# JianCao92/speaker-diarization

Hardware: AMD Instinct MI355X
Metric: diarized audio throughput (CD gw/BIC + CL hi/BIC) (higher is better)
Workload: dtype f64

## Files before the change

include/spkd.h:

```cpp
#ifndef SPKD_H
#define SPKD_H

#include <stddef.h>
#include <stdint.h>

#ifdef __cplusplus
extern "C" {
#endif

#define SPKD_ABI_VERSION 2
#define SPKD_DIM 39
#define SPKD_REC 820

typedef enum {
    SPKD_OK = 0,
    SPKD_EINVAL = 1,
    SPKD_EHIP = 2,
    SPKD_ENONFINITE = 3,
    SPKD_EOVERFLOW = 4,
    SPKD_ENOMEM = 5
} spkd_status;

typedef enum { SPKD_BIC = 0, SPKD_GLR = 1, SPKD_KL2 = 2, SPKD_KL2_PINV = 3 } spkd_kind;


typedef struct spkd_ctx spkd_ctx;

int spkd_abi_version(void);

spkd_status spkd_create(int device, void *stream, spkd_ctx **out);
spkd_status spkd_create_on_stream(int device, void *stream, spkd_ctx **out);
void spkd_destroy(spkd_ctx *ctx);
const char *spkd_last_error(const spkd_ctx *ctx);
spkd_status spkd_sync(spkd_ctx *ctx);

spkd_status spkd_malloc(spkd_ctx *ctx, size_t bytes, void **d_ptr);
spkd_status spkd_free(spkd_ctx *ctx, void *d_ptr);
spkd_status spkd_memcpy_h2d(spkd_ctx *ctx, void *d_dst, const void *h_src, size_t bytes);
spkd_status spkd_memcpy_d2h(spkd_ctx *ctx, void *h_dst, const void *d_src, size_t bytes);
spkd_status spkd_memcpy_d2d(spkd_ctx *ctx, void *d_dst, const void *d_src, size_t bytes);

enum {
    SPKD_T_CALL = 0, SPKD_T_CHUNK_STATS, SPKD_T_REDUCE_SETS, SPKD_T_PAIR_TERMS,
    SPKD_T_CLUSTER_PREP, SPKD_T_MATRIX, SPKD_T_AHC, SPKD_T_GW, SPKD_T_SW, SPKD_N_TIMERS
};
spkd_status spkd_last_kernel_ms(spkd_ctx *ctx, int which, float *ms);

spkd_status spkd_last_gw_items(spkd_ctx *ctx, int64_t *items);

spkd_status spkd_set_stats(spkd_ctx *ctx, const float *d_frames, int64_t n_frames,
                           const int64_t *h_range_begin, const int64_t *h_range_end,
                           const int32_t *h_range_set, int64_t n_ranges,
                           int64_t n_sets, double *d_stats);

#define SPKD_WANT_GLR 1
#define SPKD_WANT_KL2 2
#define SPKD_WANT_KL2_PINV 4
spkd_status spkd_pair_terms(spkd_ctx *ctx, const double *d_stats,
                            const int32_t *h_idx_a, const int32_t *h_idx_b,
                            int64_t n_pairs, int flags, double *h_terms);

spkd_status spkd_distance_matrix(spkd_ctx *ctx, int kind, double lambdac,
                                 const double *d_stats, int64_t n, double *d_matrix);

spkd_status spkd_cluster_in(spkd_ctx *ctx, const double *d_stats, int64_t n, int kind,
                            double lambdac, double threshold, int32_t *h_label,
                            double *h_dist, int64_t dist_cap, int64_t *h_dist_off,
                            int64_t *h_n_done, int64_t *h_n_clusters);

spkd_status spkd_distance_rows(spkd_ctx *ctx, int variant, int kind, double lambdac,
                               const double *d_stats, int64_t n, int64_t row_begin, int64_t row_end,
                               double *d_rows, double *h_stat_max, double *h_stat_min);

typedef struct {
    int32_t kind;
    int32_t trace;
    double lambdac;
    double threshold;
    double winsize;
    double winstep;
    double deltaws;
    double rate;
} spkd_cd_params;

typedef struct {
    int32_t turn;
    int32_t coarse;
    int64_t seq;
    double start, i, d;
    int64_t n1, n2;
} spkd_cand_log;

int64_t spkd_gw_event_capacity(int64_t turn_len, double rate);
int64_t spkd_gw_event_capacity_p(int64_t turn_len, const spkd_cd_params *params);
spkd_status spkd_gw(spkd_ctx *ctx, const float *d_frames, int64_t n_frames,
                    const int64_t *h_turn_begin, const int64_t *h_turn_end, int64_t n_turns,
                    const spkd_cd_params *params, const int64_t *h_ev_off,
                    int32_t *h_n_win, double *h_win_maxd, int32_t *h_win_det,
                    double *h_det_start, double *h_det_maxi, double *h_det_d,
                    double *h_final_start,
                    spkd_cand_log *h_log, int64_t log_cap, int64_t *h_log_count);

spkd_status spkd_gw_ex(spkd_ctx *ctx, const float *d_frames, int64_t n_frames,
                       const int64_t *h_turn_begin, const int64_t *h_turn_end, int64_t n_turns,
                       const spkd_cd_params *params, const int64_t *h_ev_off, int check_capacity,
                       int32_t *h_n_win, double *h_win_maxd, int32_t *h_win_det,
                       double *h_det_start, double *h_det_maxi, double *h_det_d,
                       double *h_final_start,
                       spkd_cand_log *h_log, int64_t log_cap, int64_t *h_log_count);

spkd_status spkd_gw_fused(spkd_ctx *ctx, const float *d_frames, int64_t n_frames,
                          const int64_t *h_turn_begin, const int64_t *h_turn_end, int64_t n_turns,
                          const spkd_cd_params *params, const int64_t *h_ev_off, int check_capacity,
                          int32_t *h_n_win, double *h_win_maxd, int32_t *h_win_det,
                          double *h_det_start, double *h_det_maxi, double *h_det_d,
                          double *h_final_start, double *d_seg_stats,
                          spkd_cand_log *h_log, int64_t log_cap, int64_t *h_log_count);

spkd_status spkd_gather_stats(spkd_ctx *ctx, const double *d_src, int64_t n_src,
                              const int64_t *h_src_index, const int64_t *h_dst_index,
                              int64_t n, int64_t n_dst, double *d_dst);

typedef struct {
    int64_t n_lines;
    int64_t n_redo;
    const int32_t *n_win;
    const double *times;
    const int32_t *turn;
    const int64_t *frame_b;
    const int64_t *frame_e;
    const int64_t *index;
    const int64_t *d_index;
    const int64_t *redo_line;
    const int64_t *redo_begin;
    const int64_t *redo_end;
} spkd_gw_lines_view;

spkd_status spkd_gw_batch(spkd_ctx *ctx, const float *d_frames, int64_t n_frames,
                          const int64_t *h_turn_begin, const int64_t *h_turn_end, int64_t n_turns,
                          const spkd_cd_params *params, const int64_t *h_ev_off,
                          const double *h_turn_start_s, const double *h_turn_end_s,
                          const int64_t *h_turn_file_off, const int64_t *h_turn_file_len,
                          double *d_seg_stats, int want_index, spkd_gw_lines_view *view);

int64_t spkd_sw_window_count(int64_t turn_len, double winsize, double winstep);
spkd_status spkd_sw(spkd_ctx *ctx, const float *d_frames, int64_t n_frames,
                    const int64_t *h_turn_begin, const int64_t *h_turn_end, int64_t n_turns,
                    const spkd_cd_params *params, const int64_t *h_d_off, double *h_d);

enum { SPKD_AHC_AUTO = 0, SPKD_AHC_MONO = 1, SPKD_AHC_WIDE = 2 };

typedef struct {
    int32_t variant;
    int32_t kind;
    int32_t max_spk;
    int32_t path;
    double lambdac;
    double threshold;
} spkd_ahc_params;

spkd_status spkd_ahc(spkd_ctx *ctx, const double *d_stats, const int64_t *h_seg_off,
                     int64_t n_problems, const spkd_ahc_params *params,
                     int32_t *h_n_merges, int32_t *h_merge_a, int32_t *h_merge_b,
                     double *h_merge_d, double *h_stat_max, double *h_stat_min);

spkd_status spkd_ahc_matrix(spkd_ctx *ctx, const double *d_stats, int64_t n, const spkd_ahc_params *params,
                            const double *d_matrix, double stat_max_in, double stat_min_in,
                            int32_t *h_n_merges, int32_t *h_merge_a, int32_t *h_merge_b,
                            double *h_merge_d, double *h_stat_max, double *h_stat_min);

spkd_status spkd_ahc_fused(spkd_ctx *ctx, const float *d_frames, int64_t n_frames,
                           const double *d_records, int64_t n_records, int64_t *d_line_index,
                           const int64_t *h_seg_off, int64_t n_problems,
                           const int64_t *h_redo_line, const int64_t *h_redo_begin,
                           const int64_t *h_redo_end, int64_t n_redo,
                           const spkd_ahc_params *params,
                           const int32_t **h_n_merges, const int32_t **h_merge_a,
                           const int32_t **h_merge_b, const double **h_merge_d,
                           const int32_t **h_labels);

typedef struct {
    int32_t sample_rate, frame_rate, window_width, n_fft, n_mel, n_cep;
    int32_t cms_left, cms_right;
    int32_t delta_width[2];
    float pre_emph;
    float delta_norm[2];
} spkd_mfcc_params;
spkd_status spkd_mfcc(spkd_ctx *ctx, const int16_t *d_pcm, int64_t n_samples,
                      const spkd_mfcc_params *params, const float *h_melfb, const float *h_dct,
                      const float *h_mean, const float *h_scale, const float *h_transform,
                      float *d_features, int64_t *h_n_frames);

typedef struct {
    int32_t n_kernels, n_states, dim;
    const float *mean;
    const float *inv_var;
    const float *log_norm;
    const int32_t *state_off;
    const int32_t *kernel;
    const float *log_weight;
} spkd_gmm_params;
spkd_status spkd_gmm_loglik(spkd_ctx *ctx, const float *d_features, int64_t n_frames,
                            const spkd_gmm_params *params, float *d_scores);

void spkd_py2_roundtrip(double *h_values, int64_t n);
spkd_status spkd_labels_from_merges(int64_t n, int64_t n_merges, const int32_t *h_a,
                                    const int32_t *h_b, int32_t *h_labels);
spkd_status spkd_labels_from_merges_batch(int64_t n_problems, const int64_t *h_seg_off,
                                          const int32_t *h_n_merges, const int32_t *h_a,
                                          const int32_t *h_b, int32_t *h_labels);

spkd_status spkd_count_flags(const int32_t *h_flags, const int64_t *h_off, const int32_t *h_n,
                             int64_t n_groups, int32_t *h_out);

spkd_status spkd_gw_lines(int64_t n_turns, const int64_t *h_off, const int32_t *h_n_det,
                          const double *h_det_start, const double *h_det_maxi,
                          const double *h_final_start, const double *h_turn_start_s,
                          const double *h_turn_end_s, const int64_t *h_turn_begin,
                          const int64_t *h_turn_end, double rate, int text_contract,
                          int64_t n_lines, double *h_times, int64_t *h_frame_b,
                          int64_t *h_frame_e, int64_t *h_index, int32_t *h_line_turn);

spkd_status spkd_vad_viterbi(int64_t n_frames, int32_t n_states, const float *h_scores,
                             int32_t n_words, const int32_t *h_word_state, const double *h_stay,
                             const double *h_exit, const double *h_enter, int64_t *h_tok_frame,
                             int32_t *h_tok_word, int64_t *h_n_tokens, double *h_score);

#ifdef __cplusplus
}
#endif
#endif
```

speaker-diarization_amd/csrc/spkd_cluster.hpp:

```cpp
#pragma once
#include "spkd_device.hpp"
#include "spkd_quad.hpp"
#include "spkd_tri.hpp"
#include "../../include/spkd.h"

namespace spkd {

constexpr double MAXINT_F = 9223372036854775808.0;
constexpr double PEN_UNIT = 39.0 + 0.5 * 39.0 * 40.0;
constexpr int AUX = 3 * DA;
constexpr int ERR_DEGENERATE_MERGE = 2;

__device__ __forceinline__ unsigned long long dkey(double v) {
    unsigned long long b = (unsigned long long)__double_as_longlong(v);
    return (b >> 63) ? ~b : (b | 0x8000000000000000ull);
}
__device__ __forceinline__ double dkey_inv(unsigned long long k) {
    unsigned long long b = (k >> 63) ? (k & 0x7fffffffffffffffull) : ~k;
    return __longlong_as_double((long long)b);
}
template <bool MAXOP>
__device__ __forceinline__ unsigned wave_red_u32(unsigned x) {
    auto op = [](unsigned a, unsigned b) { return MAXOP ? (a > b ? a : b) : (a < b ? a : b); };
    x = op(x, (unsigned)__builtin_amdgcn_update_dpp((int)x, (int)x, 0xB1, 0xf, 0xf, false));
// ... 522 lines not shown
            const double* row = Dm + r * N;
            double mv = __builtin_huge_val();
            int mc = NO_COL, nc = NO_COL;
            for (long long c0 = 0; c0 < N; c0 += 4 * WAVE) {
                double v[4];
                int a[4];
#pragma unroll
                for (int u = 0; u < 4; ++u) {
                    const long long c = c0 + u * WAVE + lane;
                    const long long cc = c < N ? c : N - 1;
                    a[u] = (c < N) ? al[cc] : 0;
                    v[u] = row[cc];
                }
#pragma unroll
                for (int u = 0; u < 4; ++u) {
                    const int c = (int)(c0 + u * WAVE + lane);
                    if (!a[u]) continue;
                    if (v[u] != v[u]) { if (c < nc) nc = c; continue; }
                    if (v[u] < mv || (v[u] == mv && c < mc)) { mv = v[u]; mc = c; }
                }
            }
            {
                unsigned long long okey;
                unsigned oc;
                wave_argmin_key(mc != NO_COL ? dkey(mv) : ~0ull, (unsigned)mc, okey, oc);
                mv = okey != ~0ull ? dkey_inv(okey) : __builtin_huge_val();
                mc = okey != ~0ull ? (int)oc : NO_COL;
                nc = __any(nc != NO_COL) ? (int)wave_red_u32<false>((unsigned)nc) : NO_COL;
            }
            if (lane == 0) { rmin[r] = mv; rarg[r] = mc; rnan[r] = nc; dirty[r] = 0; }
#ifdef SPKD_PROFILE
            if (lane == 0) atomicAdd(&g_ahc_prof[0], 1ull);
#endif
        }
    }
}

template <bool TWO>
__global__ __launch_bounds__(AHC_TPB) void k_ahc(
        double* __restrict__ ex, double* __restrict__ pk, const int64_t* __restrict__ seg_off,
        int variant, int kind, int max_spk, double lambdac, double threshold,
        double* __restrict__ ld, double* __restrict__ aux,
        double* __restrict__ mat, const int64_t* __restrict__ mat_off,
        int32_t* __restrict__ alive, double* __restrict__ tmp,
        double* __restrict__ rmin_all, int32_t* __restrict__ rcache_all,
        int32_t* __restrict__ out_n, int32_t* __restrict__ out_a, int32_t* __restrict__ out_b,
        double* __restrict__ out_d, unsigned long long* stat_max, unsigned long long* stat_min,
        double* __restrict__ final_max, double* __restrict__ final_min, int* err,
        double* pinv_ws) {
    extern __shared__ int32_t ids[];
    __shared__ double ldsA[QREC];
    __shared__ unsigned long long red3[AHC_WAVES][3];
    __shared__ unsigned long long s_masks[AHC_MAX_N / WAVE];
    __shared__ int s_cnt[2];
    __shared__ int s_nids;
    __shared__ int s_next;
    __shared__ double s_tmax[AHC_WAVES];
    const int tid = threadIdx.x, lane = lane_id(), wave = tid >> 6;
    const QuadLane L = quad_lane();
    const int p = blockIdx.x;
    const int64_t off = seg_off[p];
    const long long N = seg_off[p + 1] - off;
    double* Dm = mat + mat_off[p];
    int32_t* al = alive + off;
    double* ldp = ld + off;
    double* tp = tmp + off;
    double* rmin = rmin_all + off;
    int32_t* rarg = rcache_all + 3 * off;
    int32_t* rnan = rarg + N;
    int32_t* dirty = rnan + N;
    for (long long c = tid; c < N; c += AHC_TPB) { al[c] = 1; dirty[c] = 1; }
    __syncthreads();
    long long m = N;
    int n_merges = 0;
    const long long INF_IDX = 0x7fffffffffffffffLL;
    double fmin = 0.0;
#ifdef SPKD_PROFILE
    unsigned long long ahc_acc[5] = {0ull, 0ull, 0ull, 0ull, 0ull}, ahc_t = clock64();
#define AHC_TICK(i) do { const unsigned long long now_ = clock64(); ahc_acc[i] += now_ - ahc_t; ahc_t = now_; } while (0)
#else
#define AHC_TICK(i) ((void)0)
#endif
    while (true) {
        refresh_rows(Dm, N, al, dirty, rmin, rarg, rnan, s_masks, tid, wave, lane);
        __syncthreads();
        AHC_TICK(0);
        unsigned long long kb = ~0ull, ib = ~0ull, inan = ~0ull;
        for (long long r = tid; r < N; r += AHC_TPB) {
            if (!al[r]) continue;
            const double v = rmin[r];
            const int c = rarg[r], nc = rnan[r];
            if (nc != NO_COL) { const unsigned long long l = (unsigned long long)(r * N + nc); inan = l < inan ? l : inan; }
            if (c != NO_COL) {
                const unsigned long long kv = dkey(v);
                if (kv < kb) { kb = kv; ib = (unsigned long long)(r * N + c); }
            }
        }
        {
            const unsigned long long wk = wave_red_u64<false>(kb);
            const unsigned long long wi = wave_red_u64<false>(kb == wk ? ib : ~0ull);
            const unsigned long long wn = __any(inan != ~0ull) ? wave_red_u64<false>(inan) : ~0ull;
            if (lane == 0) { red3[wave][0] = wk; red3[wave][1] = wi; red3[wave][2] = wn; }
        }
        __syncthreads();
        unsigned long long bk = red3[0][0], bi = red3[0][1], bn = red3[0][2];
#pragma unroll
        for (int w = 1; w < AHC_WAVES; ++w) {
            const unsigned long long ok = red3[w][0], oi = red3[w][1], on = red3[w][2];
            const bool t = ok < bk || (ok == bk && oi < bi);
            bk = t ? ok : bk; bi = t ? oi : bi;
            bn = on < bn ? on : bn;
        }
        const bool has_nan = bn != ~0ull;
        const double mind = has_nan ? __builtin_nan("") : (bi != ~0ull ? dkey_inv(bk) : __builtin_huge_val());
        const long long index = has_nan ? (long long)bn : (bi != ~0ull ? (long long)bi : INF_IDX);
        fmin = mind;
        const bool go = (mind <= threshold) || (max_spk > 0 && m > max_spk);
        if (!go) break;
        AHC_TICK(1);
        const long long r0 = index / N, c0 = index - r0 * N;
        if (r0 == c0) {
            if (tid == 0) atomicOr(err, ERR_DEGENERATE_MERGE);
            break;
        }
        const long long sa = r0 < c0 ? r0 : c0, sb = r0 < c0 ? c0 : r0;
        if (tid < 2) s_cnt[tid] = 0;
        if (tid == 0) { s_nids = 1; s_next = 0; }
        __syncthreads();
        {
            int ca = 0, cb = 0;
            for (long long c = tid; c < sb; c += AHC_TPB) {
                if (al[c]) { cb++; if (c < sa) ca++; }
            }
            ca = __builtin_amdgcn_readlane(wave_scan_i32(ca), WAVE - 1);
            cb = __builtin_amdgcn_readlane(wave_scan_i32(cb), WAVE - 1);
            if (lane == 0 && ca) atomicAdd(&s_cnt[0], ca);
            if (lane == 0 && cb) atomicAdd(&s_cnt[1], cb);
        }
        __syncthreads();
        if (tid == 0) {
            const int64_t o = off + n_merges;
            out_a[o] = s_cnt[0]; out_b[o] = s_cnt[1]; out_d[o] = mind;
            al[sb] = 0;
            ids[0] = (int32_t)sa;
        }
        n_merges++;
        m--;
#ifdef SPKD_PROFILE
        if (tid == 0) atomicAdd(&g_ahc_prof[1], 1ull);
#endif
        double* A = ex + (off + sa) * QREC;
        const double* B = ex + (off + sb) * QREC;
        {
            double* Ap = pk + (off + sa) * REC;
            const double* Bp = pk + (off + sb) * REC;
            constexpr int NQ = (QREC + AHC_TPB - 1) / AHC_TPB, NP = (REC + AHC_TPB - 1) / AHC_TPB;
            double qa[NQ], qb[NQ], pa[NP], pb[NP];
#pragma unroll
            for (int u = 0; u < NQ; ++u) {
                const int e = tid + u * AHC_TPB;
                qa[u] = A[e < QREC ? e : 0]; qb[u] = B[e < QREC ? e : 0];
            }
#pragma unroll
            for (int u = 0; u < NP; ++u) {
                const int e = tid + u * AHC_TPB;
                pa[u] = Ap[e < REC ? e : 0]; pb[u] = Bp[e < REC ? e : 0];
            }
#pragma unroll
            for (int u = 0; u < NQ; ++u) {
                const int e = tid + u * AHC_TPB;
                const double v = qa[u] + qb[u];
                if (e < QREC) { A[e] = v; ldsA[e] = v; }
            }
#pragma unroll
            for (int u = 0; u < NP; ++u) {
                const int e = tid + u * AHC_TPB;
                if (e < REC) Ap[e] = pa[u] + pb[u];
            }
        }
        __syncthreads();
        for (long long c0 = 0; c0 < N; c0 += AHC_TPB) {
            const long long c = c0 + tid;
            const bool take = c < N && c != sa && al[c < N ? c : N - 1];
            const unsigned long long mk = __ballot(take);
            int base = 0;
            if (lane == 0 && mk) base = atomicAdd(&s_nids, __popcll(mk));
            base = __shfl(base, 0);
            if (take) ids[base + __popcll(mk & ((1ull << lane) - 1ull))] = (int32_t)c;
        }
        __syncthreads();
        AHC_TICK(2);
        const int nids = s_nids;
        const double nA = ldsA[QREC_COUNT_AT];
        if (kind == SPKD_KL2) {
            if (wave == 0) {
                double a[DA];
                single_rows_from_qr(A, a);
                const double mean_i = a[D] / nA;
                cov_rows(a, nA);
                kl2_aux_from_cov(a, mean_i, aux + (off + sa) * AUX, pinv_ws);
            }
        } else {
            for (;;) {
                int q4 = 0;
                if (lane == 0) q4 = atomicAdd(&s_next, 1);
                const int base = 4 * __builtin_amdgcn_readfirstlane(q4);
                if (base >= nids) break;
                int k = base + L.m;
                const bool valid = k < nids;
                k = valid ? k : nids - 1;
                const int32_t slot = ids[k];
                const double v = quad_pair_det<TWO>(kind, ldsA, nA, A, ex + (off + slot) * QREC, pk + (off + slot) * REC, k == 0, L, err);
                if (valid && L.t == 0) {
                    if (k == 0) ldp[sa] = log(v); else tp[slot] = v;
                }
            }
        }
        __syncthreads();
        AHC_TICK(3);
        double wmax = __builtin_nan(""), wmin = __builtin_nan("");
        const double ldA = ldp[sa];
        for (long long c = tid; c < N; c += AHC_TPB) {
            if (c == sa || !al[c]) continue;
            double d;
            if (kind == SPKD_KL2) {
                const double* a1 = aux + (off + sa) * AUX;
                const double* a2 = aux + (off + c) * AUX;
                double t1 = 0.0, t2 = 0.0;
                for (int i = 0; i < D; ++i) {
                    const float dm = (float)a1[2 * DA + i] - (float)a2[2 * DA + i];
                    const double delta = (double)dm;
                    t1 += (a1[i] - a2[i]) * (a2[DA + i] - a1[DA + i]);
                    t2 += ((a1[DA + i] + a2[DA + i]) * delta) * delta;
                }
                d = 0.5 * t1 + 0.5 * t2;
            } else {
                const double nC = qr_count(ex + (off + c) * QREC);
                d = finish_distance(kind, lambdac, nA, ldA, nC, ldp[c], log(tp[c]));
            }
            Dm[sa * N + c] = d;
            const int ra = rarg[c], rn = rnan[c];
            if (variant == 1) {
                Dm[c * N + sa] = d;
                if (ra == sa || ra == sb || rn == sa || rn == sb) {
                    if (rn != sa && rn != sb && d < rmin[c]) { rmin[c] = d; rarg[c] = (int)sa; }
                    else dirty[c] = 1;
                }
                else if (d != d) { if ((int)sa < rn) rnan[c] = (int)sa; }
                else if (d < rmin[c] || (d == rmin[c] && (int)sa < ra)) { rmin[c] = d; rarg[c] = (int)sa; }
                if (stat_valid(d)) {
                    wmax = (wmax != wmax || d > wmax) ? d : wmax;
                    wmin = (wmin != wmin || d < wmin) ? d : wmin;
                }
            } else {
                if (ra == sb || rn == sb) dirty[c] = 1;
            }
        }
        if (tid == 0) dirty[sa] = 1;
        if (variant == 1) {
            const unsigned long long kmax = wave_red_u64<true>(wmax == wmax ? dkey(wmax) : 0ull);
            const unsigned long long kmin = wave_red_u64<false>(wmin == wmin ? dkey(wmin) : ~0ull);
            if (lane == 0) {
                if (kmax != 0ull) atomicMax(stat_max + p, kmax);
                if (kmin != ~0ull) atomicMin(stat_min + p, kmin);
            }
        }
        __syncthreads();
        AHC_TICK(4);
    }
#ifdef SPKD_PROFILE
    if (tid == 0) for (int i = 0; i < 5; ++i) atomicAdd(&g_ahc_prof[2 + i], ahc_acc[i]);
#endif
    double tmax = -__builtin_huge_val();
    bool anynan = false;
    for (long long r = wave; r < N; r += AHC_WAVES) {
        if (!al[r]) continue;
        const double* row = Dm + r * N;
        for (long long c = lane; c < N; c += WAVE) {
            if (!al[c]) continue;
            const double v = row[c];
            if (v != v) anynan = true; else tmax = v > tmax ? v : tmax;
        }
    }
#pragma unroll
    for (int s = 1; s < WAVE; s <<= 1) {
        const double t2 = __shfl_xor(tmax, s);
        tmax = t2 > tmax ? t2 : tmax;
    }
    anynan = __any(anynan);
    if (lane == 0) s_tmax[wave] = anynan ? __builtin_nan("") : tmax;
    __syncthreads();
    if (tid == 0) {
        double mx = s_tmax[0];
        for (int w = 1; w < AHC_WAVES; ++w) {
            const double x = s_tmax[w];
            if (mx == mx) mx = (x != x) ? x : (x > mx ? x : mx);
        }
        out_n[p] = n_merges;
        final_max[p] = mx;
        final_min[p] = fmin;
    }
}

__device__ __forceinline__ void ahc_scan_row(const double* __restrict__ row, long long N,
                                             const int32_t* __restrict__ al, bool all_alive,
                                             long long sub_col, double sub_val, int lane,
                                             double& mv, int& mc, int& nc) {
    mv = __builtin_huge_val();
    mc = NO_COL; nc = NO_COL;
    for (long long c0 = 0; c0 < N; c0 += 4 * WAVE) {
        double v[4];
        int a[4];
#pragma unroll
        for (int u = 0; u < 4; ++u) {
            const long long c = c0 + u * WAVE + lane;
            const long long cc = c < N ? c : N - 1;
            a[u] = (c < N) ? (all_alive ? 1 : al[cc]) : 0;
            v[u] = row[cc];
        }
#pragma unroll
        for (int u = 0; u < 4; ++u) {
            const long long cl = c0 + u * WAVE + lane;
            const int c = (int)cl;
            if (!a[u]) continue;
            const double x = (cl == sub_col) ? sub_val : v[u];
            if (x != x) { if (c < nc) nc = c; continue; }
            if (x < mv || (x == mv && c < mc)) { mv = x; mc = c; }
        }
    }
#pragma unroll
    for (int s = 1; s < WAVE; s <<= 1) {
        const double v2 = __shfl_xor(mv, s);
        const int c2 = __shfl_xor(mc, s), n2 = __shfl_xor(nc, s);
        if (v2 < mv || (v2 == mv && c2 < mc)) { mv = v2; mc = c2; }
        nc = n2 < nc ? n2 : nc;
    }
}

constexpr int STEP_WAVES = 4;
constexpr int STEP_WIDE_FROM = 1024;
constexpr int STEP_PARTNERS = 4 * STEP_WAVES - 1;
constexpr int ALIVE_ROUND = 0x7fffffff;
constexpr int STEP_MAX_N = 16384;
constexpr int STEP_IDX_SHIFT = 14;

struct StepState {
    int32_t done, n_merges;
    long long psa;
    double fmin;
    double diag;
};

__host__ __device__ inline unsigned long long step_slot_word(int round, int new_slot, int old_slot) {
    return ((unsigned long long)(unsigned)round << 40) | ((unsigned long long)(unsigned)new_slot << 20) |
           (unsigned long long)(unsigned)old_slot;
}
__device__ __forceinline__ int step_slot_of(unsigned long long w, int k) {
    return ((int)(w >> 40) < k) ? (int)((w >> 20) & 0xfffffull) : (int)(w & 0xfffffull);
}

struct StepSel {
    double rmin, newrow;
    int32_t rarg, rnan, death, pad;
};

struct StepArrays {
    double* ex;
    double* pk;
    double* exm;
    double* pkm;
    int32_t* death;
    StepSel* sel2;
    unsigned long long* sw;
    double* cnt;
    StepState* state2;
    int64_t n_total;
    int32_t n_prob;
};

__global__ __launch_bounds__(AHC_TPB) void k_step_init(
        const int64_t* __restrict__ seg_off, const double* __restrict__ mat,
        const int64_t* __restrict__ mat_off, StepArrays Q) {
    const int lane = lane_id(), wave = threadIdx.x >> 6;
    const int p = blockIdx.y;
    const int64_t off = seg_off[p];
    const long long N = seg_off[p + 1] - off;
    if (blockIdx.x == 0 && threadIdx.x == 0) {
        StepState S;
        S.done = 0; S.n_merges = 0; S.psa = -1; S.fmin = 0.0; S.diag = 0.0;
        Q.state2[(size_t)1 * Q.n_prob + p] = S;
        Q.state2[(size_t)0 * Q.n_prob + p] = S;
    }
    const long long r = (long long)blockIdx.x * AHC_WAVES + wave;
    if (r >= N) return;
    double mv;
    int mc, nc;
    ahc_scan_row(mat + mat_off[p] + r * N, N, nullptr, true, -1, 0.0, lane, mv, mc, nc);
    if (lane == 0) {
        StepSel e;
        e.rmin = mv; e.newrow = 0.0; e.rarg = mc; e.rnan = nc; e.death = ALIVE_ROUND; e.pad = 0;
        Q.sel2[Q.n_total + off + r] = e;
        Q.sel2[off + r] = e;
        Q.death[off + r] = ALIVE_ROUND;
        Q.sw[off + r] = step_slot_word(0, (int)r, (int)r);
        Q.cnt[off + r] = Q.pk[(off + r) * REC + REC - 1];
    }
}

__device__ __forceinline__ void step_scan_row(const double* __restrict__ row, long long N,
                                              const int32_t* __restrict__ death, int k, long long sb,
                                              long long sub_col, double sub_val, int lane,
                                              double& mv, int& mc, int& nc) {
    mv = __builtin_huge_val();
    mc = NO_COL; nc = NO_COL;
    for (long long c0 = 0; c0 < N; c0 += 4 * WAVE) {
        double v[4];
        int a[4];
#pragma unroll
        for (int u = 0; u < 4; ++u) {
            const long long c = c0 + u * WAVE + lane;
            const long long cc = c < N ? c : N - 1;
            a[u] = (c < N && c != sb) ? (death[cc] > k ? 1 : 0) : 0;
            v[u] = row[cc];
        }
#pragma unroll
        for (int u = 0; u < 4; ++u) {
            const long long cl = c0 + u * WAVE + lane;
            const int c = (int)cl;
            if (!a[u]) continue;
            const double x = (cl == sub_col) ? sub_val : v[u];
            if (x != x) { if (c < nc) nc = c; continue; }
            if (x < mv || (x == mv && c < mc)) { mv = x; mc = c; }
        }
    }
#pragma unroll
    for (int s = 1; s < WAVE; s <<= 1) {
        const double v2 = __shfl_xor(mv, s);
        const int c2 = __shfl_xor(mc, s), n2 = __shfl_xor(nc, s);
        if (v2 < mv || (v2 == mv && c2 < mc)) { mv = v2; mc = c2; }
        nc = n2 < nc ? n2 : nc;
    }
}

template <bool TWO, int SW, int SP>
__global__ __launch_bounds__(SW * WAVE) void k_ahc_step(
        int k, const int64_t* __restrict__ seg_off, int variant, int kind, int max_spk, double lambdac,
        double threshold, double* __restrict__ ld, double* __restrict__ aux,
        double* __restrict__ mat, const int64_t* __restrict__ mat_off, StepArrays Q,
        int32_t* __restrict__ out_a, int32_t* __restrict__ out_b, double* __restrict__ out_d,
        unsigned long long* stat_max, unsigned long long* stat_min, int* err,
        double* pinv_ws) {
    constexpr int TPB = SW * WAVE;
    extern __shared__ int32_t s_dyn[];
    __shared__ double ldsA[QREC];
    __shared__ double s_auxA[AUX];
    __shared__ double s_ldx[4 * STEP_WAVES];
    __shared__ double s_dfin[4 * STEP_WAVES];
    __shared__ int s_rescan[4 * STEP_WAVES];
    struct RowRed { double mv; int mc, nc; };
    struct WaveRed { unsigned long long kb, kr, kmax, kmin; unsigned ib, inan; int mc, nc; };
    __shared__ WaveRed wred[SW];
    __shared__ int s_cnt[2];
    const int tid = threadIdx.x, lane = lane_id(), wave = tid >> 6;
    const QuadLane L = quad_lane();
    const int p = blockIdx.y;
#ifdef SPKD_PROFILE
    unsigned long long st_t = clock64();
#define STEP_TICK(i) do { const unsigned long long now_ = clock64(); if (blockIdx.x == 0 && tid == 0) atomicAdd(&g_ahc_prof[i], now_ - st_t); st_t = now_; } while (0)
    unsigned long long st_f = st_t;
#define STEP_FINE(i) do { const unsigned long long now_ = clock64(); if (blockIdx.x == 0 && tid == 0) atomicAdd(&g_step_prof[i], now_ - st_f); st_f = now_; } while (0)
#else
#define STEP_TICK(i) ((void)0)
#define STEP_FINE(i) ((void)0)
#endif
    asm volatile("" :: "s"(Q.state2), "s"(Q.sel2), "s"(Q.sw), "s"(Q.ex), "s"(Q.exm), "s"(Q.n_total), "s"(Q.n_prob),
                 "s"(seg_off), "s"(mat_off), "s"(mat), "s"(k));
    StepState S = Q.state2[(size_t)(k & 1) * Q.n_prob + p];
    StepState* Snext = Q.state2 + (size_t)((k + 1) & 1) * Q.n_prob + p;
    int64_t off = seg_off[p], off_end = seg_off[p + 1], moff = mat_off[p];
    asm volatile("" :: "s"(S.done), "s"(S.n_merges), "s"(off), "s"(off_end), "s"(moff));
    const long long N = off_end - off;
    const bool lead = blockIdx.x == 0;
    if (S.done) {
        if (lead && tid == 0) *Snext = S;
        return;
    }
    STEP_FINE(0);
    const int n_merges = S.n_merges;
    const long long psa = S.psa;
    const long long m = N - n_merges;
    const int n_part = (int)(m - 2);
    constexpr int sp = SP;
    const int nb = n_part > 0 ? (n_part + sp - 1) / sp : 1;
    if ((int)blockIdx.x > nb) return;
    const bool keeper = (int)blockIdx.x == nb;
    int32_t* s_ids = s_dyn;
    int32_t* s_slot = s_dyn + N;
    const int nch = (int)((N + WAVE - 1) / WAVE);
    int32_t* s_base = s_dyn + 2 * N;
    unsigned long long* s_mask = reinterpret_cast<unsigned long long*>(s_dyn + ((2 * N + nch + 1) & ~1LL));
    const int rb = k & 1, wb = (k + 1) & 1;
    const int32_t* death = Q.death + off;
    const StepSel* sel_r = Q.sel2 + (size_t)rb * Q.n_total + off;
    StepSel* sel_w = Q.sel2 + (size_t)wb * Q.n_total + off;
    double* Dm = mat + moff;
    double* ldp = ld + off;
    const long long INF_IDX = 0x7fffffffffffffffLL;
    auto rec_quad = [&](int slot) -> const double* {
        return slot < N ? Q.ex + (off + slot) * QREC : Q.exm + (off + (slot - N)) * QREC;
    };
    auto rec_packed = [&](int slot) -> const double* {
        return slot < N ? Q.pk + (off + slot) * REC : Q.pkm + (off + (slot - N)) * REC;
    };
    const double diag_psa = S.diag;
    const bool hp = psa >= 0, v1 = variant == 1;
    const unsigned NONE = 0xffffffffu;
    unsigned long long kb = ~0ull, kr = ~0ull, kmax = 0ull, kmin = ~0ull;
    unsigned ib = NONE, inan = NONE;
    int mc = NO_COL, nc = NO_COL;
    constexpr int SEL_U = 8;
    for (long long xb = 0; xb < N; xb += (long long)SEL_U * TPB) {
        const long long x0 = xb + tid;
        int dth[SEL_U], c_[SEL_U], rn_[SEL_U];
        unsigned long long w_[SEL_U];
        double dn_[SEL_U], v_[SEL_U];
#pragma unroll
        for (int u = 0; u < SEL_U; ++u) {
            if (xb + (long long)u * TPB < N) {
                const long long x = x0 + (long long)u * TPB;
                const long long xc = x < N ? x : N - 1;
                const StepSel e = sel_r[xc];
                w_[u] = Q.sw[off + xc];
                dth[u] = e.death; dn_[u] = e.newrow; v_[u] = e.rmin; c_[u] = e.rarg; rn_[u] = e.rnan;
            }
        }
#pragma unroll
        for (int u = 0; u < SEL_U; ++u) {
            if (xb + (long long)u * TPB >= N) break;
            const long long x = x0 + (long long)u * TPB;
            const unsigned xu = (unsigned)x;
            const bool in = x < N;
            const bool a = in && dth[u] >= k;
            const unsigned long long mk = __ballot(a);
            if (in) {
                s_slot[x] = a ? step_slot_of(w_[u], k) : -1;
                if (lane == 0) s_mask[x >> 6] = mk;
            }
            const bool np = a && x != psa;
            const unsigned long long kv = dkey(v_[u]);
            const bool bet = np && c_[u] != NO_COL && kv < kb;
            kb = bet ? kv : kb;
            ib = bet ? ((xu << STEP_IDX_SHIFT) | (unsigned)c_[u]) : ib;
            const unsigned ni = (np && rn_[u] != NO_COL) ? ((xu << STEP_IDX_SHIFT) | (unsigned)rn_[u]) : NONE;
            inan = ni < inan ? ni : inan;
            if (hp) {
                const double d = x == psa ? diag_psa : dn_[u];
                const bool dnan = d != d;
                const unsigned long long kd = dkey(d);
                const bool bt = a && !dnan && kd < kr;
                kr = bt ? kd : kr;
                mc = bt ? (int)x : mc;
                nc = (a && dnan && (int)x < nc) ? (int)x : nc;
                if (v1) {
                    const bool sv = np && stat_valid(d);
                    kmax = (sv && kd > kmax) ? kd : kmax;
                    kmin = (sv && kd < kmin) ? kd : kmin;
                }
            }
        }
    }
    STEP_FINE(1);
    {
        WaveRed w;
        wave_argmin_key(kb, ib, w.kb, w.ib);
        w.inan = __any(inan != NONE) ? wave_red_u32<false>(inan) : NONE;
        w.kr = ~0ull; w.mc = NO_COL; w.nc = NO_COL; w.kmax = 0ull; w.kmin = ~0ull;
        if (hp) {
            unsigned mcu;
            wave_argmin_key(kr, (unsigned)mc, w.kr, mcu);
            w.mc = (int)mcu;
            if (__any(nc != NO_COL)) w.nc = (int)wave_red_u32<false>((unsigned)nc);
            if (v1) { w.kmax = wave_red_u64<true>(kmax); w.kmin = wave_red_u64<false>(kmin); }
        }
        STEP_FINE(2);
        if (lane == 0) wred[wave] = w;
    }
    __syncthreads();
    WaveRed fw[SW];
#pragma unroll
    for (int w = 0; w < SW; ++w) fw[w] = wred[w];
#pragma unroll
    for (int st = 1; st < SW; st <<= 1) {
#pragma unroll
        for (int w = 0; w + st < SW; w += 2 * st) {
            WaveRed& x = fw[w];
            const WaveRed& o = fw[w + st];
            const bool b1 = o.kb < x.kb || (o.kb == x.kb && o.ib < x.ib);
            x.kb = b1 ? o.kb : x.kb; x.ib = b1 ? o.ib : x.ib;
            x.inan = o.inan < x.inan ? o.inan : x.inan;
            const bool b2 = o.kr < x.kr || (o.kr == x.kr && o.mc < x.mc);
            x.kr = b2 ? o.kr : x.kr; x.mc = b2 ? o.mc : x.mc;
            x.nc = o.nc < x.nc ? o.nc : x.nc;
            x.kmax = o.kmax > x.kmax ? o.kmax : x.kmax;
            x.kmin = o.kmin < x.kmin ? o.kmin : x.kmin;
        }
    }
// ... 363 lines not shown
```

speaker-diarization_amd/csrc/spkd_hip.hip:

```cpp
#include <hip/hip_runtime.h>

#include <algorithm>
#include <cmath>
#include <cstddef>
#include <cstdio>
#include <cstdlib>
#include <cstring>
#include <string>
#include <atomic>
#include <thread>
#include <vector>

#include "../../include/spkd.h"
#include "spkd_cd.hpp"
#include "spkd_cluster.hpp"
#include "spkd_device.hpp"
#include "spkd_handoff.hpp"
#include "spkd_stats.hpp"
#include "spkd_mfcc.hpp"
#include "spkd_vad.hpp"

using namespace spkd;

namespace {
constexpr int N_SLOTS = 40;
enum { PIN_GW_TURNS = 0, PIN_GW_LINES, PIN_AHC_OUT, N_PIN };
}

struct spkd_ctx {
    int device = 0;
    hipStream_t stream = nullptr;
    bool own_stream = false;
    bool gw_lds_ok = false;
    int gw_waves = 0;
    unsigned long long init_keys[2] = {0ull, ~0ull};
    int step_waves = 0;
    int step_partners = 0;
    int64_t last_gw_items = 0;
    std::string err;
    int* d_err = nullptr;
    unsigned long long* d_counter = nullptr;
    hipEvent_t ev0 = nullptr, ev1 = nullptr;
    float last_ms = 0.f;
    hipEvent_t ka[SPKD_N_TIMERS] = {}, kb[SPKD_N_TIMERS] = {};
    bool kused[SPKD_N_TIMERS] = {};
    float kms[SPKD_N_TIMERS] = {};
    void* slot[N_SLOTS] = {};
    size_t slot_bytes[N_SLOTS] = {};
    void* pinv_ws = nullptr;
    double* pinv_cur = nullptr;
    void* pin[N_PIN] = {};
    size_t pin_bytes[N_PIN] = {};
    std::vector<int64_t> redo_line, redo_begin, redo_end;
    std::vector<Chunk> redo_chunks;
    std::vector<int64_t> redo_setoff;
    std::vector<int32_t> redo_sets;
};

namespace {

spkd_status fail(spkd_ctx* c, spkd_status s, const std::string& msg) {
    if (c) c->err = msg;
    return s;
}

#define HIPCHK(c, call)                                                              \
    do {                                                                             \
        hipError_t e_ = (call);                                                      \
        if (e_ != hipSuccess)                                                        \
            return fail((c), SPKD_EHIP, std::string(#call) + ": " + hipGetErrorString(e_)); \
    } while (0)

#define TRY(expr) do { const spkd_status s_ = (expr); if (s_ != SPKD_OK) return s_; } while (0)

spkd_status scratch(spkd_ctx* c, int slot, size_t bytes, void** out) {
    if (bytes == 0) bytes = 16;
    if (c->slot_bytes[slot] < bytes) {
        if (c->slot[slot]) HIPCHK(c, hipFree(c->slot[slot]));
        c->slot[slot] = nullptr;
        c->slot_bytes[slot] = 0;
        size_t want = bytes + bytes / 4;
        hipError_t e = hipMalloc(&c->slot[slot], want);
        if (e != hipSuccess) {
            want = bytes;
            e = hipMalloc(&c->slot[slot], want);
        }
        if (e != hipSuccess) return fail(c, SPKD_ENOMEM, "scratch allocation failed");
        c->slot_bytes[slot] = want;
    }
    *out = c->slot[slot];
    return SPKD_OK;
}

spkd_status pinned(spkd_ctx* c, int which, size_t bytes, void** out) {
    if (bytes == 0) bytes = 16;
    if (c->pin_bytes[which] < bytes) {
        if (c->pin[which]) HIPCHK(c, hipHostFree(c->pin[which]));
        c->pin[which] = nullptr;
        c->pin_bytes[which] = 0;
        const size_t want = bytes + bytes / 4;
        if (hipHostMalloc(&c->pin[which], want, hipHostMallocDefault) != hipSuccess) {
            c->pin[which] = nullptr;
            return fail(c, SPKD_ENOMEM, "pinned host allocation failed");
        }
        c->pin_bytes[which] = want;
    }
    *out = c->pin[which];
    return SPKD_OK;
}

template <class T>
spkd_status upload(spkd_ctx* c, int slot, const T* h, size_t n, T** d) {
    void* p = nullptr;
    TRY(scratch(c, slot, n * sizeof(T), &p));
    if (n) HIPCHK(c, hipMemcpyAsync(p, h, n * sizeof(T), hipMemcpyHostToDevice, c->stream));
    *d = (T*)p;
    return SPKD_OK;
}

struct Layout {
    char* const base;
    char* const stage;
    size_t at = 0;
    explicit Layout(void* b = nullptr, void* s = nullptr) : base((char*)b), stage((char*)s) {}
    template <class T>
    Layout& part(T*& p, size_t count, const T* src = nullptr) {
        at = (at + alignof(T) - 1) / alignof(T) * alignof(T);
        p = base ? (T*)(base + at) : nullptr;
        if (stage && src) std::memcpy(stage + at, src, count * sizeof(T));
        at += count * sizeof(T);
        return *this;
    }
    size_t bytes() const { return at; }
};

template <class Parts>
spkd_status carve(spkd_ctx* c, spkd_status (*alloc)(spkd_ctx*, int, size_t, void**), int slot, Parts parts) {
    void* p = nullptr;
    TRY(alloc(c, slot, parts(Layout()), &p));
    parts(Layout(p));
    return SPKD_OK;
}

template <class Parts>
spkd_status upload_parts(spkd_ctx* c, int slot, std::vector<char>& image, Parts parts) {
    image.resize(parts(Layout()));
    parts(Layout(nullptr, image.data()));
    char* d = nullptr;
    TRY(upload(c, slot, image.data(), image.size(), &d));
    parts(Layout(d));
    return SPKD_OK;
}

struct Call {
    spkd_ctx* const c;
    spkd_status opened;
    int herr = 0;
    bool drained = false;
    explicit Call(spkd_ctx* ctx) : c(ctx) { opened = open(); }
    ~Call() { if (!drained) (void)hipStreamSynchronize(c->stream); }
    spkd_status open() {
        HIPCHK(c, hipSetDevice(c->device));
        for (int i = 0; i < SPKD_N_TIMERS; ++i) c->kused[i] = false;
        HIPCHK(c, hipMemsetAsync(c->d_err, 0, sizeof(int), c->stream));
        HIPCHK(c, hipEventRecord(c->ev0, c->stream));
        return SPKD_OK;
    }

    spkd_status finish() {
        HIPCHK(c, hipEventRecord(c->ev1, c->stream));
        HIPCHK(c, hipMemcpyAsync(&herr, c->d_err, sizeof(int), hipMemcpyDeviceToHost, c->stream));
        HIPCHK(c, hipStreamSynchronize(c->stream));
        drained = true;
        HIPCHK(c, hipEventElapsedTime(&c->last_ms, c->ev0, c->ev1));
        c->kms[0] = c->last_ms;
        for (int i = 1; i < SPKD_N_TIMERS; ++i)
            if (c->kused[i]) HIPCHK(c, hipEventElapsedTime(&c->kms[i], c->ka[i], c->kb[i]));
        if (herr & ERR_SWEEP) return fail(c, SPKD_EHIP, "internal error: growing-window sweep order");
        if (herr & 4) return fail(c, SPKD_EOVERFLOW, "device scratch capacity exceeded");
        if (herr & ERR_DEGENERATE_MERGE) return fail(c, SPKD_EINVAL, "degenerate merge: a diagonal cell was the minimum");
        if (herr & ERR_NONFINITE) return fail(c, SPKD_ENONFINITE, "array must not contain infs or NaNs");
        return SPKD_OK;
    }
};

spkd_status use_kind(spkd_ctx* c, int kind, int* base) {
    c->pinv_cur = nullptr;
    *base = kind;
    if (kind != SPKD_KL2_PINV) return SPKD_OK;
    *base = SPKD_KL2;
    if (!c->pinv_ws) {
        if (hipMalloc(&c->pinv_ws, PINV_WS_BYTES) != hipSuccess) {
            c->pinv_ws = nullptr;
            return fail(c, SPKD_ENOMEM, "pinv workspace allocation failed");
        }
        HIPCHK(c, hipMemsetAsync(c->pinv_ws, 0, PINV_LOCK_BYTES, c->stream));
    }
    c->pinv_cur = (double*)c->pinv_ws;
    return SPKD_OK;
}

bool bad_kind(int kind) { return kind < 0 || kind > 3; }

template <class Params>
spkd_status kernel_params(spkd_ctx* c, const Params*& P, Params& Pk) {
    Pk = *P;
    TRY(use_kind(c, P->kind, &Pk.kind));
    P = &Pk;
    return SPKD_OK;
}

struct Timer {
    spkd_ctx* const c;
    const int idx;
    Timer(spkd_ctx* ctx, int i) : c(ctx), idx(i) { (void)hipEventRecord(c->ka[idx], c->stream); }
    ~Timer() { (void)hipEventRecord(c->kb[idx], c->stream); c->kused[idx] = true; }
};

enum {
    S_CHUNKS = 0, S_SETOFF, S_PARTIAL, S_IDXA, S_IDXB, S_TERMS, S_TURNS, S_SNAP, S_CAND,
    S_GW_N_WIN, S_GW_WIN_DET, S_GW_WIN_MAXD, S_GW_DET_START, S_GW_DET_MAXI, S_GW_DET_D, S_GW_FINAL_START, S_LOG,
    S_AHC_STATS, S_AHC_LD, S_AHC_AUX, S_AHC_MAT, S_AHC_MISC, S_AHC_OUT, S_AHC_OFF, S_AHC_PROB, S_AHC_PACKED, S_MFCC_TAB, S_MFCC_STATIC,
    S_STEP_EXM, S_STEP_PKM, S_STEP_MISC, S_GMM_TAB, S_GMM_IDX,
    S_CP_TURNS, S_CP_TIMES, S_CP_LINES, S_REDO_STATS, S_REDO_IDX, S_COUNT
};
static_assert(S_COUNT <= N_SLOTS, "scratch slot table too small");

}

extern "C" {

int spkd_abi_version(void) { return SPKD_ABI_VERSION; }

static spkd_status create_ctx(int device, void* stream, bool borrow, spkd_ctx** out) {
    if (!out) return SPKD_EINVAL;
    *out = nullptr;
    int count = 0;
    if (hipGetDeviceCount(&count) != hipSuccess || device < 0 || device >= count) return SPKD_EHIP;
    spkd_ctx* c = new spkd_ctx();
    c->device = device;
    if (hipSetDevice(device) != hipSuccess) { delete c; return SPKD_EHIP; }
    if (borrow) {
        c->stream = (hipStream_t)stream;
    } else {
        if (hipStreamCreateWithFlags(&c->stream, hipStreamDefault) != hipSuccess) { delete c; return SPKD_EHIP; }
        c->own_stream = true;
    }
    if (hipMalloc(&c->d_err, sizeof(int)) != hipSuccess ||
        hipMalloc(&c->d_counter, 2 * sizeof(unsigned long long)) != hipSuccess ||
        hipEventCreate(&c->ev0) != hipSuccess || hipEventCreate(&c->ev1) != hipSuccess) {
        spkd_destroy(c);
        return SPKD_EHIP;
    }
    for (int i = 0; i < SPKD_N_TIMERS; ++i)
        if (hipEventCreate(&c->ka[i]) != hipSuccess || hipEventCreate(&c->kb[i]) != hipSuccess) {
            spkd_destroy(c);
            return SPKD_EHIP;
        }
    int lds_max = 0;
    c->gw_lds_ok = hipDeviceGetAttribute(&lds_max, hipDeviceAttributeMaxSharedMemoryPerBlock, device) == hipSuccess &&
                   Gw<4>::LDS_BYTES <= lds_max &&
                   hipFuncSetAttribute((const void*)k_gw<8>, hipFuncAttributeMaxDynamicSharedMemorySize, Gw<8>::LDS_BYTES) == hipSuccess &&
                   hipFuncSetAttribute((const void*)k_gw<4>, hipFuncAttributeMaxDynamicSharedMemorySize, Gw<4>::LDS_BYTES) == hipSuccess &&
                   hipFuncSetAttribute((const void*)k_gw<2>, hipFuncAttributeMaxDynamicSharedMemorySize, Gw<2>::LDS_BYTES) == hipSuccess &&
                   hipFuncSetAttribute((const void*)k_gw<1>, hipFuncAttributeMaxDynamicSharedMemorySize, Gw<1>::LDS_BYTES) == hipSuccess;
    if (const char* e = getenv("SPKD_GW_WAVES")) c->gw_waves = atoi(e);
    if (const char* e = getenv("SPKD_STEP_WAVES")) { const int v = atoi(e); c->step_waves = (v == 4 || v == 8) ? v : 0; }
    if (const char* e = getenv("SPKD_STEP_PARTNERS")) { const int v = atoi(e); c->step_partners = (v == 3 || v == 7 || v == 15) ? v : 0; }
    *out = c;
    return SPKD_OK;
}

spkd_status spkd_create(int device, void* stream, spkd_ctx** out) {
    return create_ctx(device, stream, stream != nullptr, out);
}

spkd_status spkd_create_on_stream(int device, void* stream, spkd_ctx** out) {
    return create_ctx(device, stream, true, out);
}

void spkd_destroy(spkd_ctx* c) {
    if (!c) return;
    (void)hipSetDevice(c->device);
    if (c->stream) (void)hipStreamSynchronize(c->stream);
    for (int i = 0; i < N_SLOTS; ++i)
        if (c->slot[i]) (void)hipFree(c->slot[i]);
    if (c->d_err) (void)hipFree(c->d_err);
    if (c->pinv_ws) (void)hipFree(c->pinv_ws);
    for (int i = 0; i < N_PIN; ++i)
        if (c->pin[i]) (void)hipHostFree(c->pin[i]);
    if (c->d_counter) (void)hipFree(c->d_counter);
    if (c->ev0) (void)hipEventDestroy(c->ev0);
    if (c->ev1) (void)hipEventDestroy(c->ev1);
    for (int i = 0; i < SPKD_N_TIMERS; ++i) {
        if (c->ka[i]) (void)hipEventDestroy(c->ka[i]);
        if (c->kb[i]) (void)hipEventDestroy(c->kb[i]);
    }
    if (c->own_stream && c->stream) (void)hipStreamDestroy(c->stream);
    delete c;
}

const char* spkd_last_error(const spkd_ctx* c) { return c ? c->err.c_str() : "null context"; }

spkd_status spkd_sync(spkd_ctx* c) {
    if (!c) return SPKD_EINVAL;
    HIPCHK(c, hipStreamSynchronize(c->stream));
    return SPKD_OK;
}

spkd_status spkd_malloc(spkd_ctx* c, size_t bytes, void** d_ptr) {
    if (!c || !d_ptr) return SPKD_EINVAL;
    HIPCHK(c, hipSetDevice(c->device));
    hipError_t e = hipMalloc(d_ptr, bytes ? bytes : 16);
    if (e != hipSuccess) return fail(c, SPKD_ENOMEM, hipGetErrorString(e));
    return SPKD_OK;
}

spkd_status spkd_free(spkd_ctx* c, void* d_ptr) {
    if (!c) return SPKD_EINVAL;
    HIPCHK(c, hipFree(d_ptr));
    return SPKD_OK;
}

spkd_status spkd_memcpy_h2d(spkd_ctx* c, void* d_dst, const void* h_src, size_t bytes) {
    if (!c) return SPKD_EINVAL;
    HIPCHK(c, hipMemcpyAsync(d_dst, h_src, bytes, hipMemcpyHostToDevice, c->stream));
    HIPCHK(c, hipStreamSynchronize(c->stream));
    return SPKD_OK;
}

spkd_status spkd_memcpy_d2h(spkd_ctx* c, void* h_dst, const void* d_src, size_t bytes) {
    if (!c) return SPKD_EINVAL;
    HIPCHK(c, hipMemcpyAsync(h_dst, d_src, bytes, hipMemcpyDeviceToHost, c->stream));
    HIPCHK(c, hipStreamSynchronize(c->stream));
    return SPKD_OK;
}

spkd_status spkd_memcpy_d2d(spkd_ctx* c, void* d_dst, const void* d_src, size_t bytes) {
    if (!c) return SPKD_EINVAL;
    HIPCHK(c, hipMemcpyAsync(d_dst, d_src, bytes, hipMemcpyDeviceToDevice, c->stream));
    HIPCHK(c, hipStreamSynchronize(c->stream));
    return SPKD_OK;
}

spkd_status spkd_last_gw_items(spkd_ctx* c, int64_t* items) {
    if (!c || !items) return SPKD_EINVAL;
    *items = c->last_gw_items;
    return SPKD_OK;
}

spkd_status spkd_last_kernel_ms(spkd_ctx* c, int which, float* ms) {
    if (!c || !ms || which < 0 || which >= SPKD_N_TIMERS) return SPKD_EINVAL;
    *ms = c->kms[which];
    return SPKD_OK;
}

namespace {
spkd_status set_stats_launch(spkd_ctx* c, const float* d_frames, int64_t n_frames,
                             const int64_t* h_begin, const int64_t* h_end, const int32_t* h_set,
                             int64_t n_ranges, int64_t n_sets, double* d_stats,
                             std::vector<Chunk>& chunks, std::vector<int64_t>& set_off) {
    chunks.clear();
    set_off.assign((size_t)n_sets + 1, 0);
    int32_t prev = 0;
    for (int64_t r = 0; r < n_ranges; ++r) {
        const int64_t b = h_begin[r], e = h_end[r];
        const int32_t s = h_set[r];
        if (b < 0 || e < b || e > n_frames || s < prev || s >= n_sets)
            return fail(c, SPKD_EINVAL, "bad frame range or set id");
        prev = s;
        for (int64_t t = b; t < e; t += STATS_CHUNK) {
            Chunk ch;
            ch.begin = t;
            ch.len = (int32_t)std::min<int64_t>(STATS_CHUNK, e - t);
            ch.set = s;
            chunks.push_back(ch);
            set_off[(size_t)s + 1]++;
        }
    }
    for (int64_t s = 0; s < n_sets; ++s) set_off[(size_t)s + 1] += set_off[(size_t)s];
    Chunk* d_chunks = nullptr;
    int64_t* d_setoff = nullptr;
    void* d_partial = nullptr;
    TRY(upload(c, S_CHUNKS, chunks.data(), chunks.size(), &d_chunks));
    TRY(upload(c, S_SETOFF, set_off.data(), set_off.size(), &d_setoff));
    TRY(scratch(c, S_PARTIAL, chunks.size() * REC * sizeof(double), &d_partial));
    if (!chunks.empty()) {
        Timer t(c, SPKD_T_CHUNK_STATS);
        hipLaunchKernelGGL(k_chunk_stats, dim3((unsigned)chunks.size()), dim3(STATS_TPB), 0, c->stream,
                           d_frames, d_chunks, (double*)d_partial);
    }
    Timer t(c, SPKD_T_REDUCE_SETS);
    hipLaunchKernelGGL(k_reduce_sets, dim3((unsigned)n_sets), dim3(STATS_TPB), 0, c->stream,
                       (const double*)d_partial, d_setoff, d_stats);
    HIPCHK(c, hipGetLastError());
    return SPKD_OK;
}
}

spkd_status spkd_set_stats(spkd_ctx* c, const float* d_frames, int64_t n_frames,
                           const int64_t* h_begin, const int64_t* h_end, const int32_t* h_set,
                           int64_t n_ranges, int64_t n_sets, double* d_stats) {
    if (!c || !d_stats || n_sets < 0 || n_ranges < 0) return SPKD_EINVAL;
    if (n_sets == 0) return SPKD_OK;
    if (n_ranges > 0 && (!h_begin || !h_end || !h_set || !d_frames)) return fail(c, SPKD_EINVAL, "null range arrays");
    std::vector<Chunk> chunks;
    std::vector<int64_t> set_off;
    Call call(c);
    TRY(call.opened);
    TRY(set_stats_launch(c, d_frames, n_frames, h_begin, h_end, h_set, n_ranges, n_sets, d_stats, chunks, set_off));
    return call.finish();
}

spkd_status spkd_pair_terms(spkd_ctx* c, const double* d_stats, const int32_t* h_a, const int32_t* h_b,
                            int64_t n_pairs, int flags, double* h_terms) {
    if (!c || n_pairs < 0) return SPKD_EINVAL;
    if (n_pairs == 0) return SPKD_OK;
    if (!d_stats || !h_a || !h_b || !h_terms) return fail(c, SPKD_EINVAL, "null argument");
    if ((flags & SPKD_WANT_KL2) && (flags & SPKD_WANT_KL2_PINV))
        return fail(c, SPKD_EINVAL, "pair_terms: SPKD_WANT_KL2 and SPKD_WANT_KL2_PINV exclude each other");
    Call call(c);
    TRY(call.opened);
    int kind_unused;
    TRY(use_kind(c, (flags & SPKD_WANT_KL2_PINV) ? (int)SPKD_KL2_PINV : (int)SPKD_KL2, &kind_unused));
    if (flags & SPKD_WANT_KL2_PINV) flags = (flags & ~SPKD_WANT_KL2_PINV) | SPKD_WANT_KL2;
    int32_t *d_a = nullptr, *d_b = nullptr;
    void* d_terms = nullptr;
    TRY(upload(c, S_IDXA, h_a, (size_t)n_pairs, &d_a));
    TRY(upload(c, S_IDXB, h_b, (size_t)n_pairs, &d_b));
    TRY(scratch(c, S_TERMS, (size_t)n_pairs * 8 * sizeof(double), &d_terms));
    const unsigned blocks = (unsigned)((n_pairs + PT2_WAVES - 1) / PT2_WAVES);
    {
        Timer t(c, SPKD_T_PAIR_TERMS);
        hipLaunchKernelGGL(k_pair_terms, dim3(blocks), dim3(PT2_WAVES * WAVE), 0, c->stream,
                           d_stats, d_a, d_b, n_pairs, flags, (double*)d_terms, c->d_err, c->pinv_cur);
    }
    HIPCHK(c, hipGetLastError());
    HIPCHK(c, hipMemcpyAsync(h_terms, d_terms, (size_t)n_pairs * 8 * sizeof(double), hipMemcpyDeviceToHost, c->stream));
    return call.finish();
}

namespace {
struct AhcPrep {
    double* ex;
    double* pk;
    double* ld;
    double* aux;
    double* mat;
    int64_t* seg_off;
    int64_t* mat_off;
    unsigned long long* smax;
    unsigned long long* smin;
    int64_t n_total = 0;
    int64_t grid_rows = 0;
    std::vector<char> offs;
    std::vector<char> prob_of;
};

unsigned long long host_dkey(double v) {
    unsigned long long b;
    std::memcpy(&b, &v, sizeof b);
    return (b >> 63) ? ~b : (b | 0x8000000000000000ull);
}

struct MatrixPlan {
    const double* d_init = nullptr;
    double init_max = NAN, init_min = NAN;
    int64_t row_begin = -1, row_end = -1;
    int64_t* d_map = nullptr;
    int64_t n_src = 0;
    const float* d_frames = nullptr;
    int64_t n_frames = 0;
    const int64_t *redo_line = nullptr, *redo_begin = nullptr, *redo_end = nullptr;
    int64_t n_redo = 0;
};

void to_quadrec(spkd_ctx* c, const double* d_stats, int64_t n, double* ex) {
    hipLaunchKernelGGL(k_to_quadrec, dim3((unsigned)n), dim3(256), 0, c->stream, d_stats, n, ex);
}

void cluster_prep(spkd_ctx* c, const double* ex, int64_t n, int kind, double* ld, double* aux) {
    const int64_t per_block = kind == SPKD_KL2 ? PT_WAVES : 4 * PT_WAVES;
    const unsigned blocks = (unsigned)((n + per_block - 1) / per_block);
    hipLaunchKernelGGL(k_cluster_prep, dim3(blocks), dim3(PT_WAVES * WAVE), 0, c->stream, ex, n, kind, ld, aux, c->d_err,
                       c->pinv_cur);
}

spkd_status ahc_prepare(spkd_ctx* c, const double* d_stats, const int64_t* h_seg_off, int64_t n_prob,
                        int variant, int kind, double lambdac, AhcPrep& B, const MatrixPlan& plan = MatrixPlan()) {
    const int64_t n_total = B.n_total = h_seg_off[n_prob];
    const size_t np = (size_t)n_prob;
    std::vector<int64_t> mat_off(np + 1);
    int64_t cells = 0;
    for (int64_t p = 0; p < n_prob; ++p) {
        const int64_t n = h_seg_off[p + 1] - h_seg_off[p];
        if (n < 0) return fail(c, SPKD_EINVAL, "seg_off must be non-decreasing");
        mat_off[(size_t)p] = cells;
        cells += n * n;
    }
    mat_off[np] = cells;
    std::vector<int32_t> prob((size_t)n_total, 0);
    for (int64_t p = 0; p < n_prob; ++p)
        for (int64_t r = h_seg_off[p]; r < h_seg_off[p + 1]; ++r) prob[(size_t)r] = (int32_t)p;
    int32_t *d_prob = nullptr, *d_sched = nullptr;
    {
        const int X = 8;
        std::vector<std::vector<int32_t>> lists(X);
        if (plan.row_begin >= 0) {
            for (int64_t r = plan.row_begin; r < plan.row_end; ++r) lists[(size_t)((r - plan.row_begin) % X)].push_back((int32_t)r);
        } else if (n_prob >= X) {
            std::vector<int64_t> order((size_t)n_prob);
            for (int64_t p = 0; p < n_prob; ++p) order[(size_t)p] = p;
            std::stable_sort(order.begin(), order.end(), [&](int64_t a, int64_t b) {
                return h_seg_off[a + 1] - h_seg_off[a] > h_seg_off[b + 1] - h_seg_off[b];
            });
            double load[X] = {0, 0, 0, 0, 0, 0, 0, 0};
            for (int64_t p : order) {
                int x = 0;
                for (int i = 1; i < X; ++i) if (load[i] < load[x]) x = i;
                const double n = (double)(h_seg_off[p + 1] - h_seg_off[p]);
                load[x] += n * n;
                for (int64_t r = h_seg_off[p]; r < h_seg_off[p + 1]; ++r) lists[x].push_back((int32_t)r);
            }
        } else {
            for (int64_t r = 0; r < n_total; ++r) lists[(size_t)(r % X)].push_back((int32_t)r);
        }
        size_t longest = 0;
        for (auto& l : lists) longest = std::max(longest, l.size());
        B.grid_rows = (int64_t)longest * X;
        std::vector<int32_t> sched((size_t)B.grid_rows, -1);
        for (int x = 0; x < X; ++x)
            for (size_t i = 0; i < lists[x].size(); ++i) sched[i * X + x] = lists[x][i];
        TRY(upload_parts(c, S_AHC_OFF, B.offs, [&](Layout L) {
            return L.part(B.seg_off, np + 1, h_seg_off).part(B.mat_off, np + 1, mat_off.data()).bytes();
        }));
        TRY(upload_parts(c, S_AHC_PROB, B.prob_of, [&](Layout L) {
            return L.part(d_prob, prob.size(), prob.data()).part(d_sched, sched.size(), sched.data()).bytes();
        }));
    }
    const size_t nt = (size_t)n_total;
    TRY(carve(c, scratch, S_AHC_LD, [&](Layout L) { return L.part(B.ld, nt).bytes(); }));
    TRY(carve(c, scratch, S_AHC_AUX, [&](Layout L) { return L.part(B.aux, nt * AUX).bytes(); }));
    TRY(carve(c, scratch, S_AHC_MAT, [&](Layout L) { return L.part(B.mat, (size_t)cells).bytes(); }));
    TRY(carve(c, scratch, S_AHC_MISC, [&](Layout L) { return L.part(B.smax, np).part(B.smin, np).bytes(); }));
    HIPCHK(c, hipMemsetAsync(B.smax, 0x00, (size_t)n_prob * sizeof(unsigned long long), c->stream));
    HIPCHK(c, hipMemsetAsync(B.smin, 0xff, (size_t)n_prob * sizeof(unsigned long long), c->stream));
    if (plan.d_init && n_prob == 1) {
        c->init_keys[0] = plan.init_max == plan.init_max ? host_dkey(plan.init_max) : 0ull;
        c->init_keys[1] = plan.init_min == plan.init_min ? host_dkey(plan.init_min) : ~0ull;
        HIPCHK(c, hipMemcpyAsync(B.smax, &c->init_keys[0], sizeof(unsigned long long), hipMemcpyHostToDevice, c->stream));
        HIPCHK(c, hipMemcpyAsync(B.smin, &c->init_keys[1], sizeof(unsigned long long), hipMemcpyHostToDevice, c->stream));
    }
    TRY(carve(c, scratch, S_AHC_STATS, [&](Layout L) { return L.part(B.ex, nt * QREC).bytes(); }));
    TRY(carve(c, scratch, S_AHC_PACKED, [&](Layout L) { return L.part(B.pk, nt * REC).bytes(); }));
    if (n_total > 0) {
        if (plan.d_map) {
            void* d_redo = nullptr;
            if (plan.n_redo > 0) {
                int64_t* d_rl = nullptr;
                TRY(scratch(c, S_REDO_STATS, (size_t)plan.n_redo * REC * sizeof(double), &d_redo));
                TRY(upload(c, S_REDO_IDX, plan.redo_line, (size_t)plan.n_redo, &d_rl));
                c->redo_sets.resize((size_t)plan.n_redo);
                for (int64_t k = 0; k < plan.n_redo; ++k) c->redo_sets[(size_t)k] = (int32_t)k;
                TRY(set_stats_launch(c, plan.d_frames, plan.n_frames, plan.redo_begin, plan.redo_end, c->redo_sets.data(),
                                     plan.n_redo, plan.n_redo, (double*)d_redo, c->redo_chunks, c->redo_setoff));
                hipLaunchKernelGGL(k_patch_map, dim3((unsigned)((plan.n_redo + 255) / 256)), dim3(256), 0, c->stream,
                                   (const int64_t*)d_rl, plan.n_redo, plan.d_map);
            }
            hipLaunchKernelGGL(k_records_from_map, dim3((unsigned)n_total), dim3(256), 0, c->stream, d_stats, plan.n_src,
                               (const int64_t*)plan.d_map, (const double*)d_redo, plan.n_redo, n_total, B.ex, B.pk, c->d_err);
        } else {
            to_quadrec(c, d_stats, n_total, B.ex);
            HIPCHK(c, hipMemcpyAsync(B.pk, d_stats, (size_t)n_total * REC * sizeof(double), hipMemcpyDeviceToDevice, c->stream));
        }
        {
            Timer t(c, SPKD_T_CLUSTER_PREP);
            cluster_prep(c, B.ex, n_total, kind, B.ld, B.aux);
        }
        auto kmat = kind == SPKD_GLR ? k_matrix<true> : k_matrix<false>;
        if (plan.d_init) {
            HIPCHK(c, hipMemcpyAsync(B.mat, plan.d_init, (size_t)cells * sizeof(double), hipMemcpyDeviceToDevice, c->stream));
        } else if (B.grid_rows > 0) {
            Timer t(c, SPKD_T_MATRIX);
            hipLaunchKernelGGL(kmat, dim3((unsigned)B.grid_rows), dim3(MX_WAVES * WAVE), 0, c->stream,
                               (const double*)B.ex, (const double*)B.pk, (const int64_t*)B.seg_off, (const int32_t*)d_prob,
                               (const int32_t*)d_sched, variant, kind, lambdac,
                               (const double*)B.ld, (const double*)B.aux, B.mat, (const int64_t*)B.mat_off,
                               B.smax, B.smin, c->d_err);
        }
    }
    HIPCHK(c, hipGetLastError());
    return SPKD_OK;
}

double key_to_double(unsigned long long k, bool is_max) {
    if (is_max ? (k == 0ull) : (k == ~0ull)) return std::nan("");
    unsigned long long b = (k >> 63) ? (k & 0x7fffffffffffffffull) : ~k;
    double v;
    std::memcpy(&v, &b, sizeof v);
    return v;
}
}

spkd_status spkd_distance_matrix(spkd_ctx* c, int kind, double lambdac, const double* d_stats,
                                 int64_t n, double* d_matrix) {
    if (!c || n < 0 || bad_kind(kind)) return SPKD_EINVAL;
    if (n == 0) return SPKD_OK;
    if (!d_stats || !d_matrix) return fail(c, SPKD_EINVAL, "null argument");
    const int64_t seg_off[2] = {0, n};
    AhcPrep B;
    Call call(c);
    TRY(call.opened);
    TRY(use_kind(c, kind, &kind));
    TRY(ahc_prepare(c, d_stats, seg_off, 1, 1, kind, lambdac, B));
    HIPCHK(c, hipMemcpyAsync(d_matrix, B.mat, (size_t)n * n * sizeof(double), hipMemcpyDeviceToDevice, c->stream));
    return call.finish();
}

spkd_status spkd_cluster_in(spkd_ctx* c, const double* d_stats, int64_t n, int kind, double lambdac, double threshold,
                            int32_t* h_label, double* h_dist, int64_t dist_cap, int64_t* h_dist_off,
                            int64_t* h_n_done, int64_t* h_n_clusters) {
    if (!c || n < 0 || dist_cap < 0 || bad_kind(kind)) return SPKD_EINVAL;
    if (h_n_done) *h_n_done = 0;
    if (h_n_clusters) *h_n_clusters = 0;
    if (n == 0) return SPKD_OK;
    if (!d_stats || !h_label || !h_dist_off || !h_n_done || !h_n_clusters || (dist_cap > 0 && !h_dist))
        return fail(c, SPKD_EINVAL, "null argument");
    long long done2[2] = {0, 0};
    Call call(c);
    TRY(call.opened);
    TRY(use_kind(c, kind, &kind));
    void *p_ex = nullptr, *p_ld = nullptr, *p_aux = nullptr, *p_cex = nullptr, *p_cpk = nullptr, *p_dist = nullptr;
    const size_t nn = (size_t)n;
    TRY(scratch(c, S_AHC_STATS, nn * QREC * sizeof(double), &p_ex));
    TRY(scratch(c, S_AHC_LD, nn * sizeof(double), &p_ld));
    TRY(scratch(c, S_AHC_AUX, nn * AUX * sizeof(double), &p_aux));
    TRY(scratch(c, S_STEP_EXM, nn * QREC * sizeof(double), &p_cex));
    TRY(scratch(c, S_STEP_PKM, nn * REC * sizeof(double), &p_cpk));
    double *clu_ld, *tmp, *clu_aux;
    long long *d_off, *d_done;
    int32_t* d_label;
    TRY(carve(c, scratch, S_STEP_MISC, [&](Layout L) {
        return L.part(clu_ld, nn).part(tmp, nn).part(clu_aux, nn * AUX).part(d_off, nn + 1).part(d_done, 2)
            .part(d_label, nn).bytes();
    }));
    TRY(scratch(c, S_AHC_MAT, (size_t)std::max<int64_t>(dist_cap, 1) * sizeof(double), &p_dist));
    HIPCHK(c, hipMemsetAsync(d_done, 0, 2 * sizeof(long long), c->stream));
    to_quadrec(c, d_stats, n, (double*)p_ex);
    {
        Timer t(c, SPKD_T_CLUSTER_PREP);
        cluster_prep(c, (const double*)p_ex, n, kind == SPKD_KL2 ? (int)SPKD_BIC : kind, (double*)p_ld, (double*)p_aux);
    }
    if (kind == SPKD_KL2) {
        void* p_ld2 = nullptr;
        TRY(scratch(c, S_AHC_OUT, nn * sizeof(double), &p_ld2));
        cluster_prep(c, (const double*)p_ex, n, SPKD_KL2, (double*)p_ld2, (double*)p_aux);
    }
    auto kin = kind == SPKD_GLR ? k_cluster_in<true> : k_cluster_in<false>;
    {
        Timer t(c, SPKD_T_AHC);
        hipLaunchKernelGGL(kin, dim3(1), dim3(CIN_TPB), 0, c->stream,
                           (const double*)p_ex, d_stats, (const double*)p_ld, (const double*)p_aux, (long long)n, kind, lambdac, threshold,
                           (double*)p_cex, (double*)p_cpk, clu_ld, clu_aux, tmp, d_label, (double*)p_dist, (long long)dist_cap,
                           d_off, d_done, c->d_err, c->pinv_cur);
    }
    HIPCHK(c, hipGetLastError());
    HIPCHK(c, hipMemcpyAsync(done2, d_done, sizeof done2, hipMemcpyDeviceToHost, c->stream));
    HIPCHK(c, hipMemcpyAsync(h_label, d_label, nn * sizeof(int32_t), hipMemcpyDeviceToHost, c->stream));
    HIPCHK(c, hipMemcpyAsync(h_dist_off, d_off, (nn + 1) * sizeof(long long), hipMemcpyDeviceToHost, c->stream));
    if (dist_cap > 0)
        HIPCHK(c, hipMemcpyAsync(h_dist, p_dist, (size_t)dist_cap * sizeof(double), hipMemcpyDeviceToHost, c->stream));
    const spkd_status st = call.finish();
    *h_n_done = done2[0];
    *h_n_clusters = done2[1];
    return st;
}

spkd_status spkd_distance_rows(spkd_ctx* c, int variant, int kind, double lambdac, const double* d_stats,
                               int64_t n, int64_t row_begin, int64_t row_end, double* d_rows,
                               double* h_stat_max, double* h_stat_min) {
    if (!c || n < 0 || bad_kind(kind) || (variant != 1 && variant != 2)) return SPKD_EINVAL;
    if (row_begin < 0 || row_end < row_begin || row_end > n) return fail(c, SPKD_EINVAL, "distance_rows: bad row block");
    if (h_stat_max) *h_stat_max = std::nan("");
    if (h_stat_min) *h_stat_min = std::nan("");
    if (n == 0 || row_end == row_begin) return SPKD_OK;
    if (!d_stats || !d_rows) return fail(c, SPKD_EINVAL, "null argument");
    const int64_t seg_off[2] = {0, n};
    AhcPrep B;
    MatrixPlan plan;
    plan.row_begin = row_begin;
    plan.row_end = row_end;
    unsigned long long keys[2] = {0ull, ~0ull};
    Call call(c);
    TRY(call.opened);
    TRY(use_kind(c, kind, &kind));
    TRY(ahc_prepare(c, d_stats, seg_off, 1, variant, kind, lambdac, B, plan));
    HIPCHK(c, hipMemcpyAsync(d_rows, B.mat + row_begin * n, (size_t)(row_end - row_begin) * n * sizeof(double),
                             hipMemcpyDeviceToDevice, c->stream));
    HIPCHK(c, hipMemcpyAsync(&keys[0], B.smax, sizeof(unsigned long long), hipMemcpyDeviceToHost, c->stream));
    HIPCHK(c, hipMemcpyAsync(&keys[1], B.smin, sizeof(unsigned long long), hipMemcpyDeviceToHost, c->stream));
    const spkd_status st = call.finish();
    if (h_stat_max) *h_stat_max = key_to_double(keys[0], true);
    if (h_stat_min) *h_stat_min = key_to_double(keys[1], false);
    return st;
}

namespace {
spkd_status ahc_impl(spkd_ctx* c, const double* d_stats, const int64_t* h_seg_off, int64_t n_prob,
                     const spkd_ahc_params* P, const MatrixPlan& plan, int32_t* h_n_merges, int32_t* h_merge_a,
                     int32_t* h_merge_b, double* h_merge_d, double* h_stat_max, double* h_stat_min) {
    if (!c || !P || n_prob < 0) return SPKD_EINVAL;
    if (n_prob == 0) return SPKD_OK;
    if (!d_stats || !h_seg_off || !h_n_merges || !h_merge_a || !h_merge_b || !h_merge_d ||
        !h_stat_max || !h_stat_min)
        return fail(c, SPKD_EINVAL, "null argument");
    if ((P->variant != 1 && P->variant != 2) || bad_kind(P->kind))
        return fail(c, SPKD_EINVAL, "bad variant / kind");
    for (int64_t p = 0; p < n_prob; ++p)
        if (h_seg_off[p + 1] - h_seg_off[p] < 1) return fail(c, SPKD_EINVAL, "empty clustering problem");
    int64_t n_max = 0;
    for (int64_t p = 0; p < n_prob; ++p) n_max = std::max<int64_t>(n_max, h_seg_off[p + 1] - h_seg_off[p]);
    if (n_max > AHC_MAX_N) return fail(c, SPKD_EINVAL, "clustering problem larger than 65536 records");
    int path = P->path;
    if (path != SPKD_AHC_MONO && path != SPKD_AHC_WIDE) path = n_prob <= 64 ? SPKD_AHC_WIDE : SPKD_AHC_MONO;
    const size_t lds = (size_t)(n_max + 4) * sizeof(int32_t);
    if (path == SPKD_AHC_MONO && lds > 150 * 1024) path = SPKD_AHC_WIDE;
    if (path == SPKD_AHC_WIDE && n_max > STEP_MAX_N)
        return fail(c, SPKD_EINVAL, "clustering problem larger than 16384 records (wide merge loop)");
    AhcPrep B;
    std::vector<unsigned long long> kmax((size_t)n_prob), kmin((size_t)n_prob);
    std::vector<double> fmax((size_t)n_prob), fmin((size_t)n_prob);
    Call call(c);
    TRY(call.opened);
    spkd_ahc_params Pk;
    TRY(kernel_params(c, P, Pk));
    TRY(ahc_prepare(c, d_stats, h_seg_off, n_prob, P->variant, P->kind, P->lambdac, B, plan));
    const int64_t n_total = B.n_total;
    const size_t nt = (size_t)n_total, np = (size_t)n_prob;
    double *d_merge_d, *d_tmp, *d_rmin, *d_fmax, *d_fmin;
    int32_t *d_a, *d_b, *d_alive, *d_rcache, *d_n;
    TRY(carve(c, scratch, S_AHC_OUT, [&](Layout L) {
        return L.part(d_merge_d, nt).part(d_tmp, nt).part(d_rmin, nt).part(d_fmax, np).part(d_fmin, np)
            .part(d_a, nt).part(d_b, nt).part(d_alive, nt).part(d_rcache, 3 * nt).part(d_n, np).bytes();
    }));
    if (path == SPKD_AHC_MONO) {
        auto kahc = P->kind == SPKD_GLR ? k_ahc<true> : k_ahc<false>;
        if (lds > 48 * 1024)
            (void)hipFuncSetAttribute((const void*)kahc, hipFuncAttributeMaxDynamicSharedMemorySize, (int)lds);
        Timer t(c, SPKD_T_AHC);
        hipLaunchKernelGGL(kahc, dim3((unsigned)n_prob), dim3(AHC_TPB), lds, c->stream,
                           B.ex, B.pk, (const int64_t*)B.seg_off, P->variant, P->kind, P->max_spk, P->lambdac,
                           P->threshold, B.ld, B.aux, B.mat, (const int64_t*)B.mat_off, d_alive, d_tmp,
                           d_rmin, d_rcache, d_n, d_a, d_b, d_merge_d, B.smax, B.smin, d_fmax, d_fmin, c->d_err,
                           c->pinv_cur);
    } else {
        StepArrays Q;
        void *pe = nullptr, *pp = nullptr;
        TRY(carve(c, scratch, S_STEP_MISC, [&](Layout L) {
            return L.part(Q.sel2, 2 * nt).part(Q.cnt, nt).part(Q.sw, nt).part(Q.state2, 2 * np).part(Q.death, nt).bytes();
        }));
        TRY(scratch(c, S_STEP_EXM, nt * QREC * sizeof(double), &pe));
        TRY(scratch(c, S_STEP_PKM, nt * REC * sizeof(double), &pp));
        Q.ex = B.ex; Q.pk = B.pk; Q.exm = (double*)pe; Q.pkm = (double*)pp;
        Q.n_total = n_total;
        Q.n_prob = (int32_t)n_prob;
        const int step_waves = c->step_waves ? c->step_waves : (n_max > STEP_WIDE_FROM ? 8 : 4);
        const bool glr_k = P->kind == SPKD_GLR;
        using StepKernel = decltype(&k_ahc_step<false, 4, 3>);
        StepKernel kvar[3];
        if (step_waves == 8) {
            kvar[0] = glr_k ? k_ahc_step<true, 8, 3> : k_ahc_step<false, 8, 3>;
            kvar[1] = glr_k ? k_ahc_step<true, 8, 7> : k_ahc_step<false, 8, 7>;
            kvar[2] = glr_k ? k_ahc_step<true, 8, STEP_PARTNERS> : k_ahc_step<false, 8, STEP_PARTNERS>;
        } else {
            kvar[0] = glr_k ? k_ahc_step<true, 4, 3> : k_ahc_step<false, 4, 3>;
            kvar[1] = glr_k ? k_ahc_step<true, 4, 7> : k_ahc_step<false, 4, 7>;
            kvar[2] = glr_k ? k_ahc_step<true, 4, STEP_PARTNERS> : k_ahc_step<false, 4, STEP_PARTNERS>;
        }
        auto sp_of_round = [&](int64_t partners) -> int {
            if (c->step_partners) return c->step_partners;
            const int64_t free_cus = 255;
            if (partners * n_prob <= 3 * free_cus) return 3;
            if (partners * n_prob <= 7 * free_cus) return 7;
            return STEP_PARTNERS;
        };
        const size_t nch_max = (size_t)((n_max + WAVE - 1) / WAVE);
        const size_t step_lds = ((size_t)2 * n_max + nch_max + 2) * sizeof(int32_t) + nch_max * sizeof(unsigned long long);
        if (step_lds + 20 * 1024 > 48 * 1024)
            for (int v = 0; v < 3; ++v)
                (void)hipFuncSetAttribute((const void*)kvar[v], hipFuncAttributeMaxDynamicSharedMemorySize, (int)step_lds);
        Timer t(c, SPKD_T_AHC);
        const unsigned row_blocks = (unsigned)((n_max + AHC_WAVES - 1) / AHC_WAVES);
        hipLaunchKernelGGL(k_step_init, dim3(row_blocks, (unsigned)n_prob), dim3(AHC_TPB), 0, c->stream,
                           (const int64_t*)B.seg_off, (const double*)B.mat, (const int64_t*)B.mat_off, Q);
        for (int64_t it = 1; it < n_max; ++it) {
            const int64_t partners = n_max - it - 1;
            const int step_sp = sp_of_round(partners);
            StepKernel kstep = kvar[step_sp == 3 ? 0 : (step_sp == 7 ? 1 : 2)];
            const unsigned blocks = (unsigned)std::max<int64_t>(1, (partners + step_sp - 1) / step_sp) + 1;
            hipLaunchKernelGGL(kstep, dim3(blocks, (unsigned)n_prob), dim3(step_waves * WAVE), step_lds, c->stream,
                               (int)it, (const int64_t*)B.seg_off, P->variant, P->kind, P->max_spk, P->lambdac,
                               P->threshold, B.ld, B.aux, B.mat, (const int64_t*)B.mat_off, Q, d_a, d_b, d_merge_d,
                               B.smax, B.smin, c->d_err, c->pinv_cur);
        }
        hipLaunchKernelGGL(k_step_final, dim3((unsigned)n_prob), dim3(AHC_TPB), 0, c->stream,
                           (int)(n_max - 1), (const int64_t*)B.seg_off, (const double*)B.mat, (const int64_t*)B.mat_off,
                           Q, d_n, d_fmax, d_fmin);
    }
    HIPCHK(c, hipGetLastError());
    HIPCHK(c, hipMemcpyAsync(h_n_merges, d_n, (size_t)n_prob * sizeof(int32_t), hipMemcpyDeviceToHost, c->stream));
    HIPCHK(c, hipMemcpyAsync(h_merge_a, d_a, (size_t)n_total * sizeof(int32_t), hipMemcpyDeviceToHost, c->stream));
    HIPCHK(c, hipMemcpyAsync(h_merge_b, d_b, (size_t)n_total * sizeof(int32_t), hipMemcpyDeviceToHost, c->stream));
    HIPCHK(c, hipMemcpyAsync(h_merge_d, d_merge_d, (size_t)n_total * sizeof(double), hipMemcpyDeviceToHost, c->stream));
    HIPCHK(c, hipMemcpyAsync(kmax.data(), B.smax, (size_t)n_prob * sizeof(unsigned long long), hipMemcpyDeviceToHost, c->stream));
    HIPCHK(c, hipMemcpyAsync(kmin.data(), B.smin, (size_t)n_prob * sizeof(unsigned long long), hipMemcpyDeviceToHost, c->stream));
    HIPCHK(c, hipMemcpyAsync(fmax.data(), d_fmax, (size_t)n_prob * sizeof(double), hipMemcpyDeviceToHost, c->stream));
    HIPCHK(c, hipMemcpyAsync(fmin.data(), d_fmin, (size_t)n_prob * sizeof(double), hipMemcpyDeviceToHost, c->stream));
    const spkd_status st = call.finish();
    for (int64_t p = 0; p < n_prob; ++p) {
        if (P->variant == 1) {
            h_stat_max[p] = key_to_double(kmax[(size_t)p], true);
            h_stat_min[p] = key_to_double(kmin[(size_t)p], false);
        } else {
            h_stat_max[p] = fmax[(size_t)p];
            h_stat_min[p] = fmin[(size_t)p];
        }
    }
    return st;
}
}

spkd_status spkd_ahc(spkd_ctx* c, const double* d_stats, const int64_t* h_seg_off, int64_t n_prob,
                     const spkd_ahc_params* P, int32_t* h_n_merges, int32_t* h_merge_a,
                     int32_t* h_merge_b, double* h_merge_d, double* h_stat_max, double* h_stat_min) {
    return ahc_impl(c, d_stats, h_seg_off, n_prob, P, MatrixPlan(), h_n_merges, h_merge_a, h_merge_b, h_merge_d,
                    h_stat_max, h_stat_min);
}

spkd_status spkd_ahc_matrix(spkd_ctx* c, const double* d_stats, int64_t n, const spkd_ahc_params* P,
                            const double* d_matrix, double stat_max_in, double stat_min_in,
                            int32_t* h_n_merges, int32_t* h_merge_a, int32_t* h_merge_b, double* h_merge_d,
                            double* h_stat_max, double* h_stat_min) {
    if (!c || n < 1) return SPKD_EINVAL;
    if (!d_matrix) return fail(c, SPKD_EINVAL, "ahc_matrix: null matrix");
    const int64_t seg_off[2] = {0, n};
    MatrixPlan plan;
    plan.d_init = d_matrix;
    plan.init_max = stat_max_in;
    plan.init_min = stat_min_in;
    return ahc_impl(c, d_stats, seg_off, 1, P, plan, h_n_merges, h_merge_a, h_merge_b, h_merge_d, h_stat_max, h_stat_min);
}

int64_t spkd_gw_event_capacity(int64_t turn_len, double rate) {
    if (turn_len < 0 || !(rate >= 10.0)) return -1;
    return (int64_t)((double)turn_len / (0.2 * rate)) + 8;
}

int64_t spkd_gw_event_capacity_p(int64_t turn_len, const spkd_cd_params* P) {
    if (turn_len < 0 || !P || !(P->rate >= 10.0) || !(P->winstep >= 1.0)) return -1;
    const double step = std::min(0.2 * P->rate, std::min(0.5 * P->rate, P->winstep));
    return (int64_t)((double)turn_len / step) + 8;
}

int64_t spkd_sw_window_count(int64_t turn_len, double winsize, double winstep) {
    if (!(winstep >= 1.0) || !(winsize >= 1.0)) return -1;
    int64_t w = 0;
    for (double s = 0; s + 2 * winsize <= (double)turn_len; s += winstep) ++w;
    return w;
}

namespace {
spkd_status build_turns(spkd_ctx* c, int64_t n_frames, const int64_t* hb, const int64_t* he, int64_t n_turns,
                        const spkd_cd_params* P, const int64_t* h_off, bool gw, std::vector<TurnDesc>& turns,
                        int64_t& n_cand) {
    n_cand = 0;
    turns.resize((size_t)n_turns);
    for (int64_t t = 0; t < n_turns; ++t) {
        if (hb[t] < 0 || he[t] < hb[t] || he[t] > n_frames) return fail(c, SPKD_EINVAL, "bad turn range");
        TurnDesc& T = turns[(size_t)t];
        T.begin = hb[t];
        T.len = he[t] - hb[t];
        T.cand_off = n_cand;
        T.cand_cap = gw ? (int64_t)((double)T.len / (P->rate / 10)) + (int64_t)(2 * (P->rate / 10)) + 16 : 0;
        n_cand += T.cand_cap;
        T.ev_off = h_off[t];
        T.ev_cap = h_off[t + 1] - h_off[t];
        T.id = t;
        if (T.ev_cap < 0) return fail(c, SPKD_EINVAL, "offsets must be non-decreasing");
    }
    if (gw) std::stable_sort(turns.begin(), turns.end(), [](const TurnDesc& a, const TurnDesc& b) { return a.len > b.len; });
    return SPKD_OK;
}

struct GwBatch {
    const double *turn_start_s, *turn_end_s;
    const int64_t *file_off, *file_len;
    int want_index;
    spkd_gw_lines_view* view;
    double *d_ls = nullptr, *d_le = nullptr;
    int64_t* d_line_off = nullptr;
    int32_t *d_n_det = nullptr, *d_pos = nullptr;
    int64_t* h_head = nullptr;
    int32_t* h_n_win = nullptr;
    int64_t n_lines = 0;
    bool have_lines = false;
};

spkd_status gw_batch_upload(spkd_ctx* c, GwBatch& G, int64_t n_turns) {
    const size_t nt = (size_t)n_turns;
    TRY(carve(c, scratch, S_CP_TURNS, [&](Layout L) {
        return L.part(G.d_ls, nt).part(G.d_le, nt).part(G.d_line_off, nt + 1).part(G.d_n_det, nt).part(G.d_pos, nt).bytes();
    }));
    HIPCHK(c, hipMemcpyAsync(G.d_ls, G.turn_start_s, nt * sizeof(double), hipMemcpyHostToDevice, c->stream));
    HIPCHK(c, hipMemcpyAsync(G.d_le, G.turn_end_s, nt * sizeof(double), hipMemcpyHostToDevice, c->stream));
    return carve(c, pinned, PIN_GW_TURNS, [&](Layout L) { return L.part(G.h_head, 2).part(G.h_n_win, nt).bytes(); });
}

struct GwEvents {
    int32_t* n_win = nullptr;
    double* win_maxd = nullptr;
    int32_t* win_det = nullptr;
    double *det_start = nullptr, *det_maxi = nullptr, *det_d = nullptr, *final_start = nullptr;
};

struct LineArrays {
    int64_t* frame;
    int64_t* index;
    int32_t* turn;
    Layout& parts(Layout& L, size_t n) { return L.part(frame, 2 * n).part(index, n).part(turn, n); }
};

spkd_status gw_batch_compact(spkd_ctx* c, GwBatch& G, const TurnDesc* d_turns, int64_t n_turns, const GwEvents& ev,
                             double rate) {
    const unsigned blocks = (unsigned)((n_turns + CP_TPB - 1) / CP_TPB);
    hipLaunchKernelGGL(k_cp_count, dim3(blocks), dim3(CP_TPB), 0, c->stream, d_turns, n_turns, (const int32_t*)ev.n_win,
                       (const int32_t*)ev.win_det, (const int*)c->d_err, G.d_n_det, G.d_pos);
    hipLaunchKernelGGL(k_cp_scan, dim3(1), dim3(CP_SCAN_TPB), 0, c->stream, (const int32_t*)G.d_n_det, n_turns,
                       (const int*)c->d_err, G.d_line_off);
    HIPCHK(c, hipGetLastError());
    G.h_head[0] = 0;
    G.h_head[1] = 0;
    HIPCHK(c, hipMemcpyAsync(&G.h_head[0], G.d_line_off + n_turns, sizeof(int64_t), hipMemcpyDeviceToHost, c->stream));
    HIPCHK(c, hipMemcpyAsync(&G.h_head[1], c->d_err, sizeof(int), hipMemcpyDeviceToHost, c->stream));
    HIPCHK(c, hipMemcpyAsync(G.h_n_win, ev.n_win, (size_t)n_turns * sizeof(int32_t), hipMemcpyDeviceToHost, c->stream));
    HIPCHK(c, hipStreamSynchronize(c->stream));
    if (G.h_head[1] != 0) return SPKD_OK;
    const int64_t n = G.h_head[0];
    if (n < n_turns) return fail(c, SPKD_EHIP, "internal error: fewer lines than turns");
    const size_t nn = (size_t)n;
    void* d_t = nullptr;
    LineArrays D, H;
    double* h_times;
    TRY(scratch(c, S_CP_TIMES, nn * 2 * sizeof(double), &d_t));
    TRY(carve(c, scratch, S_CP_LINES, [&](Layout L) { return D.parts(L, nn).bytes(); }));
    TRY(carve(c, pinned, PIN_GW_LINES, [&](Layout L) { return H.parts(L.part(h_times, 2 * nn), nn).bytes(); }));
    hipLaunchKernelGGL(k_cp_lines, dim3(blocks), dim3(CP_TPB), 0, c->stream, d_turns, n_turns,
                       (const int32_t*)G.d_n_det, (const int32_t*)G.d_pos, (const int64_t*)G.d_line_off, n,
                       (const double*)ev.det_start, (const double*)ev.det_maxi, (const double*)ev.final_start,
                       (const double*)G.d_ls, (const double*)G.d_le, rate,
                       (const int*)c->d_err, (double*)d_t, D.frame, D.frame + nn, D.index, D.turn);
    HIPCHK(c, hipGetLastError());
    HIPCHK(c, hipMemcpyAsync(h_times, d_t, nn * 2 * sizeof(double), hipMemcpyDeviceToHost, c->stream));
    HIPCHK(c, hipMemcpyAsync(H.frame, D.frame, nn * 2 * sizeof(int64_t), hipMemcpyDeviceToHost, c->stream));
    HIPCHK(c, hipMemcpyAsync(H.turn, D.turn, nn * sizeof(int32_t), hipMemcpyDeviceToHost, c->stream));
    if (G.want_index)
        HIPCHK(c, hipMemcpyAsync(H.index, D.index, nn * sizeof(int64_t), hipMemcpyDeviceToHost, c->stream));
    spkd_gw_lines_view& V = *G.view;
    V.n_lines = n;
    V.n_win = G.h_n_win;
    V.times = h_times;
    V.turn = H.turn;
    V.frame_b = H.frame;
    V.frame_e = H.frame + nn;
    V.index = G.want_index ? H.index : nullptr;
    V.d_index = D.index;
    G.n_lines = n;
    G.have_lines = true;
    return SPKD_OK;
}

spkd_status gw_batch_finish(spkd_ctx* c, GwBatch& G, int64_t n_turns, double rate) {
    spkd_gw_lines_view& V = *G.view;
    double* times = const_cast<double*>(V.times);
    spkd_py2_roundtrip(times, 2 * V.n_lines);
    c->redo_line.clear();
    c->redo_begin.clear();
    c->redo_end.clear();
    for (int64_t i = 0; i < V.n_lines; ++i) {
        const int64_t t = V.turn[i];
        if (t < 0 || t >= n_turns) return fail(c, SPKD_EHIP, "internal error: line of no turn");
        const int64_t fn = G.file_len[t];
        int64_t a0 = (int64_t)(times[2 * i] * rate), a1 = (int64_t)(times[2 * i + 1] * rate);
        a0 = a0 < 0 ? 0 : (a0 > fn ? fn : a0);
        a1 = a1 < 0 ? 0 : (a1 > fn ? fn : a1);
        if (a1 < a0) a1 = a0;
        const int64_t b = G.file_off[t] + a0, e = G.file_off[t] + a1;
        if (b != V.frame_b[i] || e != V.frame_e[i]) {
            c->redo_line.push_back(i);
            c->redo_begin.push_back(b);
            c->redo_end.push_back(e);
        }
    }
    V.n_redo = (int64_t)c->redo_line.size();
    V.redo_line = c->redo_line.data();
    V.redo_begin = c->redo_begin.data();
    V.redo_end = c->redo_end.data();
    return SPKD_OK;
}

struct GwIn {
    const float* d_frames = nullptr;
    int64_t n_frames = 0, n_turns = 0;
    const int64_t *hb = nullptr, *he = nullptr, *h_ev_off = nullptr;
    const spkd_cd_params* P = nullptr;
    int check_capacity = 0;
    double* d_seg_stats = nullptr;
};
struct GwOut {
    int32_t *h_n_win = nullptr, *h_win_det = nullptr;
    double *h_win_maxd = nullptr, *h_det_start = nullptr, *h_det_maxi = nullptr, *h_det_d = nullptr,
           *h_final_start = nullptr;
    spkd_cand_log* h_log = nullptr;
    int64_t log_cap = 0;
    int64_t* h_log_count = nullptr;
};

struct GwEventArray { int slot; size_t elem; bool per_turn; size_t dev, host; };
#define SPKD_EV(SLOT, T, per_turn, name) {SLOT, sizeof(T), per_turn, offsetof(GwEvents, name), offsetof(GwOut, h_##name)}
const GwEventArray GW_EVENT_ARRAYS[] = {
    SPKD_EV(S_GW_N_WIN, int32_t, true, n_win),
    SPKD_EV(S_GW_WIN_MAXD, double, false, win_maxd),
    SPKD_EV(S_GW_WIN_DET, int32_t, false, win_det),
    SPKD_EV(S_GW_DET_START, double, false, det_start),
    SPKD_EV(S_GW_DET_MAXI, double, false, det_maxi),
    SPKD_EV(S_GW_DET_D, double, false, det_d),
    SPKD_EV(S_GW_FINAL_START, double, true, final_start),
};
#undef SPKD_EV
void* get_pointer(const void* s, size_t off) { void* p; std::memcpy(&p, (const char*)s + off, sizeof p); return p; }
void set_pointer(void* s, size_t off, void* p) { std::memcpy((char*)s + off, &p, sizeof p); }

constexpr int64_t GW_WAVE_PER_TURN_FROM = 4096;
constexpr int64_t GW_EIGHT_WAVES_UP_TO = 256;
spkd_status gw_impl(spkd_ctx* c, const GwIn& in, const GwOut& out, GwBatch* batch = nullptr) {
    const int64_t n_turns = in.n_turns, log_cap = out.log_cap;
    const spkd_cd_params* P = in.P;
    if (!c || !P || n_turns < 0) return SPKD_EINVAL;
    if (out.h_log_count) *out.h_log_count = 0;
    if (n_turns == 0) return SPKD_OK;
    if (!in.d_frames || !in.hb || !in.he || !in.h_ev_off) return fail(c, SPKD_EINVAL, "null argument");
    for (const GwEventArray& a : GW_EVENT_ARRAYS)
        if (!batch && !get_pointer(&out, a.host)) return fail(c, SPKD_EINVAL, "null argument");
    if (bad_kind(P->kind)) return fail(c, SPKD_EINVAL, "gw: bad kind");
    if (!(P->rate >= 10.0) || !(P->winsize >= 1.0) || !(P->winstep >= 1.0))
        return fail(c, SPKD_EINVAL, "gw: rate >= 10, winsize >= 1 frame and winstep >= 1 frame required");
    if (log_cap < 0 || (log_cap > 0 && !out.h_log)) return fail(c, SPKD_EINVAL, "gw: log capacity without a log buffer");
    if (!c->gw_lds_ok) return fail(c, SPKD_EHIP, "gw: the kernel's dynamic LDS size was not admitted on this device");
    std::vector<TurnDesc> turns;
    int64_t n_cand;
    TRY(build_turns(c, in.n_frames, in.hb, in.he, n_turns, P, in.h_ev_off, true, turns, n_cand));
    for (int64_t t = 0; in.check_capacity && t < n_turns; ++t)
        if (turns[(size_t)t].ev_cap < spkd_gw_event_capacity_p(turns[(size_t)t].len, P))
            return fail(c, SPKD_EINVAL, "gw: event capacity too small, see spkd_gw_event_capacity_p");
    unsigned long long cnt2[2] = {0ull, 0ull};
    Call call(c);
    TRY(call.opened);
    spkd_cd_params Pk;
    TRY(kernel_params(c, P, Pk));
    const int64_t n_ev = in.h_ev_off[n_turns];
    TurnDesc* d_turns = nullptr;
    void *d_snap = nullptr, *d_cand = nullptr, *d_log = nullptr;
    GwEvents ev;
    TRY(upload(c, S_TURNS, turns.data(), turns.size(), &d_turns));
    TRY(scratch(c, S_SNAP, (size_t)n_cand * REC * sizeof(double), &d_snap));
    TRY(scratch(c, S_CAND, (size_t)n_cand * 4 * sizeof(double), &d_cand));
    auto ev_bytes = [&](const GwEventArray& a) { return (size_t)(a.per_turn ? n_turns : n_ev) * a.elem; };
    bool missing = false;
    for (const GwEventArray& a : GW_EVENT_ARRAYS) {
        void* p = nullptr;
        TRY(scratch(c, a.slot, ev_bytes(a), &p));
        set_pointer(&ev, a.dev, p);
        missing = missing || !p;
    }
    TRY(scratch(c, S_LOG, (size_t)std::max<int64_t>(log_cap, 1) * sizeof(spkd_cand_log), &d_log));
    if (missing || !d_turns || !d_snap || !d_cand || !d_log || !c->d_counter || !c->d_err)
        return fail(c, SPKD_EHIP, "gw: a device scratch buffer is missing");
    HIPCHK(c, hipMemsetAsync(c->d_counter, 0, 2 * sizeof(unsigned long long), c->stream));
    if (batch) TRY(gw_batch_upload(c, *batch, n_turns));
    int nw = c->gw_waves;
    if (nw != 1 && nw != 2 && nw != 4 && nw != 8)
        nw = n_turns >= GW_WAVE_PER_TURN_FROM ? 1 : (n_turns <= GW_EIGHT_WAVES_UP_TO ? 8 : 4);
#define SPKD_GW_LAUNCH(NW_)                                                                                     \
    hipLaunchKernelGGL(k_gw<NW_>, dim3((unsigned)n_turns), dim3(Gw<NW_>::TPB), Gw<NW_>::LDS_BYTES, c->stream, \
                       in.d_frames, (const TurnDesc*)d_turns, *P, (double*)d_snap, (double*)d_cand,            \
                       ev.n_win, ev.win_maxd, ev.win_det, ev.det_start, ev.det_maxi, ev.det_d, ev.final_start,  \
                       in.d_seg_stats, (spkd_cand_log*)d_log, (long long)log_cap, c->d_counter, c->d_err,      \
                       c->pinv_cur)
    {
        Timer t(c, SPKD_T_GW);
        if (nw == 1) SPKD_GW_LAUNCH(1); else if (nw == 2) SPKD_GW_LAUNCH(2);
        else if (nw == 8) SPKD_GW_LAUNCH(8); else SPKD_GW_LAUNCH(4);
    }
#undef SPKD_GW_LAUNCH
    HIPCHK(c, hipGetLastError());
    unsigned long long& cnt = cnt2[0];
    if (batch) {
        TRY(gw_batch_compact(c, *batch, d_turns, n_turns, ev, P->rate));
        HIPCHK(c, hipMemcpyAsync(cnt2, c->d_counter, sizeof cnt2, hipMemcpyDeviceToHost, c->stream));
        const spkd_status st = call.finish();
        c->last_gw_items = (int64_t)cnt2[1];
        if (st != SPKD_OK) return st;
        if (!batch->have_lines) return fail(c, SPKD_EHIP, "internal error: no lines from a clean call");
        return gw_batch_finish(c, *batch, n_turns, P->rate);
    }
    for (const GwEventArray& a : GW_EVENT_ARRAYS)
        HIPCHK(c, hipMemcpyAsync(get_pointer(&out, a.host), get_pointer(&ev, a.dev), ev_bytes(a), hipMemcpyDeviceToHost,
                                 c->stream));
    HIPCHK(c, hipMemcpyAsync(cnt2, c->d_counter, sizeof cnt2, hipMemcpyDeviceToHost, c->stream));
    const spkd_status st = call.finish();
    c->last_gw_items = (int64_t)cnt2[1];
    if (out.h_log_count) *out.h_log_count = (int64_t)cnt;
    if (out.h_log && log_cap > 0 && cnt > 0) {
        const size_t ncopy = (size_t)std::min<int64_t>((int64_t)cnt, log_cap);
        HIPCHK(c, hipMemcpy(out.h_log, d_log, ncopy * sizeof(spkd_cand_log), hipMemcpyDeviceToHost));
    }
    if (st == SPKD_OK && (int64_t)cnt > log_cap && out.h_log)
        return fail(c, SPKD_EOVERFLOW, "candidate log too small");
    return st;
}

spkd_status gw_to_host(spkd_ctx* c, const float* d_frames, int64_t n_frames, const int64_t* hb,
                       const int64_t* he, int64_t n_turns, const spkd_cd_params* P, const int64_t* h_ev_off,
                       int check_capacity, int32_t* h_n_win, double* h_win_maxd, int32_t* h_win_det,
                       double* h_det_start, double* h_det_maxi, double* h_det_d, double* h_final_start,
                       double* d_seg_stats, spkd_cand_log* h_log, int64_t log_cap, int64_t* h_log_count) {
    GwIn in;
    in.d_frames = d_frames; in.n_frames = n_frames; in.hb = hb; in.he = he; in.n_turns = n_turns;
    in.P = P; in.h_ev_off = h_ev_off; in.check_capacity = check_capacity; in.d_seg_stats = d_seg_stats;
    GwOut out;
    out.h_n_win = h_n_win; out.h_win_maxd = h_win_maxd; out.h_win_det = h_win_det; out.h_det_start = h_det_start;
    out.h_det_maxi = h_det_maxi; out.h_det_d = h_det_d; out.h_final_start = h_final_start;
    out.h_log = h_log; out.log_cap = log_cap; out.h_log_count = h_log_count;
    return gw_impl(c, in, out);
}
}

spkd_status spkd_gw(spkd_ctx* c, const float* d_frames, int64_t n_frames, const int64_t* hb,
                    const int64_t* he, int64_t n_turns, const spkd_cd_params* P, const int64_t* h_ev_off,
                    int32_t* h_n_win, double* h_win_maxd, int32_t* h_win_det, double* h_det_start,
                    double* h_det_maxi, double* h_det_d, double* h_final_start, spkd_cand_log* h_log,
                    int64_t log_cap, int64_t* h_log_count) {
    return gw_to_host(c, d_frames, n_frames, hb, he, n_turns, P, h_ev_off, 1, h_n_win, h_win_maxd, h_win_det,
                      h_det_start, h_det_maxi, h_det_d, h_final_start, nullptr, h_log, log_cap, h_log_count);
}

spkd_status spkd_gw_ex(spkd_ctx* c, const float* d_frames, int64_t n_frames, const int64_t* hb,
                       const int64_t* he, int64_t n_turns, const spkd_cd_params* P, const int64_t* h_ev_off,
                       int check_capacity, int32_t* h_n_win, double* h_win_maxd, int32_t* h_win_det,
                       double* h_det_start, double* h_det_maxi, double* h_det_d, double* h_final_start,
                       spkd_cand_log* h_log, int64_t log_cap, int64_t* h_log_count) {
    return gw_to_host(c, d_frames, n_frames, hb, he, n_turns, P, h_ev_off, check_capacity, h_n_win, h_win_maxd,
                      h_win_det, h_det_start, h_det_maxi, h_det_d, h_final_start, nullptr, h_log, log_cap, h_log_count);
}

spkd_status spkd_gw_fused(spkd_ctx* c, const float* d_frames, int64_t n_frames, const int64_t* hb,
                          const int64_t* he, int64_t n_turns, const spkd_cd_params* P, const int64_t* h_ev_off,
                          int check_capacity, int32_t* h_n_win, double* h_win_maxd, int32_t* h_win_det,
                          double* h_det_start, double* h_det_maxi, double* h_det_d, double* h_final_start,
                          double* d_seg_stats, spkd_cand_log* h_log, int64_t log_cap, int64_t* h_log_count) {
    if (c && !d_seg_stats) return fail(c, SPKD_EINVAL, "gw_fused: null statistics buffer");
    return gw_to_host(c, d_frames, n_frames, hb, he, n_turns, P, h_ev_off, check_capacity, h_n_win, h_win_maxd,
                      h_win_det, h_det_start, h_det_maxi, h_det_d, h_final_start, d_seg_stats, h_log, log_cap,
                      h_log_count);
}

spkd_status spkd_gw_batch(spkd_ctx* c, const float* d_frames, int64_t n_frames, const int64_t* hb,
                          const int64_t* he, int64_t n_turns, const spkd_cd_params* P, const int64_t* h_ev_off,
                          const double* h_turn_start_s, const double* h_turn_end_s, const int64_t* h_turn_file_off,
                          const int64_t* h_turn_file_len, double* d_seg_stats, int want_index,
                          spkd_gw_lines_view* view) {
    if (!c || !view) return SPKD_EINVAL;
    std::memset(view, 0, sizeof *view);
    if (!d_seg_stats) return fail(c, SPKD_EINVAL, "gw_batch: null statistics buffer");
    if (n_turns > 0 && (!h_turn_start_s || !h_turn_end_s || !h_turn_file_off || !h_turn_file_len))
        return fail(c, SPKD_EINVAL, "gw_batch: null turn arrays");
    GwBatch G;
    G.turn_start_s = h_turn_start_s;
    G.turn_end_s = h_turn_end_s;
    G.file_off = h_turn_file_off;
    G.file_len = h_turn_file_len;
    G.want_index = want_index;
    G.view = view;
    GwIn in;
    in.d_frames = d_frames; in.n_frames = n_frames; in.hb = hb; in.he = he; in.n_turns = n_turns;
    in.P = P; in.h_ev_off = h_ev_off; in.d_seg_stats = d_seg_stats;
    const spkd_status st = gw_impl(c, in, GwOut(), &G);
    if (st != SPKD_OK) std::memset(view, 0, sizeof *view);
    return st;
}

spkd_status spkd_ahc_fused(spkd_ctx* c, const float* d_frames, int64_t n_frames, const double* d_records,
                           int64_t n_records, int64_t* d_line_index, const int64_t* h_seg_off, int64_t n_prob,
                           const int64_t* h_redo_line, const int64_t* h_redo_begin, const int64_t* h_redo_end,
                           int64_t n_redo, const spkd_ahc_params* P, const int32_t** h_n_merges,
                           const int32_t** h_merge_a, const int32_t** h_merge_b, const double** h_merge_d,
                           const int32_t** h_labels) {
    if (!c || !P || n_prob < 0 || n_redo < 0) return SPKD_EINVAL;
    if (!h_n_merges || !h_merge_a || !h_merge_b || !h_merge_d || !h_labels)
        return fail(c, SPKD_EINVAL, "ahc_fused: null output");
    *h_n_merges = *h_merge_a = *h_merge_b = *h_labels = nullptr;
    *h_merge_d = nullptr;
    if (n_prob == 0) return SPKD_OK;
    if (!d_records || !d_line_index || !h_seg_off || n_records < 1 || h_seg_off[0] != 0)
        return fail(c, SPKD_EINVAL, "ahc_fused: null argument or first offset not 0");
    for (int64_t p = 0; p < n_prob; ++p)
        if (h_seg_off[p + 1] < h_seg_off[p]) return fail(c, SPKD_EINVAL, "seg_off must be non-decreasing");
    const int64_t n_total = h_seg_off[n_prob];
    if (n_redo > 0 && (!h_redo_line || !h_redo_begin || !h_redo_end || !d_frames))
        return fail(c, SPKD_EINVAL, "ahc_fused: null redo arrays");
    for (int64_t k = 0; k < n_redo; ++k)
        if (h_redo_line[k] < 0 || h_redo_line[k] >= n_total || (k > 0 && h_redo_line[k] <= h_redo_line[k - 1]))
            return fail(c, SPKD_EINVAL, "ahc_fused: redo lines must be ascending line indices");
    const size_t nt = (size_t)n_total, np = (size_t)n_prob;
    double *md, *smax, *smin;
    int32_t *ma, *mb, *lab, *nm;
    TRY(carve(c, pinned, PIN_AHC_OUT, [&](Layout L) {
        return L.part(md, nt).part(smax, np).part(smin, np).part(ma, nt).part(mb, nt).part(lab, nt).part(nm, np).bytes();
    }));
    MatrixPlan plan;
    plan.d_map = d_line_index;
    plan.n_src = n_records;
    plan.d_frames = d_frames;
    plan.n_frames = n_frames;
    plan.redo_line = h_redo_line;
    plan.redo_begin = h_redo_begin;
    plan.redo_end = h_redo_end;
    plan.n_redo = n_redo;
    TRY(ahc_impl(c, d_records, h_seg_off, n_prob, P, plan, nm, ma, mb, md, smax, smin));
    if (spkd_labels_from_merges_batch(n_prob, h_seg_off, nm, ma, mb, lab) != SPKD_OK)
        return fail(c, SPKD_EHIP, "internal error: merge log does not replay");
    *h_n_merges = nm;
    *h_merge_a = ma;
    *h_merge_b = mb;
    *h_merge_d = md;
    *h_labels = lab;
    return SPKD_OK;
}

spkd_status spkd_gather_stats(spkd_ctx* c, const double* d_src, int64_t n_src, const int64_t* h_src_index,
                              const int64_t* h_dst_index, int64_t n, int64_t n_dst, double* d_dst) {
    if (!c || n < 0) return SPKD_EINVAL;
    if (n == 0) return SPKD_OK;
    if (!d_src || !h_src_index || !d_dst) return fail(c, SPKD_EINVAL, "null argument");
    for (int64_t i = 0; i < n; ++i) {
        if (h_src_index[i] < 0 || h_src_index[i] >= n_src) return fail(c, SPKD_EINVAL, "gather: source index out of range");
        const int64_t d = h_dst_index ? h_dst_index[i] : i;
        if (d < 0 || d >= n_dst) return fail(c, SPKD_EINVAL, "gather: destination index out of range");
    }
    Call call(c);
    TRY(call.opened);
    int64_t *d_si = nullptr, *d_di = nullptr;
    TRY(upload(c, S_IDXA, h_src_index, (size_t)n, &d_si));
    if (h_dst_index) TRY(upload(c, S_IDXB, h_dst_index, (size_t)n, &d_di));
    hipLaunchKernelGGL(k_gather_records, dim3((unsigned)n), dim3(256), 0, c->stream, d_src,
                       (const int64_t*)d_si, (const int64_t*)d_di, n, d_dst);
    HIPCHK(c, hipGetLastError());
    return call.finish();
}

spkd_status spkd_sw(spkd_ctx* c, const float* d_frames, int64_t n_frames, const int64_t* hb,
                    const int64_t* he, int64_t n_turns, const spkd_cd_params* P, const int64_t* h_d_off,
                    double* h_d) {
    if (!c || !P || n_turns < 0) return SPKD_EINVAL;
    if (n_turns == 0) return SPKD_OK;
    if (!d_frames || !hb || !he || !h_d_off || !h_d) return fail(c, SPKD_EINVAL, "null argument");
    if (bad_kind(P->kind)) return fail(c, SPKD_EINVAL, "bad kind");
    if (!(P->winsize >= 1.0) || !(P->winstep >= 1.0)) return fail(c, SPKD_EINVAL, "sw: window and step must be >= 1 frame");
    const int64_t n_d = h_d_off[n_turns];
    std::vector<int64_t> rb, re;
    std::vector<int32_t> rs;
    rb.reserve((size_t)(2 * n_d)); re.reserve((size_t)(2 * n_d)); rs.reserve((size_t)(2 * n_d));
    const int64_t wsz = (int64_t)P->winsize;
    for (int64_t t = 0; t < n_turns; ++t) {
        if (hb[t] < 0 || he[t] < hb[t] || he[t] > n_frames) return fail(c, SPKD_EINVAL, "bad turn range");
        const int64_t len = he[t] - hb[t];
        const int64_t W = spkd_sw_window_count(len, P->winsize, P->winstep);
        if (h_d_off[t + 1] - h_d_off[t] != W) return fail(c, SPKD_EINVAL, "sw: offsets do not match spkd_sw_window_count");
        for (int64_t w = 0; w < W; ++w) {
            const int64_t a = hb[t] + (int64_t)((double)w * P->winstep);
            const int32_t s0 = (int32_t)(2 * (h_d_off[t] + w));
            rb.push_back(a); re.push_back(a + wsz); rs.push_back(s0);
            rb.push_back(a + wsz); re.push_back(a + 2 * wsz); rs.push_back(s0 + 1);
        }
    }
    if (n_d == 0) return SPKD_OK;
    if (2 * n_d > 0x7fffffffLL) return fail(c, SPKD_EINVAL, "sw: too many windows in one call");
    std::vector<Chunk> chunks;
    std::vector<int64_t> set_off;
    AhcPrep B;
    Call call(c);
    TRY(call.opened);
    spkd_cd_params Pk;
    TRY(kernel_params(c, P, Pk));
    void *d_rec = nullptr, *d_out = nullptr;
    TRY(scratch(c, S_SNAP, (size_t)(2 * n_d) * REC * sizeof(double), &d_rec));
    TRY(scratch(c, S_GW_WIN_MAXD, (size_t)n_d * sizeof(double), &d_out));
    {
        Timer t(c, SPKD_T_SW);
        TRY(set_stats_launch(c, d_frames, n_frames, rb.data(), re.data(), rs.data(), 2 * n_d, 2 * n_d, (double*)d_rec,
                             chunks, set_off));
        std::vector<int64_t> seg_off((size_t)n_d + 1);
        for (int64_t w = 0; w <= n_d; ++w) seg_off[(size_t)w] = 2 * w;
        TRY(ahc_prepare(c, (const double*)d_rec, seg_off.data(), n_d, 1, P->kind, P->lambdac, B));
        hipLaunchKernelGGL(k_take_pair_distance, dim3((unsigned)((n_d + 255) / 256)), dim3(256), 0, c->stream,
                           (const double*)B.mat, n_d, (double*)d_out);
    }
    HIPCHK(c, hipGetLastError());
    HIPCHK(c, hipMemcpyAsync(h_d, d_out, (size_t)n_d * sizeof(double), hipMemcpyDeviceToHost, c->stream));
    return call.finish();
}

spkd_status spkd_mfcc(spkd_ctx* c, const int16_t* d_pcm, int64_t n_samples, const spkd_mfcc_params* P,
                      const float* h_melfb, const float* h_dct, const float* h_mean, const float* h_scale,
                      const float* h_transform, float* d_features, int64_t* h_n_frames) {
    if (!c || !P || !h_n_frames) return SPKD_EINVAL;
    *h_n_frames = 0;
    if (n_samples < 0 || !h_melfb || !h_dct || !h_mean || !h_scale || !h_transform)
        return fail(c, SPKD_EINVAL, "mfcc: null argument");
    if ((P->window_width != MF_WIN && P->window_width != MF_WIN_VAD) || P->n_fft != MF_NFFT || P->n_mel != MF_MEL ||
        P->n_cep != MF_CEP || P->frame_rate <= 0 || P->sample_rate <= 0 || P->sample_rate % P->frame_rate != 0)
        return fail(c, SPKD_EINVAL, "mfcc: this build does 400- or 256-sample windows, a 512-point transform, 21 mel bins, 12 cepstra");
    if (P->cms_left < 0 || P->cms_right < 0 || P->cms_left + P->cms_right > 1024 || P->delta_width[0] < 1 ||
        P->delta_width[0] > 2 || P->delta_width[1] < 1 || P->delta_width[1] > 2 || !(P->delta_norm[0] > 0.f) ||
        !(P->delta_norm[1] > 0.f))
        return fail(c, SPKD_EINVAL, "mfcc: unsupported mean-subtraction window or delta parameters");
    const int hop = P->sample_rate / P->frame_rate;
    if (hop < 1) return fail(c, SPKD_EINVAL, "mfcc: frame rate above the sample rate");
    const int span = MP_FR + 2 * MP_HALO;
    const size_t lds = (size_t)((span + P->cms_left + P->cms_right) * MF_STATIC + 2 * span * MF_STATIC +
                                MP_FR * MF_DIM + MF_DIM * MF_DIM) * sizeof(float);
    if (lds > 60 * 1024) return fail(c, SPKD_EINVAL, "mfcc: mean-subtraction window too wide for the LDS tile");
    const int64_t T = n_samples / hop;
    *h_n_frames = T;
    if (T == 0) return SPKD_OK;
    if (!d_pcm || !d_features) return fail(c, SPKD_EINVAL, "mfcc: null device buffer");
    float *d_fb, *d_dct, *d_mean, *d_scale, *d_tr;
    std::vector<char> tab;
    Call call(c);
    TRY(call.opened);
    void* d_static = nullptr;
    TRY(upload_parts(c, S_MFCC_TAB, tab, [&](Layout L) {
        return L.part(d_fb, MF_MEL * MF_BINS, h_melfb).part(d_dct, MF_CEP * MF_MEL, h_dct).part(d_mean, MF_DIM, h_mean)
            .part(d_scale, MF_DIM, h_scale).part(d_tr, MF_DIM * MF_DIM, h_transform).bytes();
    }));
    TRY(scratch(c, S_MFCC_STATIC, (size_t)T * MF_STATIC * sizeof(float), &d_static));
    if (P->window_width == MF_WIN)
        hipLaunchKernelGGL(k_mfcc_static<MF_WIN>, dim3((unsigned)((T + MF_FR - 1) / MF_FR)), dim3(MF_TPB), 0, c->stream,
                           d_pcm, (long long)n_samples, (long long)T, hop, P->pre_emph, d_fb, d_dct, (float*)d_static);
    else
        hipLaunchKernelGGL(k_mfcc_static<MF_WIN_VAD>, dim3((unsigned)((T + MF_FR - 1) / MF_FR)), dim3(MF_TPB), 0,
                           c->stream, d_pcm, (long long)n_samples, (long long)T, hop, P->pre_emph, d_fb, d_dct,
                           (float*)d_static);
    hipLaunchKernelGGL(k_mfcc_post, dim3((unsigned)((T + MP_FR - 1) / MP_FR)), dim3(MF_TPB), lds, c->stream,
                       (const float*)d_static, (long long)T, P->cms_left, P->cms_right, P->delta_width[0],
                       P->delta_norm[0], P->delta_width[1], P->delta_norm[1], d_mean, d_scale, d_tr, d_features);
    if (hipGetLastError() != hipSuccess) return fail(c, SPKD_EHIP, "mfcc: kernel launch failed");
    return call.finish();
}

spkd_status spkd_gmm_loglik(spkd_ctx* c, const float* d_features, int64_t n_frames, const spkd_gmm_params* P,
                            float* d_scores) {
    if (!c || !P) return SPKD_EINVAL;
    const int K = P->n_kernels, S = P->n_states;
    if (P->dim != GM_DIM || K < 1 || K > GM_MAX_K || S < 1 || S > GM_MAX_S || n_frames < 0)
        return fail(c, SPKD_EINVAL, "gmm_loglik: dim must be 39, 1 <= kernels <= 256, 1 <= states <= 16");
    if (!P->mean || !P->inv_var || !P->log_norm || !P->state_off || !P->kernel || !P->log_weight)
        return fail(c, SPKD_EINVAL, "gmm_loglik: null model array");
    if (P->state_off[0] != 0) return fail(c, SPKD_EINVAL, "gmm_loglik: state_off[0] must be 0");
    for (int s = 0; s < S; ++s)
        if (P->state_off[s + 1] < P->state_off[s] || P->state_off[s + 1] - P->state_off[s] > K)
            return fail(c, SPKD_EINVAL, "gmm_loglik: state_off must be non-decreasing, at most 256 kernels a state");
    const int nnz = P->state_off[S];
    for (int j = 0; j < nnz; ++j) {
        const float lw = P->log_weight[j];
        if (P->kernel[j] < 0 || P->kernel[j] >= K || std::isnan(lw) || lw == INFINITY)
            return fail(c, SPKD_EINVAL, "gmm_loglik: kernel index out of range or log weight NaN / +inf");
    }
    for (int64_t i = 0; i < (int64_t)K * GM_DIM; ++i)
        if (!std::isfinite(P->mean[i]) || !std::isfinite(P->inv_var[i]) || !(P->inv_var[i] > 0.f))
            return fail(c, SPKD_EINVAL, "gmm_loglik: means must be finite, inverse variances finite and positive");
    for (int k = 0; k < K; ++k)
        if (!std::isfinite(P->log_norm[k])) return fail(c, SPKD_EINVAL, "gmm_loglik: non-finite normalising constant");
    if (n_frames == 0) return SPKD_OK;
    if (!d_features || !d_scores) return fail(c, SPKD_EINVAL, "gmm_loglik: null device buffer");
    const int64_t n_blocks = (n_frames + GM_TPB - 1) / GM_TPB;
    if (n_blocks > 0x7fffffffLL) return fail(c, SPKD_EINVAL, "gmm_loglik: too many frames in one call");
    float *d_mean, *d_iv, *d_c, *d_lw;
    int32_t *d_state_off, *d_kernel;
    std::vector<char> tab, idx;
    Call call(c);
    TRY(call.opened);
    TRY(upload_parts(c, S_GMM_TAB, tab, [&](Layout L) {
        return L.part(d_mean, (size_t)K * GM_DIM, P->mean).part(d_iv, (size_t)K * GM_DIM, P->inv_var)
            .part(d_c, (size_t)K, P->log_norm).part(d_lw, (size_t)nnz, P->log_weight).bytes();
    }));
    TRY(upload_parts(c, S_GMM_IDX, idx, [&](Layout L) {
        return L.part(d_state_off, (size_t)S + 1, P->state_off).part(d_kernel, (size_t)nnz, P->kernel).bytes();
    }));
    hipLaunchKernelGGL(k_gmm_loglik, dim3((unsigned)n_blocks), dim3(GM_TPB), 0, c->stream, d_features,
                       (long long)n_frames, d_mean, d_iv, d_c, (const int*)d_state_off, (const int*)d_kernel, d_lw,
                       S, d_scores);
    if (hipGetLastError() != hipSuccess) return fail(c, SPKD_EHIP, "gmm_loglik: kernel launch failed");
    return call.finish();
}

static const double kPow10[23] = {1e0, 1e1, 1e2, 1e3, 1e4, 1e5, 1e6, 1e7, 1e8, 1e9, 1e10, 1e11,
                                  1e12, 1e13, 1e14, 1e15, 1e16, 1e17, 1e18, 1e19, 1e20, 1e21, 1e22};
static const uint64_t kPow10u[20] = {1ull, 10ull, 100ull, 1000ull, 10000ull, 100000ull, 1000000ull,
                                     10000000ull, 100000000ull, 1000000000ull, 10000000000ull,
                                     100000000000ull, 1000000000000ull, 10000000000000ull,
                                     100000000000000ull, 1000000000000000ull, 10000000000000000ull,
                                     100000000000000000ull, 1000000000000000000ull,
                                     10000000000000000000ull};

static bool roundtrip_fast(double x, double* out) {
    if (!(x >= 1e-3 && x < 1e11)) return false;
    int e10 = (int)std::floor(std::log10(x));
    if (e10 < -3) e10 = -3;
    if (e10 >= 0) { if (x < kPow10[e10]) --e10; else if (e10 + 1 <= 22 && x >= kPow10[e10 + 1]) ++e10; }
    else { if (x * kPow10[-e10] < 1.0) --e10; else if (x * kPow10[-e10 - 1] >= 1.0) ++e10; }
    if (e10 < -3 || e10 > 10) return false;
    int s = 11 - e10;
    int k;
    const double fr = std::frexp(x, &k);
    const uint64_t m = (uint64_t)std::ldexp(fr, 53);
    k -= 53;
    unsigned __int128 prod = (unsigned __int128)m * kPow10u[s];
    uint64_t q;
    if (k >= 0) {
        if (k > 20) return false;
        q = (uint64_t)(prod << k);
    } else {
        const int sh = -k;
        if (sh >= 120) return false;
        const unsigned __int128 one = 1;
        const unsigned __int128 fl = prod >> sh;
        const unsigned __int128 remn = prod & ((one << sh) - 1);
        const unsigned __int128 half = one << (sh - 1);
        q = (uint64_t)fl;
        if (remn > half || (remn == half && (q & 1))) ++q;
    }
    if (q >= 1000000000000ull) {
        if (q != 1000000000000ull) return false;
        q = 100000000000ull;
        s -= 1;
    } else if (q < 100000000000ull) {
        return false;
    }
    *out = s >= 0 ? (double)q / kPow10[s] : (double)q * kPow10[-s];
    return true;
}

static void roundtrip_range(double* v, int64_t lo, int64_t hi) {
    char buf[64];
    for (int64_t i = lo; i < hi; ++i) {
        double r;
        if (roundtrip_fast(v[i], &r)) { v[i] = r; continue; }
        std::snprintf(buf, sizeof buf, "%.12g", v[i]);
        v[i] = std::strtod(buf, nullptr);
    }
}

void spkd_py2_roundtrip(double* v, int64_t n) {
    const int64_t kMinPerThread = 8192;
    int nthreads = (int)std::min<int64_t>(8, n / kMinPerThread);
    if (nthreads <= 1) { roundtrip_range(v, 0, n); return; }
    std::vector<std::thread> pool;
    const int64_t step = (n + nthreads - 1) / nthreads;
    for (int t = 0; t < nthreads; ++t) {
        const int64_t lo = t * step, hi = std::min<int64_t>(n, lo + step);
        if (lo < hi) pool.emplace_back(roundtrip_range, v, lo, hi);
    }
    for (auto& th : pool) th.join();
}

spkd_status spkd_labels_from_merges(int64_t n, int64_t n_merges, const int32_t* h_a, const int32_t* h_b,
                                    int32_t* h_labels) {
    if (n < 0 || n_merges < 0 || (n > 0 && !h_labels) || (n_merges > 0 && (!h_a || !h_b))) return SPKD_EINVAL;
    std::vector<int32_t> ids((size_t)n), parent((size_t)n);
    for (int64_t i = 0; i < n; ++i) ids[(size_t)i] = parent[(size_t)i] = (int32_t)i;
    int64_t m = n;
    for (int64_t k = 0; k < n_merges; ++k) {
        const int32_t a = h_a[k], b = h_b[k];
        if (a < 0 || b <= a || b >= m) return SPKD_EINVAL;
        parent[(size_t)ids[(size_t)b]] = ids[(size_t)a];
        ids.erase(ids.begin() + b);
        --m;
    }
    std::vector<int32_t> where((size_t)n, -1);
    for (int64_t p = 0; p < m; ++p) where[(size_t)ids[(size_t)p]] = (int32_t)p;
    for (int64_t i = 0; i < n; ++i) {
        int32_t r = (int32_t)i;
        while (parent[(size_t)r] != r) r = parent[(size_t)r];
        int32_t c = (int32_t)i;
        while (parent[(size_t)c] != r) { const int32_t nx = parent[(size_t)c]; parent[(size_t)c] = r; c = nx; }
        h_labels[i] = where[(size_t)r] + 1;
    }
    return SPKD_OK;
}

spkd_status spkd_count_flags(const int32_t* h_flags, const int64_t* h_off, const int32_t* h_n, int64_t n_groups,
                             int32_t* h_out) {
    if (n_groups < 0 || (n_groups > 0 && (!h_flags || !h_off || !h_n || !h_out))) return SPKD_EINVAL;
    for (int64_t g = 0; g < n_groups; ++g) {
        if (h_n[g] < 0 || h_off[g] < 0) return SPKD_EINVAL;
        h_out[g] = count_detections(h_flags + h_off[g], h_n[g]);
    }
    return SPKD_OK;
}

spkd_status spkd_gw_lines(int64_t n_turns, const int64_t* h_off, const int32_t* h_n_det, const double* h_det_start,
                          const double* h_det_maxi, const double* h_final_start, const double* h_turn_start_s,
                          const double* h_turn_end_s, const int64_t* h_turn_begin, const int64_t* h_turn_end,
                          double rate, int text_contract, int64_t n_lines, double* h_times, int64_t* h_frame_b,
                          int64_t* h_frame_e, int64_t* h_index, int32_t* h_line_turn) {
    if (n_turns < 0 || n_lines < 0) return SPKD_EINVAL;
    if (n_turns > 0 && (!h_off || !h_n_det || !h_det_start || !h_det_maxi || !h_final_start || !h_turn_start_s ||
                        !h_turn_end_s || !h_turn_begin || !h_turn_end || !h_times))
        return SPKD_EINVAL;
    int64_t i = 0;
    for (int64_t t = 0; t < n_turns; ++t) {
        const int64_t nd = h_n_det[t];
        if (nd < 0 || i + nd + 1 > n_lines) return SPKD_EINVAL;
        const double ls = h_turn_start_s[t], le = h_turn_end_s[t];
        for (int64_t j = 0; j <= nd; ++j, ++i) {
            const RecipeLine L = recipe_line(h_turn_begin[t], h_turn_end[t] - h_turn_begin[t], h_off[t], j, nd,
                                             h_det_start, h_det_maxi, h_final_start + t, ls, le, rate);
            h_times[2 * i] = L.start_s;
            h_times[2 * i + 1] = L.end_s;
            if (h_frame_b) h_frame_b[i] = L.frame_b;
            if (h_frame_e) h_frame_e[i] = L.frame_e;
            if (h_index) h_index[i] = L.index;
            if (h_line_turn) h_line_turn[i] = (int32_t)t;
        }
    }
    if (i != n_lines) return SPKD_EINVAL;
    if (text_contract) spkd_py2_roundtrip(h_times, 2 * n_lines);
    return SPKD_OK;
}

spkd_status spkd_vad_viterbi(int64_t n_frames, int32_t n_states, const float* h_scores, int32_t n_words,
                             const int32_t* h_word_state, const double* h_stay, const double* h_exit,
                             const double* h_enter, int64_t* h_tok_frame, int32_t* h_tok_word, int64_t* h_n_tokens,
                             double* h_score) {
    if (!h_n_tokens || !h_score || n_frames < 0 || n_states < 1 || n_states > GM_MAX_S || n_words < 1 ||
        n_words > GM_MAX_S || !h_word_state || !h_stay || !h_exit || !h_enter)
        return SPKD_EINVAL;
    *h_n_tokens = 0;
    *h_score = -INFINITY;
    for (int32_t j = 0; j < n_words; ++j)
        if (h_word_state[j] < 0 || h_word_state[j] >= n_states) return SPKD_EINVAL;
    if (n_frames == 0) return SPKD_OK;
    if (!h_scores || !h_tok_frame || !h_tok_word) return SPKD_EINVAL;
    const int W = n_words;
    std::vector<int8_t> back((size_t)n_frames * W);
    double d[GM_MAX_S], nd[GM_MAX_S], obs[GM_MAX_S];
    for (int64_t t = 0; t < n_frames; ++t) {
        bool all_ninf = true;
        for (int j = 0; j < W; ++j) {
            const double o = (double)h_scores[t * n_states + h_word_state[j]];
            obs[j] = std::isnan(o) ? -INFINITY : o;
            all_ninf = all_ninf && obs[j] == -INFINITY;
        }
        if (all_ninf)
            for (int j = 0; j < W; ++j) obs[j] = 0.0;
        if (t == 0) {
            for (int j = 0; j < W; ++j) { d[j] = h_enter[j] + obs[j]; back[(size_t)j] = -1; }
            continue;
        }
        double best = d[0] + h_exit[0];
        int bi = 0;
        for (int i = 1; i < W; ++i) {
            const double v = d[i] + h_exit[i];
            if (v > best) { best = v; bi = i; }
        }
        for (int j = 0; j < W; ++j) {
            const double stay = d[j] + h_stay[j], sw = best + h_enter[j];
            int8_t& b = back[(size_t)t * W + j];
            if (stay >= sw) { nd[j] = stay + obs[j]; b = -1; }
            else { nd[j] = sw + obs[j]; b = (int8_t)bi; }
        }
        for (int j = 0; j < W; ++j) d[j] = nd[j];
    }
    int j = 0;
    for (int i = 1; i < W; ++i)
        if (d[i] > d[j]) j = i;
    *h_score = d[j];
    int64_t n = 0;
    for (int64_t t = n_frames - 1; t >= 0; --t) {
        const int8_t b = back[(size_t)t * W + j];
        if (t == 0 || b >= 0) { h_tok_frame[n] = t; h_tok_word[n] = j; ++n; }
        if (t > 0 && b >= 0) j = b;
    }
    std::reverse(h_tok_frame, h_tok_frame + n);
    std::reverse(h_tok_word, h_tok_word + n);
    *h_n_tokens = n;
    return SPKD_OK;
}

spkd_status spkd_labels_from_merges_batch(int64_t n_problems, const int64_t* h_seg_off, const int32_t* h_n_merges,
                                          const int32_t* h_a, const int32_t* h_b, int32_t* h_labels) {
    if (n_problems < 0 || (n_problems > 0 && (!h_seg_off || !h_n_merges || !h_a || !h_b || !h_labels)))
        return SPKD_EINVAL;
    std::atomic<int> bad{0};
    auto work = [&](int64_t lo, int64_t hi) {
        for (int64_t p = lo; p < hi; ++p) {
            const int64_t o = h_seg_off[p];
            if (spkd_labels_from_merges(h_seg_off[p + 1] - o, h_n_merges[p], h_a + o, h_b + o, h_labels + o) != SPKD_OK)
                bad.store(1);
        }
    };
    const int nthreads = (int)std::min<int64_t>(8, n_problems / 16);
    if (nthreads <= 1) {
        work(0, n_problems);
    } else {
        std::vector<std::thread> pool;
        const int64_t step = (n_problems + nthreads - 1) / nthreads;
        for (int t = 0; t < nthreads; ++t) {
            const int64_t lo = t * step, hi = std::min<int64_t>(n_problems, lo + step);
            if (lo < hi) pool.emplace_back(work, lo, hi);
        }
        for (auto& th : pool) th.join();
    }
    return bad.load() ? SPKD_EINVAL : SPKD_OK;
}

}

#ifdef SPKD_PROFILE
extern "C" int spkd_debug_ahc_prof(unsigned long long* out4) {
    unsigned long long z[8] = {0, 0, 0, 0, 0, 0, 0, 0};
    if (hipMemcpyFromSymbol(out4, HIP_SYMBOL(spkd::g_ahc_prof), sizeof z) != hipSuccess) return 1;
    if (hipMemcpyToSymbol(HIP_SYMBOL(spkd::g_ahc_prof), z, sizeof z) != hipSuccess) return 1;
    return 0;
}

extern "C" int spkd_debug_step_prof(unsigned long long* out8) {
    unsigned long long z[8] = {0, 0, 0, 0, 0, 0, 0, 0};
    if (hipMemcpyFromSymbol(out8, HIP_SYMBOL(spkd::g_step_prof), sizeof z) != hipSuccess) return 1;
    if (hipMemcpyToSymbol(HIP_SYMBOL(spkd::g_step_prof), z, sizeof z) != hipSuccess) return 1;
    return 0;
}

extern "C" int spkd_debug_pass_prof(unsigned long long* out4) {
    unsigned long long z[4] = {0, 0, 0, 0};
    if (hipMemcpyFromSymbol(out4, HIP_SYMBOL(spkd::g_pass_prof), sizeof z) != hipSuccess) return 1;
    if (hipMemcpyToSymbol(HIP_SYMBOL(spkd::g_pass_prof), z, sizeof z) != hipSuccess) return 1;
    return 0;
}

extern "C" int spkd_debug_gw_prof(unsigned long long* out12) {
    unsigned long long z[12] = {0, 0, 0, 0, 0, 0, 0, 0, 0, 0, 0, 0};
    if (hipMemcpyFromSymbol(out12, HIP_SYMBOL(spkd::g_gw_prof), sizeof z) != hipSuccess) return 1;
    if (hipMemcpyToSymbol(HIP_SYMBOL(spkd::g_gw_prof), z, sizeof z) != hipSuccess) return 1;
    return 0;
}
#endif
```

speaker-diarization_amd/hipabi.py:

```python
import ctypes as C
import os

import numpy as np

HERE = os.path.dirname(os.path.abspath(__file__))
LIB_PATH = os.environ.get('SPKD_HIP_LIBRARY') or os.path.join(HERE, 'csrc', 'libspkd_hip.so')

SPKD_OK, SPKD_EINVAL, SPKD_EHIP, SPKD_ENONFINITE, SPKD_EOVERFLOW, SPKD_ENOMEM = range(6)
KINDS = {'BIC': 0, 'GLR': 1, 'KL2': 2, 'KL2P': 3}
WANT_GLR, WANT_KL2, WANT_KL2_PINV = 1, 2, 4
TIMERS = {n: i for i, n in enumerate(['call', 'chunk_stats', 'reduce_sets', 'pair_terms',
                                        'cluster_prep', 'matrix', 'ahc', 'gw', 'sw'])}
REC = 820
DIM = 39

EXPORTS = ['spkd_abi_version', 'spkd_create', 'spkd_create_on_stream', 'spkd_destroy', 'spkd_last_error', 'spkd_sync',
           'spkd_malloc', 'spkd_free', 'spkd_memcpy_h2d', 'spkd_memcpy_d2h', 'spkd_memcpy_d2d',
           'spkd_last_kernel_ms', 'spkd_last_gw_items', 'spkd_set_stats', 'spkd_pair_terms',
           'spkd_distance_matrix', 'spkd_gw_event_capacity', 'spkd_gw_event_capacity_p', 'spkd_gw', 'spkd_gw_ex', 'spkd_gw_fused', 'spkd_gw_batch', 'spkd_ahc_fused', 'spkd_gather_stats', 'spkd_mfcc',
           'spkd_sw_window_count', 'spkd_sw', 'spkd_ahc', 'spkd_ahc_matrix', 'spkd_distance_rows', 'spkd_cluster_in', 'spkd_py2_roundtrip',
           'spkd_labels_from_merges', 'spkd_labels_from_merges_batch', 'spkd_count_flags', 'spkd_gw_lines',
           'spkd_gmm_loglik', 'spkd_vad_viterbi']


class CdParams(C.Structure):
    _fields_ = [('kind', C.c_int32), ('trace', C.c_int32), ('lambdac', C.c_double),
                ('threshold', C.c_double), ('winsize', C.c_double), ('winstep', C.c_double),
                ('deltaws', C.c_double), ('rate', C.c_double)]


class CandLog(C.Structure):
    _fields_ = [('turn', C.c_int32), ('coarse', C.c_int32), ('seq', C.c_int64),
                ('start', C.c_double), ('i', C.c_double), ('d', C.c_double),
                ('n1', C.c_int64), ('n2', C.c_int64)]


class GwLinesView(C.Structure):
    _fields_ = [('n_lines', C.c_int64), ('n_redo', C.c_int64), ('n_win', C.c_void_p), ('times', C.c_void_p),
                ('turn', C.c_void_p), ('frame_b', C.c_void_p), ('frame_e', C.c_void_p), ('index', C.c_void_p),
                ('d_index', C.c_void_p), ('redo_line', C.c_void_p), ('redo_begin', C.c_void_p),
                ('redo_end', C.c_void_p)]


AHC_AUTO, AHC_MONO, AHC_WIDE = 0, 1, 2


class MfccParams(C.Structure):
    _fields_ = [('sample_rate', C.c_int32), ('frame_rate', C.c_int32), ('window_width', C.c_int32),
                ('n_fft', C.c_int32), ('n_mel', C.c_int32), ('n_cep', C.c_int32), ('cms_left', C.c_int32),
                ('cms_right', C.c_int32), ('delta_width', C.c_int32 * 2), ('pre_emph', C.c_float),
                ('delta_norm', C.c_float * 2)]


class GmmParams(C.Structure):
    _fields_ = [('n_kernels', C.c_int32), ('n_states', C.c_int32), ('dim', C.c_int32), ('mean', C.c_void_p),
                ('inv_var', C.c_void_p), ('log_norm', C.c_void_p), ('state_off', C.c_void_p), ('kernel', C.c_void_p),
                ('log_weight', C.c_void_p)]


class AhcParams(C.Structure):
    _fields_ = [('variant', C.c_int32), ('kind', C.c_int32), ('max_spk', C.c_int32),
                ('path', C.c_int32), ('lambdac', C.c_double), ('threshold', C.c_double)]


class SpkdError(RuntimeError):
    def __init__(self, status, text):
        RuntimeError.__init__(self, 'spkd status %d: %s' % (status, text))
        self.status = status


_lib = None


def _one_hip_runtime():
    import sys
    if 'torch' in sys.modules or os.environ.get('SPKD_SYSTEM_HIP'):
        return
    try:
        import importlib.util
        spec = importlib.util.find_spec('torch')
        where = list(spec.submodule_search_locations)[0] if spec and spec.submodule_search_locations else None
    except (ImportError, ValueError, AttributeError):
        where = None
    if where:
        rt = os.path.join(where, 'lib', 'libamdhip64.so')
        if os.path.exists(rt):
            try:
                C.CDLL(rt, mode=C.RTLD_GLOBAL)
            except OSError:
                pass


def mapped_hip_runtimes():
    found = set()
    try:
        with open('/proc/self/maps') as f:
            for line in f:
                path = line.rsplit(None, 1)[-1] if '/' in line else ''
                if os.path.basename(path).startswith('libamdhip64.so'):
                    found.add(os.path.realpath(path))
    except OSError:
        pass
    return sorted(found)


def _check_one_runtime():
    rts = mapped_hip_runtimes()
    if len(rts) > 1:
        raise ImportError('two HIP runtimes are mapped into this process (%s): libspkd_hip.so and the PyTorch '
                          'wheel link against different libamdhip64 sonames.  Set SPKD_SYSTEM_HIP=1 for a '
                          'torch-free process, or import torch before this package.' % ', '.join(rts))


def load_library(path=None):
    global _lib
    if _lib is not None and path is None:
        return _lib
    p = path or LIB_PATH
    if not os.path.exists(p):
        raise ImportError('HIP extension %s is not built: run `python -c "import __graft_entry__ as g; '
                          'g.build()"` (or make -C speaker-diarization_amd/csrc)' % p)
    _one_hip_runtime()
    lib = C.CDLL(p)
    _check_one_runtime()
    vp, i64, i32, dbl = C.c_void_p, C.c_int64, C.c_int32, C.c_double
    P = C.POINTER
    lib.spkd_abi_version.restype = C.c_int
    lib.spkd_create.argtypes = [C.c_int, vp, P(vp)]
    lib.spkd_create_on_stream.argtypes = [C.c_int, vp, P(vp)]
    lib.spkd_destroy.argtypes = [vp]
    lib.spkd_destroy.restype = None
    lib.spkd_last_error.argtypes = [vp]
    lib.spkd_last_error.restype = C.c_char_p
    lib.spkd_sync.argtypes = [vp]
    lib.spkd_malloc.argtypes = [vp, C.c_size_t, P(vp)]
    lib.spkd_free.argtypes = [vp, vp]
    lib.spkd_memcpy_h2d.argtypes = [vp, vp, vp, C.c_size_t]
    lib.spkd_memcpy_d2h.argtypes = [vp, vp, vp, C.c_size_t]
    lib.spkd_memcpy_d2d.argtypes = [vp, vp, vp, C.c_size_t]
    lib.spkd_last_kernel_ms.argtypes = [vp, C.c_int, P(C.c_float)]
    lib.spkd_last_gw_items.argtypes = [vp, P(C.c_int64)]
    lib.spkd_set_stats.argtypes = [vp, vp, i64, vp, vp, vp, i64, i64, vp]
    lib.spkd_pair_terms.argtypes = [vp, vp, vp, vp, i64, C.c_int, vp]
    lib.spkd_distance_matrix.argtypes = [vp, C.c_int, dbl, vp, i64, vp]
    lib.spkd_gw_event_capacity.argtypes = [i64, dbl]
    lib.spkd_gw_event_capacity.restype = i64
    lib.spkd_gw_event_capacity_p.argtypes = [i64, P(CdParams)]
    lib.spkd_gw_event_capacity_p.restype = i64
    lib.spkd_gw.argtypes = [vp, vp, i64, vp, vp, i64, P(CdParams), vp, vp, vp, vp, vp, vp, vp, vp,
                            vp, i64, P(i64)]
    lib.spkd_gw_ex.argtypes = [vp, vp, i64, vp, vp, i64, P(CdParams), vp, C.c_int, vp, vp, vp, vp, vp, vp,
                               vp, vp, i64, P(i64)]
    lib.spkd_gw_fused.argtypes = [vp, vp, i64, vp, vp, i64, P(CdParams), vp, C.c_int, vp, vp, vp, vp, vp, vp,
                                  vp, vp, vp, i64, P(i64)]
    lib.spkd_gw_batch.argtypes = [vp, vp, i64, vp, vp, i64, P(CdParams), vp, vp, vp, vp, vp, vp, C.c_int, P(GwLinesView)]
    lib.spkd_ahc_fused.argtypes = [vp, vp, i64, vp, i64, vp, vp, i64, vp, vp, vp, i64, P(AhcParams),
                                   P(vp), P(vp), P(vp), P(vp), P(vp)]
    lib.spkd_gather_stats.argtypes = [vp, vp, i64, vp, vp, i64, i64, vp]
    lib.spkd_mfcc.argtypes = [vp, vp, i64, P(MfccParams), vp, vp, vp, vp, vp, vp, P(i64)]
    lib.spkd_sw_window_count.argtypes = [i64, dbl, dbl]
    lib.spkd_sw_window_count.restype = i64
    lib.spkd_sw.argtypes = [vp, vp, i64, vp, vp, i64, P(CdParams), vp, vp]
    lib.spkd_ahc.argtypes = [vp, vp, vp, i64, P(AhcParams), vp, vp, vp, vp, vp, vp]
    lib.spkd_ahc_matrix.argtypes = [vp, vp, i64, P(AhcParams), vp, dbl, dbl, vp, vp, vp, vp, vp, vp]
    lib.spkd_distance_rows.argtypes = [vp, C.c_int, C.c_int, dbl, vp, i64, i64, i64, vp, P(dbl), P(dbl)]
    lib.spkd_cluster_in.argtypes = [vp, vp, i64, C.c_int, dbl, dbl, vp, vp, i64, vp, P(i64), P(i64)]
    lib.spkd_py2_roundtrip.argtypes = [vp, i64]
    lib.spkd_py2_roundtrip.restype = None
    lib.spkd_labels_from_merges.argtypes = [i64, i64, vp, vp, vp]
    lib.spkd_labels_from_merges_batch.argtypes = [i64, vp, vp, vp, vp, vp]
    lib.spkd_count_flags.argtypes = [vp, vp, vp, i64, vp]
    lib.spkd_gmm_loglik.argtypes = [vp, vp, i64, P(GmmParams), vp]
    lib.spkd_vad_viterbi.argtypes = [i64, i32, vp, i32, vp, vp, vp, vp, vp, vp, P(i64), P(dbl)]
    lib.spkd_gw_lines.argtypes = [i64, vp, vp, vp, vp, vp, vp, vp, vp, vp, dbl, C.c_int, i64, vp, vp, vp, vp, vp]
    if lib.spkd_abi_version() != 2:
        raise ImportError('libspkd_hip.so ABI version mismatch')
    if path is None:
        _lib = lib
    return lib


def _ptr(a):
    return a.ctypes.data_as(C.c_void_p)


def _view(addr, n, dtype):
    if not addr or n <= 0:
        return np.zeros(0, dtype=dtype)
    ct = {np.int32: C.c_int32, np.int64: C.c_int64, np.float64: C.c_double}[dtype]
    return np.ctypeslib.as_array(C.cast(C.c_void_p(addr), C.POINTER(ct)), shape=(int(n),))


def py2_roundtrip(values):
    v = np.ascontiguousarray(values, dtype=np.float64).copy()
    if v.size:
        load_library().spkd_py2_roundtrip(_ptr(v), v.size)
    return v


def labels_from_merges(n, a, b):
    a = np.ascontiguousarray(a, dtype=np.int32)
    b = np.ascontiguousarray(b, dtype=np.int32)
    out = np.zeros(n, dtype=np.int32)
    st = load_library().spkd_labels_from_merges(n, len(a), _ptr(a), _ptr(b), _ptr(out))
    if st != SPKD_OK:
        raise SpkdError(st, 'bad merge log')
    return out


def count_flags(flags, off, n):
    flags = np.ascontiguousarray(flags, dtype=np.int32)
    off = np.ascontiguousarray(off, dtype=np.int64)
    n = np.ascontiguousarray(n, dtype=np.int32)
    if len(off) != len(n):
        raise SpkdError(SPKD_EINVAL, 'one offset per group')
    if len(n) and (int((off + n).max()) > len(flags) or int(n.min()) < 0 or int(off.min()) < 0):
        raise SpkdError(SPKD_EINVAL, 'flag ranges outside the array')
    out = np.zeros(len(n), dtype=np.int32)
    st = load_library().spkd_count_flags(_ptr(flags), _ptr(off), _ptr(n), len(n), _ptr(out))
    if st != SPKD_OK:
        raise SpkdError(st, 'bad flag ranges')
    return out


def gw_lines(off, n_det, det_start, det_maxi, final_start, turn_start_s, turn_end_s, turn_begin, turn_end,
             rate, text_contract=True, want_frames=False):
    c = np.ascontiguousarray
    off = c(off, dtype=np.int64); n_det = c(n_det, dtype=np.int32)
    nt = len(n_det)
    arrs = [c(det_start, dtype=np.float64), c(det_maxi, dtype=np.float64), c(final_start, dtype=np.float64),
            c(turn_start_s, dtype=np.float64), c(turn_end_s, dtype=np.float64), c(turn_begin, dtype=np.int64),
            c(turn_end, dtype=np.int64)]
    if len(off) != nt or any(len(a) != nt for a in arrs[2:]):
        raise SpkdError(SPKD_EINVAL, 'one entry per turn')
    if nt and (int(n_det.min()) < 0 or int(off.min()) < 0 or int((off + n_det).max()) > min(len(arrs[0]), len(arrs[1]))):
        raise SpkdError(SPKD_EINVAL, 'detections outside the event arrays')
    n_lines = int(n_det.sum(dtype=np.int64)) + nt
    times = np.empty((n_lines, 2), dtype=np.float64)
    turn = np.empty(n_lines, dtype=np.int32)
    fb = np.empty(n_lines, dtype=np.int64) if want_frames else None
    fe = np.empty(n_lines, dtype=np.int64) if want_frames else None
    ix = np.empty(n_lines, dtype=np.int64) if want_frames else None
    p = lambda a: _ptr(a) if a is not None else None
    st = load_library().spkd_gw_lines(nt, _ptr(off), _ptr(n_det), *[_ptr(a) for a in arrs], float(rate),
                                      1 if text_contract else 0, n_lines, _ptr(times), p(fb), p(fe), p(ix), _ptr(turn))
    if st != SPKD_OK:
        raise SpkdError(st, 'bad growing-window result')
    return {'times': times, 'turn': turn, 'frame_b': fb, 'frame_e': fe, 'index': ix}


def vad_viterbi(scores, word_state, stay, exit_, enter):
    c = np.ascontiguousarray
    scores = c(scores, dtype=np.float32)
    if scores.ndim != 2:
        raise SpkdError(SPKD_EINVAL, 'scores must be [frames, states]')
    ws = c(word_state, dtype=np.int32)
    consts = [c(a, dtype=np.float64) for a in (stay, exit_, enter)]
    if any(len(a) != len(ws) for a in consts):
        raise SpkdError(SPKD_EINVAL, 'one constant of each kind per word')
    T, S = scores.shape
    tf = np.zeros(max(T, 1), dtype=np.int64)
    tw = np.zeros(max(T, 1), dtype=np.int32)
    n = C.c_int64(0)
    sc = C.c_double(0.0)
    st = load_library().spkd_vad_viterbi(T, S, _ptr(scores), len(ws), _ptr(ws), *[_ptr(a) for a in consts],
                                         _ptr(tf), _ptr(tw), C.byref(n), C.byref(sc))
    if st != SPKD_OK:
        raise SpkdError(st, 'bad decoder input')
    return tf[:n.value].copy(), tw[:n.value].copy(), sc.value


def labels_from_merges_batch(seg_off, n_merges, a, b):
    seg_off = np.ascontiguousarray(seg_off, dtype=np.int64)
    n_merges = np.ascontiguousarray(n_merges, dtype=np.int32)
    a = np.ascontiguousarray(a, dtype=np.int32)
    b = np.ascontiguousarray(b, dtype=np.int32)
    out = np.zeros(int(seg_off[-1]), dtype=np.int32)
    st = load_library().spkd_labels_from_merges_batch(len(seg_off) - 1, _ptr(seg_off), _ptr(n_merges),
                                                      _ptr(a), _ptr(b), _ptr(out))
    if st != SPKD_OK:
        raise SpkdError(st, 'bad merge log')
    return out


def _gw_capacity_ladder(turn_len, params, tight, first_guess_scale):
    if not (params.rate >= 10.0 and params.winstep >= 1.0):
        raise SpkdError(SPKD_EINVAL, 'unsupported growing-window parameters (frame rate >= 10 and '
                                     'a window step of at least one frame needed)')
    step = min(0.2 * params.rate, 0.5 * params.rate, params.winstep)
    full = (turn_len.astype(np.float64) / step).astype(np.int64) + 8
    if first_guess_scale != 1.0:
        full = np.maximum((full * float(first_guess_scale)).astype(np.int64), 2)
    grow = 1
    while True:
        caps = (full // 4 + 8) if tight else full * grow
        off = np.zeros(len(full) + 1, dtype=np.int64)
        off[1:] = np.cumsum(caps)
        yield off
        if tight:
            tight = False
        elif grow < 1024:
            grow *= 2
        else:
            return


class Context(object):

    def __init__(self, device=0, stream=None):
        self.lib = load_library()
        h = C.c_void_p()
        if stream is None:
            st = self.lib.spkd_create(int(device), None, C.byref(h))
        else:
            st = self.lib.spkd_create_on_stream(int(device), C.c_void_p(int(stream)), C.byref(h))
        if st != SPKD_OK:
            raise SpkdError(st, 'spkd_create failed (no usable HIP device %d?)' % device)
        self.h = h
        self.device = device

    def close(self):
        if getattr(self, 'h', None):
            for ptr, _ in self.__dict__.pop('_dev_scratch', {}).values():
                self.lib.spkd_free(self.h, C.c_void_p(ptr))
            self.lib.spkd_destroy(self.h)
            self.h = None

    def __del__(self):
        try:
            self.close()
        except Exception:
            pass

    def check(self, st, allow=()):
        if st != SPKD_OK and st not in allow:
            raise SpkdError(st, self.lib.spkd_last_error(self.h).decode())
        return st

    def last_ms(self, which='call'):
        ms = C.c_float()
        self.check(self.lib.spkd_last_kernel_ms(self.h, TIMERS[which], C.byref(ms)))
        return ms.value

    def last_gw_items(self):
        n = C.c_int64()
        self.check(self.lib.spkd_last_gw_items(self.h, C.byref(n)))
        return int(n.value)

    def dev_alloc(self, nbytes):
        p = C.c_void_p()
        self.check(self.lib.spkd_malloc(self.h, nbytes, C.byref(p)))
        return p.value

    def dev_free(self, ptr):
        if ptr:
            self.check(self.lib.spkd_free(self.h, C.c_void_p(ptr)))

    def dev_scratch(self, name, nbytes):
        cache = self.__dict__.setdefault('_dev_scratch', {})
        ptr, cap = cache.get(name, (None, 0))
        if ptr is None or cap < nbytes:
            if ptr is not None:
                self.dev_free(ptr)
            ptr, cap = self.dev_alloc(nbytes), nbytes
            cache[name] = (ptr, cap)
        return ptr

    def h2d(self, dptr, arr):
        arr = np.ascontiguousarray(arr)
        self.check(self.lib.spkd_memcpy_h2d(self.h, C.c_void_p(dptr), _ptr(arr), arr.nbytes))

    def copy_d2d(self, d_dst, d_src, nbytes):
        self.check(self.lib.spkd_memcpy_d2d(self.h, C.c_void_p(d_dst), C.c_void_p(d_src), int(nbytes)))

    def d2h(self, arr, dptr):
        assert arr.flags['C_CONTIGUOUS']
        self.check(self.lib.spkd_memcpy_d2h(self.h, _ptr(arr), C.c_void_p(dptr), arr.nbytes))

    def set_stats(self, d_frames, n_frames, begins, ends, sets, n_sets, d_stats):
        b = np.ascontiguousarray(begins, dtype=np.int64)
        e = np.ascontiguousarray(ends, dtype=np.int64)
        s = np.ascontiguousarray(sets, dtype=np.int32)
        self.check(self.lib.spkd_set_stats(self.h, C.c_void_p(d_frames), n_frames, _ptr(b), _ptr(e),
                                           _ptr(s), len(b), n_sets, C.c_void_p(d_stats)))

    def pair_terms(self, d_stats, ia, ib, flags=0):
        ia = np.ascontiguousarray(ia, dtype=np.int32)
        ib = np.ascontiguousarray(ib, dtype=np.int32)
        out = np.empty((len(ia), 8), dtype=np.float64)
        st = self.lib.spkd_pair_terms(self.h, C.c_void_p(d_stats), _ptr(ia), _ptr(ib), len(ia),
                                      flags, _ptr(out))
        self.check(st, allow=(SPKD_ENONFINITE,))
        return out, st

    def distance_matrix(self, kind, lambdac, d_stats, n, d_matrix):
        st = self.lib.spkd_distance_matrix(self.h, KINDS[kind], lambdac, C.c_void_p(d_stats), n,
                                           C.c_void_p(d_matrix))
        return self.check(st, allow=(SPKD_ENONFINITE,))

    def _buf(self, name, n, dtype):
        cache = self.__dict__.setdefault('_bufs', {})
        arr = cache.get(name)
        if arr is None or arr.shape[0] < n or arr.dtype != np.dtype(dtype):
            arr = cache[name] = np.empty(max(n, 1), dtype=dtype)
        return arr[:n]

    def gather_stats(self, d_src, n_src, src_index, d_dst, n_dst, dst_index=None):
        si = np.ascontiguousarray(src_index, dtype=np.int64)
        di = None if dst_index is None else np.ascontiguousarray(dst_index, dtype=np.int64)
        self.check(self.lib.spkd_gather_stats(self.h, C.c_void_p(d_src), n_src, _ptr(si),
                                              None if di is None else _ptr(di), len(si), n_dst,
                                              C.c_void_p(d_dst)))

    def gw(self, d_frames, n_frames, begins, ends, params, log_cap=4096, tight=False, reuse=False,
           seg_stats=None, first_guess_scale=1.0):
        b = np.ascontiguousarray(begins, dtype=np.int64)
        e = np.ascontiguousarray(ends, dtype=np.int64)
        nt = len(b)
        for off in _gw_capacity_ladder(e - b, params, tight, first_guess_scale):
            nev = int(off[-1])
            mk = self._buf if reuse else (lambda name, n, dt: np.empty(n, dtype=dt))
            n_win = mk('n_win', nt, np.int32)
            win_maxd = mk('win_maxd', nev, np.float64)
            win_det = mk('win_det', nev, np.int32)
            det_start = mk('det_start', nev, np.float64)
            det_maxi = mk('det_maxi', nev, np.float64)
            det_d = mk('det_d', nev, np.float64)
            final_start = mk('final_start', nt, np.float64)
            d_seg = None if seg_stats is None else seg_stats(nev)
            while True:
                log = (CandLog * max(log_cap, 1))()
                cnt = C.c_int64(0)
                if seg_stats is None:
                    st = self.lib.spkd_gw_ex(self.h, C.c_void_p(d_frames), n_frames, _ptr(b), _ptr(e), nt,
                                             C.byref(params), _ptr(off), 0, _ptr(n_win),
                                             _ptr(win_maxd), _ptr(win_det), _ptr(det_start), _ptr(det_maxi),
                                             _ptr(det_d), _ptr(final_start), C.cast(log, C.c_void_p), log_cap,
                                             C.byref(cnt))
                else:
                    st = self.lib.spkd_gw_fused(self.h, C.c_void_p(d_frames), n_frames, _ptr(b), _ptr(e), nt,
                                                C.byref(params), _ptr(off), 0, _ptr(n_win),
                                                _ptr(win_maxd), _ptr(win_det), _ptr(det_start), _ptr(det_maxi),
                                                _ptr(det_d), _ptr(final_start), C.c_void_p(d_seg),
                                                C.cast(log, C.c_void_p), log_cap, C.byref(cnt))
                if not (st == SPKD_EOVERFLOW and cnt.value > log_cap):
                    break
                log_cap = int(cnt.value) + 16
            if st != SPKD_EOVERFLOW:
                break
        self.check(st, allow=(SPKD_ENONFINITE,))
        return dict(status=st, off=off, n_ev=nev, n_win=n_win, win_maxd=win_maxd, win_det=win_det,
                    det_start=det_start, det_maxi=det_maxi, det_d=det_d, final_start=final_start,
                    log=log, log_count=min(int(cnt.value), log_cap))

    def gw_batch(self, d_frames, n_frames, begins, ends, params, turn_start_s, turn_end_s, file_off, file_len,
                 seg_stats, tight=True, first_guess_scale=1.0, want_index=False):
        c = np.ascontiguousarray
        b = c(begins, dtype=np.int64)
        e = c(ends, dtype=np.int64)
        nt = len(b)
        host = [c(turn_start_s, dtype=np.float64), c(turn_end_s, dtype=np.float64), c(file_off, dtype=np.int64),
                c(file_len, dtype=np.int64)]
        if any(len(a) != nt for a in host):
            raise SpkdError(SPKD_EINVAL, 'one entry per turn')
        view = GwLinesView()
        for off in _gw_capacity_ladder(e - b, params, tight, first_guess_scale):
            nev = int(off[-1])
            d_seg = seg_stats(nev)
            st = self.lib.spkd_gw_batch(self.h, C.c_void_p(d_frames), n_frames, _ptr(b), _ptr(e), nt, C.byref(params),
                                        _ptr(off), *[_ptr(a) for a in host], C.c_void_p(d_seg),
                                        1 if want_index else 0, C.byref(view))
            if st != SPKD_EOVERFLOW:
                break
        self.check(st, allow=(SPKD_ENONFINITE,))
        n, nr = int(view.n_lines), int(view.n_redo)
        return dict(status=st, off=off, n_ev=nev, d_seg=d_seg, n_lines=n, n_win=_view(view.n_win, nt if n else 0, np.int32),
                    times=_view(view.times, 2 * n, np.float64).reshape(-1, 2), turn=_view(view.turn, n, np.int32),
                    frame_b=_view(view.frame_b, n, np.int64), frame_e=_view(view.frame_e, n, np.int64),
                    index=_view(view.index, n, np.int64) if want_index else None, d_index=view.d_index,
                    redo_line=_view(view.redo_line, nr, np.int64), redo_begin=_view(view.redo_begin, nr, np.int64),
                    redo_end=_view(view.redo_end, nr, np.int64))

    def ahc_fused(self, d_frames, n_frames, d_records, n_records, d_line_index, seg_off, redo_line, redo_begin,
                  redo_end, params):
        c = np.ascontiguousarray
        seg_off = c(seg_off, dtype=np.int64)
        rl, rb, re_ = c(redo_line, dtype=np.int64), c(redo_begin, dtype=np.int64), c(redo_end, dtype=np.int64)
        if not (len(rl) == len(rb) == len(re_)):
            raise SpkdError(SPKD_EINVAL, 'one range per redo line')
        npb, nt = len(seg_off) - 1, int(seg_off[-1])
        out = [C.c_void_p() for _ in range(5)]
        st = self.lib.spkd_ahc_fused(self.h, C.c_void_p(d_frames), n_frames, C.c_void_p(d_records), n_records,
                                     C.c_void_p(d_line_index), _ptr(seg_off), npb, _ptr(rl), _ptr(rb), _ptr(re_), len(rl),
                                     C.byref(params), *[C.byref(o) for o in out])
        self.check(st, allow=(SPKD_ENONFINITE,))
        if st != SPKD_OK:
            return dict(status=st)
        return dict(status=st, n_merges=_view(out[0].value, npb, np.int32), a=_view(out[1].value, nt, np.int32),
                    b=_view(out[2].value, nt, np.int32), d=_view(out[3].value, nt, np.float64),
                    labels=_view(out[4].value, nt, np.int32))

    def sw(self, d_frames, n_frames, begins, ends, params):
        b = np.ascontiguousarray(begins, dtype=np.int64)
        e = np.ascontiguousarray(ends, dtype=np.int64)
        nt = len(b)
        cnt = [self.lib.spkd_sw_window_count(int(e[t] - b[t]), params.winsize, params.winstep)
               for t in range(nt)]
        if any(c < 0 for c in cnt):
            raise SpkdError(SPKD_EINVAL, 'window size and step must be at least one frame')
        off = np.zeros(nt + 1, dtype=np.int64)
        off[1:] = np.cumsum(cnt)
        d = np.zeros(int(off[-1]), dtype=np.float64)
        st = self.lib.spkd_sw(self.h, C.c_void_p(d_frames), n_frames, _ptr(b), _ptr(e), nt,
                              C.byref(params), _ptr(off), _ptr(d))
        self.check(st, allow=(SPKD_ENONFINITE,))
        return st, off, d

    def mfcc(self, d_pcm, n_samples, params, melfb, dct, mean, scale, transform, d_features):
        arrs = [np.ascontiguousarray(a, dtype=np.float32) for a in (melfb, dct, mean, scale, transform)]
        n = C.c_int64(0)
        self.check(self.lib.spkd_mfcc(self.h, C.c_void_p(d_pcm), n_samples, C.byref(params), *[_ptr(a) for a in arrs],
                                      C.c_void_p(d_features), C.byref(n)))
        return int(n.value)

    def gmm_loglik(self, d_features, n_frames, gmm, d_scores):
        a = {k: np.ascontiguousarray(gmm[k], dtype=np.int32 if k in ('state_off', 'kernel') else np.float32)
             for k in ('mean', 'inv_var', 'log_norm', 'state_off', 'kernel', 'log_weight')}
        K, S = len(a['log_norm']), len(a['state_off']) - 1
        if a['mean'].size != K * DIM or a['inv_var'].size != K * DIM or S < 1 or \
                len(a['kernel']) != len(a['log_weight']) or int(a['state_off'][-1]) != len(a['kernel']):
            raise SpkdError(SPKD_EINVAL, 'inconsistent model array sizes')
        p = GmmParams(K, S, a['mean'].shape[-1] if a['mean'].ndim == 2 else DIM,
                      *[_ptr(a[k]) for k in ('mean', 'inv_var', 'log_norm', 'state_off', 'kernel', 'log_weight')])
        self.check(self.lib.spkd_gmm_loglik(self.h, C.c_void_p(d_features), int(n_frames), C.byref(p),
                                            C.c_void_p(d_scores)))

    def ahc(self, d_stats, seg_off, params):
        seg_off = np.ascontiguousarray(seg_off, dtype=np.int64)
        npb = len(seg_off) - 1
        nt = int(seg_off[-1])
        n_merges = np.zeros(npb, dtype=np.int32)
        ma = np.zeros(nt, dtype=np.int32)
        mb = np.zeros(nt, dtype=np.int32)
        md = np.zeros(nt, dtype=np.float64)
        smax = np.zeros(npb, dtype=np.float64)
        smin = np.zeros(npb, dtype=np.float64)
        st = self.lib.spkd_ahc(self.h, C.c_void_p(d_stats), _ptr(seg_off), npb, C.byref(params),
                               _ptr(n_merges), _ptr(ma), _ptr(mb), _ptr(md), _ptr(smax), _ptr(smin))
        self.check(st, allow=(SPKD_ENONFINITE,))
        return dict(status=st, n_merges=n_merges, a=ma, b=mb, d=md, stat_max=smax, stat_min=smin)

    def distance_rows(self, variant, kind, lambdac, d_stats, n, row_begin, row_end, d_rows):
        smax, smin = C.c_double(), C.c_double()
        st = self.lib.spkd_distance_rows(self.h, int(variant), KINDS[kind] if isinstance(kind, str) else int(kind),
                                         float(lambdac), C.c_void_p(d_stats), int(n), int(row_begin), int(row_end),
                                         C.c_void_p(d_rows), C.byref(smax), C.byref(smin))
        self.check(st, allow=(SPKD_ENONFINITE,))
        if st == SPKD_ENONFINITE:
            raise ValueError('array must not contain infs or NaNs')
        return smax.value, smin.value

    def cluster_in(self, d_stats, n, kind, lambdac, threshold):
        n = int(n)
        label = np.zeros(max(n, 1), dtype=np.int32)
        off = np.zeros(n + 1, dtype=np.int64)
        done, nclu = C.c_int64(0), C.c_int64(0)
        full = n * (n - 1) // 2
        cap = min(full, 32 * n)
        while True:
            dist = np.empty(max(cap, 1), dtype=np.float64)
            st = self.lib.spkd_cluster_in(self.h, C.c_void_p(d_stats), n, KINDS[kind] if isinstance(kind, str) else int(kind),
                                          float(lambdac), float(threshold), _ptr(label), _ptr(dist), cap, _ptr(off),
                                          C.byref(done), C.byref(nclu))
            if st == SPKD_EOVERFLOW and cap < full:
                cap = min(full, 4 * cap)
                continue
            break
        self.check(st, allow=(SPKD_ENONFINITE,))
        nd = int(done.value)
        dists = [dist[int(off[s]):int(off[s + 1])].copy() for s in range(nd)]
        return label[:n], dists, nd, int(nclu.value), st

    def ahc_matrix(self, d_stats, n, params, d_matrix, stat_max_in=float('nan'), stat_min_in=float('nan')):
        n = int(n)
        n_merges = np.zeros(1, dtype=np.int32)
        ma = np.zeros(n, dtype=np.int32)
        mb = np.zeros(n, dtype=np.int32)
        md = np.zeros(n, dtype=np.float64)
        smax = np.zeros(1, dtype=np.float64)
        smin = np.zeros(1, dtype=np.float64)
        st = self.lib.spkd_ahc_matrix(self.h, C.c_void_p(d_stats), n, C.byref(params), C.c_void_p(d_matrix),
                                      float(stat_max_in), float(stat_min_in), _ptr(n_merges), _ptr(ma), _ptr(mb),
                                      _ptr(md), _ptr(smax), _ptr(smin))
        self.check(st, allow=(SPKD_ENONFINITE,))
        return dict(status=st, n_merges=n_merges, a=ma, b=mb, d=md, stat_max=smax, stat_min=smin)
```

speaker-diarization_amd/pipeline.py:

```python
import time

import numpy as np

from . import hipabi
from .recipe import py2_float_str

DIA2_CD = dict(kind='BIC', lambdac=1.0, threshold=0.0, winsize_s=1.0, winstep_s=3.0, deltaws_s=0.1)
DIA2_CL = dict(variant=1, kind='BIC', lambdac=1.3, threshold=0.0, max_spk=0)


class BatchFile(object):

    def __init__(self, frame_off, n_frames, vad):
        self.frame_off = int(frame_off)
        self.n_frames = int(n_frames)
        self.vad = [(float(s), float(e)) for (s, e) in vad]
        self.vad_arr = np.array(self.vad, dtype=np.float64).reshape(-1, 2)


class FusedStats(object):

    def __init__(self, d_buf, n_buf, index, begin, end):
        self.d_buf, self.n_buf, self.index, self.begin, self.end = d_buf, n_buf, index, begin, end


def _turn_table(files, rate):
    nturn = [len(f.vad) for f in files]
    if sum(nturn) == 0:
        return None
    vad = np.concatenate([f.vad_arr for f in files])
    owner = np.repeat(np.arange(len(files)), nturn)
    foff = np.array([f.frame_off for f in files], dtype=np.int64)[owner]
    fn = np.array([f.n_frames for f in files], dtype=np.int64)[owner]
    ls, le = vad[:, 0], vad[:, 1]
    f0 = np.minimum((ls * rate).astype(np.int64), fn)
    f1 = np.maximum(f0, np.minimum((le * rate).astype(np.int64), fn))
    return owner, foff, fn, ls, le, foff + f0, foff + f1


def _cd_params(cd, rate):
    return hipabi.CdParams(hipabi.KINDS[cd['kind']], 0, cd['lambdac'], cd['threshold'],
                           float(np.floor(cd['winsize_s'] * rate)), float(np.floor(cd['winstep_s'] * rate)),
                           float(np.floor(rate * cd['deltaws_s'])), rate)


def _ahc_params(cl):
    return hipabi.AhcParams(cl['variant'], hipabi.KINDS[cl['kind']], cl['max_spk'], cl.get('path', 0),
                            cl['lambdac'], cl['threshold'])


def _detector_done(ctx, timings, tb, te, r):
    if timings is not None:
        timings.setdefault('gw', []).append(ctx.last_ms('gw'))
        timings.setdefault('gw_stream_ms', []).append(ctx.last_ms('call'))
        timings['gw_frames'] = int((te - tb).sum())
        timings['gw_windows'] = int(r['n_win'].sum())
        timings['gw_dets'] = ctx.last_gw_items()
    if r['status'] == hipabi.SPKD_ENONFINITE:
        raise ValueError('array must not contain infs or NaNs')


def _time_stats(ctx, timings, n, begin, end):
    if len(begin):
        timings.setdefault('chunk_stats', []).append(ctx.last_ms('chunk_stats'))
        timings.setdefault('reduce_sets', []).append(ctx.last_ms('reduce_sets'))
    timings['stats_frames'] = int((end - begin).sum())
    timings['stats_sets'] = n
    timings['stats_recomputed'] = len(begin)


def _clustering_done(ctx, timings, seg_off, r):
    if timings is not None:
        for k in ('cluster_prep', 'matrix', 'ahc'):
            timings.setdefault(k, []).append(ctx.last_ms(k))
    if r['status'] == hipabi.SPKD_ENONFINITE:
        raise ValueError('array must not contain infs or NaNs')
    if timings is not None:
        npb = np.diff(seg_off)
        nm = r['n_merges'].astype(np.int64)
        timings['matrix_pairs'] = int((npb * (npb - 1) // 2).sum())
        timings['ahc_pairs'] = int((nm * (npb - 2) - nm * (nm - 1) // 2).sum())


def _problems(cnt):
    cnt = np.asarray(cnt, dtype=np.int64)
    kept = np.nonzero(cnt)[0]
    seg_off = np.zeros(len(kept) + 1, dtype=np.int64)
    seg_off[1:] = np.cumsum(cnt[kept])
    return kept, seg_off


def _recipe_rows(times, line_file, labels, rate):
    k0, k1 = times[:, 0] * rate, times[:, 1] * rate
    in_order = (line_file[1:] != line_file[:-1]) | (k0[1:] > k0[:-1]) | ((k0[1:] == k0[:-1]) & (k1[1:] >= k1[:-1]))
    rows = np.column_stack([times, labels.astype(np.float64)])
    if not bool(in_order.all()):
        rows = rows[np.lexsort((np.arange(len(rows)), k1, k0, line_file))]
    return rows


def change_detect_batch(ctx, d_frames, total_frames, files, rate=125.0, cd=DIA2_CD, timings=None,
                        text_contract=True, fused=None):
    rate = float(rate)
    _t0 = time.perf_counter()
    table = _turn_table(files, rate)
    if table is None:
        return [[] for _ in files]
    owner, _, _, ls, le, tb, te = table
    p = _cd_params(cd, rate)
    _t1 = time.perf_counter()
    seg_buf = {}

    def seg_alloc(n_rec):
        seg_buf['n'] = n_rec
        seg_buf['p'] = ctx.dev_scratch('fused_segment_stats', max(n_rec, 1) * hipabi.REC * 8)
        return seg_buf['p']

    r = ctx.gw(d_frames, total_frames, tb, te, p, log_cap=4096, tight=True, reuse=True,
               seg_stats=seg_alloc if fused is not None else None)
    _t2 = time.perf_counter()
    _detector_done(ctx, timings, tb, te, r)
    off = r['off']
    nd = hipabi.count_flags(r['win_det'], off[:-1], r['n_win'])
    lines = hipabi.gw_lines(off[:-1], nd, r['det_start'], r['det_maxi'], r['final_start'], ls, le, tb, te, rate,
                            text_contract=text_contract, want_frames=fused is not None)
    rt, line_turn = lines['times'], lines['turn']
    if fused is not None:
        fused.append(FusedStats(seg_buf['p'], seg_buf['n'], lines['index'], lines['frame_b'], lines['frame_e']))
    line_file = owner[line_turn]
    bounds = np.searchsorted(line_file, np.arange(len(files) + 1))
    out = [rt[bounds[i]:bounds[i + 1]] for i in range(len(files))]
    if timings is not None:
        _t3 = time.perf_counter()
        timings.setdefault('wall_cd_prepare', []).append(1e3 * (_t1 - _t0))
        timings.setdefault('wall_cd_call', []).append(1e3 * (_t2 - _t1))
        timings.setdefault('wall_cd_finish', []).append(1e3 * (_t3 - _t2))
    return out


def segment_stats(ctx, d_frames, total_frames, files, segments, rate=125.0, timings=None, fused=None,
                  scratch_name='segment_stats'):
    cnt = [len(s) for s in segments]
    seg_off = np.zeros(len(files) + 1, dtype=np.int64)
    seg_off[1:] = np.cumsum(cnt)
    n = int(seg_off[-1])
    allseg = np.concatenate([np.asarray(s, dtype=np.float64).reshape(-1, 2) for s in segments]) if n else np.zeros((0, 2))
    owner = np.repeat(np.arange(len(files)), cnt)
    foff = np.array([f.frame_off for f in files], dtype=np.int64)[owner]
    fn = np.array([f.n_frames for f in files], dtype=np.int64)[owner]
    a0 = np.clip((allseg[:, 0] * rate).astype(np.int64), 0, fn)
    a1 = np.maximum(a0, np.clip((allseg[:, 1] * rate).astype(np.int64), 0, fn))
    b, e = foff + a0, foff + a1
    d_stats = ctx.dev_scratch(scratch_name, max(n, 1) * hipabi.REC * 8)
    _t1 = time.perf_counter()
    if fused is None:
        ctx.set_stats(d_frames, total_frames, b, e, np.arange(n, dtype=np.int32), n, d_stats)
        redo = np.arange(n)
    else:
        same = (fused.begin == b) & (fused.end == e)
        keep = np.nonzero(same)[0]
        redo = np.nonzero(~same)[0]
        ctx.gather_stats(fused.d_buf, fused.n_buf, fused.index[keep], d_stats, n, keep)
        if len(redo):
            d_tmp = ctx.dev_scratch(scratch_name + '_redo', len(redo) * hipabi.REC * 8)
            ctx.set_stats(d_frames, total_frames, b[redo], e[redo], np.arange(len(redo), dtype=np.int32),
                          len(redo), d_tmp)
            ctx.gather_stats(d_tmp, len(redo), np.arange(len(redo)), d_stats, n, redo)
    if timings is not None:
        _time_stats(ctx, timings, n, b[redo], e[redo])
    return d_stats, seg_off, n, _t1


def cluster_batch(ctx, d_frames, total_frames, files, segments, rate=125.0, cl=DIA2_CL, timings=None,
                  want_merges=False, fused=None):
    rate = float(rate)
    cnt = [len(s) for s in segments]
    keep = _problems(cnt)[0]
    if len(keep) < len(files):
        out = [(np.zeros(0, dtype=np.int32), [] if want_merges else None) for _ in files]
        if len(keep):
            sub = cluster_batch(ctx, d_frames, total_frames, [files[i] for i in keep],
                                [segments[i] for i in keep], rate, cl, timings, want_merges, fused)
            for i, r in zip(keep, sub):
                out[i] = r
        return out
    _t0 = time.perf_counter()
    d_stats, seg_off, n, _t1 = segment_stats(ctx, d_frames, total_frames, files, segments, rate, timings, fused)
    _t2 = time.perf_counter()
    r = ctx.ahc(d_stats, seg_off, _ahc_params(cl))
    _t3 = time.perf_counter()
    _clustering_done(ctx, timings, seg_off, r)
    all_labels = hipabi.labels_from_merges_batch(seg_off, r['n_merges'], r['a'], r['b'])
    out = []
    for fi in range(len(files)):
        o, c = int(seg_off[fi]), cnt[fi]
        merges = None
        if want_merges:
            nm = int(r['n_merges'][fi])
            merges = list(zip(r['a'][o:o + nm].tolist(), r['b'][o:o + nm].tolist(), r['d'][o:o + nm].tolist()))
        out.append((all_labels[o:o + c], merges))
    if timings is not None:
        _t4 = time.perf_counter()
        timings.setdefault('wall_cl_prepare', []).append(1e3 * (_t1 - _t0))
        timings.setdefault('wall_cl_stats_call', []).append(1e3 * (_t2 - _t1))
        timings.setdefault('wall_cl_ahc_call', []).append(1e3 * (_t3 - _t2))
        timings.setdefault('wall_cl_finish', []).append(1e3 * (_t4 - _t3))
    return out


def diarize_batch_device(ctx, d_frames, total_frames, files, rate=125.0, cd=DIA2_CD, cl=DIA2_CL, timings=None,
                         detail=None, first_guess_scale=1.0):
    rate = float(rate)
    _t0 = time.perf_counter()
    table = _turn_table(files, rate)
    if table is None:
        return [np.zeros((0, 3)) for _ in files]
    owner, foff, fn, ls, le, tb, te = table
    ls, le = np.ascontiguousarray(ls), np.ascontiguousarray(le)
    p = _cd_params(cd, rate)
    _t1 = time.perf_counter()
    r = ctx.gw_batch(d_frames, total_frames, tb, te, p, ls, le, foff, fn,
                     lambda n_rec: ctx.dev_scratch('fused_segment_stats', max(n_rec, 1) * hipabi.REC * 8),
                     tight=True, first_guess_scale=first_guess_scale, want_index=detail is not None)
    _t2 = time.perf_counter()
    _detector_done(ctx, timings, tb, te, r)
    line_file = owner[r['turn']]
    bounds = np.searchsorted(line_file, np.arange(len(files) + 1))
    _t3 = time.perf_counter()
    seg_off = _problems(np.diff(bounds))[1]
    ap = _ahc_params(cl)
    _t4 = time.perf_counter()
    a = ctx.ahc_fused(d_frames, total_frames, r['d_seg'], r['n_ev'], r['d_index'], seg_off, r['redo_line'],
                      r['redo_begin'], r['redo_end'], ap)
    _t5 = time.perf_counter()
    if timings is not None:
        _time_stats(ctx, timings, r['n_lines'], r['redo_begin'], r['redo_end'])
    _clustering_done(ctx, timings, seg_off, a)
    if detail is not None:
        detail['lines'] = {k: (np.array(v) if isinstance(v, np.ndarray) else v) for k, v in r.items()}
        detail['merges'] = [list(zip(a['a'][o:o + m].tolist(), a['b'][o:o + m].tolist(), a['d'][o:o + m].tolist()))
                            for o, m in zip(seg_off[:-1].tolist(), a['n_merges'].tolist())]
    rows = _recipe_rows(r['times'], line_file, a['labels'], rate)
    out = [rows[bounds[i]:bounds[i + 1]] for i in range(len(files))]
    if timings is not None:
        _t6 = time.perf_counter()
        timings.setdefault('wall_cd_prepare', []).append(1e3 * (_t1 - _t0))
        timings.setdefault('wall_cd_call', []).append(1e3 * (_t2 - _t1))
        timings.setdefault('wall_cd_finish', []).append(1e3 * (_t3 - _t2))
        timings.setdefault('wall_cl_prepare', []).append(1e3 * (_t4 - _t3))
        timings.setdefault('wall_cl_stats_call', []).append(0.0)
        timings.setdefault('wall_cl_ahc_call', []).append(1e3 * (_t5 - _t4))
        timings.setdefault('wall_cl_finish', []).append(1e3 * (_t6 - _t5))
    return out


def diarize_batch(ctx, d_frames, total_frames, files, rate=125.0, cd=DIA2_CD, cl=DIA2_CL, timings=None,
                  text_contract=True, fused=False, handoff=None):
    if handoff is None:
        handoff = 'device' if fused and text_contract else 'host'
    if handoff == 'device':
        if not (fused and text_contract):
            raise ValueError('the device hand-off is the fused mode with the text contract')
        return diarize_batch_device(ctx, d_frames, total_frames, files, rate, cd, cl, timings)
    if handoff != 'host':
        raise ValueError('handoff: device or host')
    box = [] if fused else None
    segs = change_detect_batch(ctx, d_frames, total_frames, files, rate, cd, timings, text_contract, box)
    fs = box[0] if box else None
    if fused and fs is None:
        return [np.zeros((0, 3)) for _ in files]
    return _cluster_and_order(ctx, d_frames, total_frames, files, segs, rate, cl, timings, fs)


def _cluster_and_order(ctx, d_frames, total_frames, files, segs, rate, cl, timings, fs):
    res = cluster_batch(ctx, d_frames, total_frames, files, segs, rate, cl, timings, fused=fs)
    cnt = [len(s) for s in segs]
    if sum(cnt) == 0:
        return [np.zeros((0, 3)) for _ in segs]
    allseg = np.concatenate([np.asarray(s, dtype=np.float64).reshape(-1, 2) for s in segs])
    labels = np.concatenate([lab for (lab, _) in res])
    rows = _recipe_rows(allseg, np.repeat(np.arange(len(segs)), cnt), labels, rate)
    bounds = np.zeros(len(segs) + 1, dtype=np.int64)
    bounds[1:] = np.cumsum(cnt)
    out = [rows[bounds[i]:bounds[i + 1]] for i in range(len(segs))]
    return out


def in_flight(contexts, n_jobs, job):
    import threading
    if len(contexts) == 1 or n_jobs <= 1:
        for k in range(n_jobs):
            yield job(contexts[0], k)
        return
    results = [None] * n_jobs
    done = [threading.Event() for _ in range(n_jobs)]
    nxt = [0]
    lock = threading.Lock()
    failure = []

    def worker(ctx):
        while not failure:
            with lock:
                k = nxt[0]
                nxt[0] += 1
            if k >= n_jobs:
                return
            try:
                results[k] = job(ctx, k)
            except BaseException as e:
                failure.append(e)
            finally:
                done[k].set()

    threads = [threading.Thread(target=worker, args=(c,)) for c in contexts]
    for th in threads:
        th.start()
    try:
        for k in range(n_jobs):
            done[k].wait()
            if failure:
                break
            r, results[k] = results[k], None
            yield r
    finally:
        if not failure:
            failure.append(None)
        for th in threads:
            th.join()
    if failure and failure[0] is not None:
        raise failure[0]
```

Before: 1447.

## Replay merge labels on device, fuse/parallelise host roundtrip, radix-sort turns

Adds a GPU kernel that replays AHC merges into cluster labels per problem, so only labels, not the full merge log, are copied back unless the caller asks for it. The py2 decimal roundtrip gets a cheaper exponent estimate and is fused with the redo-line check in a multithreaded pass. The turn length sort becomes a radix sort over an index order, and the turn start/end uploads move into a separate table. Together these aim to cut host-side post-processing and device-to-host transfer, at the cost of more code paths and a serial per-merge shift loop on device.

Measured after the change: 1467 (median of 6 runs). About the same (+1.4%).

```diff
diff --git a/include/spkd.h b/include/spkd.h
--- a/include/spkd.h
+++ b/include/spkd.h
@@ -174,7 +174,7 @@
                            const int64_t *h_seg_off, int64_t n_problems,
                            const int64_t *h_redo_line, const int64_t *h_redo_begin,
                            const int64_t *h_redo_end, int64_t n_redo,
-                           const spkd_ahc_params *params,
+                           const spkd_ahc_params *params, int want_merges,
                            const int32_t **h_n_merges, const int32_t **h_merge_a,
                            const int32_t **h_merge_b, const double **h_merge_d,
                            const int32_t **h_labels);
@@ -204,6 +204,7 @@
                             const spkd_gmm_params *params, float *d_scores);
 
 void spkd_py2_roundtrip(double *h_values, int64_t n);
+void spkd_py2_roundtrip_printf(double *h_values, int64_t n);
 spkd_status spkd_labels_from_merges(int64_t n, int64_t n_merges, const int32_t *h_a,
                                     const int32_t *h_b, int32_t *h_labels);
 spkd_status spkd_labels_from_merges_batch(int64_t n_problems, const int64_t *h_seg_off,
diff --git a/speaker-diarization_amd/csrc/spkd_cluster.hpp b/speaker-diarization_amd/csrc/spkd_cluster.hpp
--- a/speaker-diarization_amd/csrc/spkd_cluster.hpp
+++ b/speaker-diarization_amd/csrc/spkd_cluster.hpp
@@ -848,6 +848,74 @@
     }
 }
 
+constexpr int RP_TPB = 256;
+constexpr int RP_PER_THREAD = 8;
+constexpr long long REPLAY_MAX_N = RP_TPB * RP_PER_THREAD;
+__global__ __launch_bounds__(RP_TPB) void k_replay_labels(const int64_t* __restrict__ seg_off,
+                                                         const int32_t* __restrict__ n_merges,
+                                                         const int32_t* __restrict__ merge_a,
+                                                         const int32_t* __restrict__ merge_b,
+                                                         int32_t* __restrict__ labels, int32_t* __restrict__ bad) {
+    extern __shared__ int32_t rp_lds[];
+    __shared__ int s_bad;
+    const int tid = threadIdx.x;
+    const int p = blockIdx.x;
+    const int64_t off = seg_off[p];
+    const int N = (int)(seg_off[p + 1] - off);
+    if (N <= 0 || N > REPLAY_MAX_N) {
+        if (tid == 0 && N > 0) atomicOr(bad, 1);
+        return;
+    }
+    int32_t* ids = rp_lds;
+    int32_t* lab = ids + N;
+    int32_t* la = lab + N;
+    int32_t* lb = la + N;
+    int nm = n_merges[p];
+    if (tid == 0) s_bad = nm < 0 || nm > N - 1;
+    nm = nm < 0 ? 0 : (nm > N - 1 ? N - 1 : nm);
+    for (int c = tid; c < N; c += RP_TPB) {
+        ids[c] = c;
+        lab[c] = c;
+        la[c] = c < nm ? merge_a[off + c] : 0;
+        lb[c] = c < nm ? merge_b[off + c] : 0;
+    }
+    __syncthreads();
+    int m = N, done = 0;
+    for (; done < nm; ++done) {
+        const int a = la[done], b = lb[done];
+        if (a < 0 || b <= a || b >= m) break;
+        const int ra = ids[a], rb = ids[b];
+        int32_t v[RP_PER_THREAD];
+#pragma unroll
+        for (int j = 0; j < RP_PER_THREAD; ++j) {
+            const int i = b + tid + j * RP_TPB;
+            v[j] = i < m - 1 ? ids[i + 1] : 0;
+        }
+        __syncthreads();
+#pragma unroll
+        for (int j = 0; j < RP_PER_THREAD; ++j) {
+            const int i = b + tid + j * RP_TPB;
+            if (i < m - 1) ids[i] = v[j];
+        }
+        if (tid == 0) { lab[rb] = ra; la[done] = rb; }
+        --m;
+        __syncthreads();
+    }
+    if (done < nm && tid == 0) s_bad = 1;
+    __syncthreads();
+    if (s_bad) {
+        for (int c = tid; c < N; c += RP_TPB) labels[off + c] = 0;
+        if (tid == 0) atomicOr(bad, 1);
+        return;
+    }
+    for (int q = tid; q < m; q += RP_TPB) lab[ids[q]] = q + 1;
+    __syncthreads();
+    if (tid == 0)
+        for (int k = nm - 1; k >= 0; --k) { const int rb = la[k]; lab[rb] = lab[lab[rb]]; }
+    __syncthreads();
+    for (int c = tid; c < N; c += RP_TPB) labels[off + c] = lab[c];
+}
+
 __device__ __forceinline__ void ahc_scan_row(const double* __restrict__ row, long long N,
                                              const int32_t* __restrict__ al, bool all_alive,
                                              long long sub_col, double sub_val, int lane,
diff --git a/speaker-diarization_amd/csrc/spkd_hip.hip b/speaker-diarization_amd/csrc/spkd_hip.hip
--- a/speaker-diarization_amd/csrc/spkd_hip.hip
+++ b/speaker-diarization_amd/csrc/spkd_hip.hip
@@ -24,7 +24,7 @@
 
 namespace {
 constexpr int N_SLOTS = 40;
-enum { PIN_GW_TURNS = 0, PIN_GW_LINES, PIN_AHC_OUT, N_PIN };
+enum { PIN_GW_TURNS = 0, PIN_GW_LINES, PIN_AHC_OUT, PIN_GW_TABLE, N_PIN };
 }
 
 struct spkd_ctx {
@@ -225,6 +225,68 @@
     S_CP_TURNS, S_CP_TIMES, S_CP_LINES, S_REDO_STATS, S_REDO_IDX, S_COUNT
 };
 static_assert(S_COUNT <= N_SLOTS, "scratch slot table too small");
+
+const double kPow10[23] = {1e0, 1e1, 1e2, 1e3, 1e4, 1e5, 1e6, 1e7, 1e8, 1e9, 1e10, 1e11,
+                           1e12, 1e13, 1e14, 1e15, 1e16, 1e17, 1e18, 1e19, 1e20, 1e21, 1e22};
+const uint64_t kPow10u[20] = {1ull, 10ull, 100ull, 1000ull, 10000ull, 100000ull, 1000000ull,
+                              10000000ull, 100000000ull, 1000000000ull, 10000000000ull,
+                              100000000000ull, 1000000000000ull, 10000000000000ull,
+                              100000000000000ull, 1000000000000000ull, 10000000000000000ull,
+                              100000000000000000ull, 1000000000000000000ull,
+                              10000000000000000000ull};
+
+inline uint64_t scaled_digits(uint64_t m, int s, int sh) {
+    const unsigned __int128 prod = (unsigned __int128)m * kPow10u[s];
+    const unsigned __int128 one = 1;
+    const unsigned __int128 remn = prod & ((one << sh) - 1), half = one << (sh - 1);
+    uint64_t q = (uint64_t)(prod >> sh);
+    if (remn > half || (remn == half && (q & 1))) ++q;
+    return q;
+}
+
+inline bool roundtrip_fast(double x, double* out) {
+    if (!(x >= 1e-3 && x < 1e11)) return false;
+    uint64_t bits;
+    std::memcpy(&bits, &x, sizeof bits);
+    const int k2 = (int)(bits >> 52) - 1023;
+    const uint64_t m = (bits & 0xfffffffffffffull) | (1ull << 52);
+    const int sh = 52 - k2;
+    int s = 11 - ((k2 * 1233) >> 12);
+    uint64_t q = scaled_digits(m, s, sh);
+    if (q >= 1000000000000ull) {
+        --s;
+        q = scaled_digits(m, s, sh);
+    }
+    if (q < 100000000000ull || q > 1000000000000ull) return false;
+    *out = (double)q / kPow10[s];
+    return true;
+}
+
+inline double roundtrip_one(double x) {
+    double r;
+    if (roundtrip_fast(x, &r)) return r;
+    char buf[64];
+    std::snprintf(buf, sizeof buf, "%.12g", x);
+    return std::strtod(buf, nullptr);
+}
+
+void roundtrip_range(double* v, int64_t lo, int64_t hi) {
+    for (int64_t i = lo; i < hi; ++i) v[i] = roundtrip_one(v[i]);
+}
+
+template <class Work>
+void split_over_threads(int64_t n, int64_t min_per_thread, Work work) {
+    const int nthreads = (int)std::min<int64_t>(16, n / min_per_thread);
+    if (nthreads <= 1) { work(0, 0, n); return; }
+    std::vector<std::thread> pool;
+    const int64_t step = (n + nthreads - 1) / nthreads;
+    for (int t = 1; t < nthreads; ++t) {
+        const int64_t lo = t * step, hi = std::min<int64_t>(n, lo + step);
+        if (lo < hi) pool.emplace_back(work, t, lo, hi);
+    }
+    work(0, 0, std::min<int64_t>(n, step));
+    for (auto& th : pool) th.join();
+}
 
 }
 
@@ -706,9 +768,17 @@
 }
 
 namespace {
+struct LabelReplay {
+    int32_t* h_labels;
+    int32_t* h_bad;
+    bool want_log;
+    bool* on_device;
+};
+
 spkd_status ahc_impl(spkd_ctx* c, const double* d_stats, const int64_t* h_seg_off, int64_t n_prob,
                      const spkd_ahc_params* P, const MatrixPlan& plan, int32_t* h_n_merges, int32_t* h_merge_a,
-                     int32_t* h_merge_b, double* h_merge_d, double* h_stat_max, double* h_stat_min) {
+                     int32_t* h_merge_b, double* h_merge_d, double* h_stat_max, double* h_stat_min,
+                     const LabelReplay* replay = nullptr) {
     if (!c || !P || n_prob < 0) return SPKD_EINVAL;
     if (n_prob == 0) return SPKD_OK;
     if (!d_stats || !h_seg_off || !h_n_merges || !h_merge_a || !h_merge_b || !h_merge_d ||
@@ -738,21 +808,32 @@
     const int64_t n_total = B.n_total;
     const size_t nt = (size_t)n_total, np = (size_t)n_prob;
     double *d_merge_d, *d_tmp, *d_rmin, *d_fmax, *d_fmin;
-    int32_t *d_a, *d_b, *d_alive, *d_rcache, *d_n;
+    int32_t *d_a, *d_b, *d_alive, *d_rcache, *d_n, *d_lab, *d_bad;
     TRY(carve(c, scratch, S_AHC_OUT, [&](Layout L) {
         return L.part(d_merge_d, nt).part(d_tmp, nt).part(d_rmin, nt).part(d_fmax, np).part(d_fmin, np)
-            .part(d_a, nt).part(d_b, nt).part(d_alive, nt).part(d_rcache, 3 * nt).part(d_n, np).bytes();
+            .part(d_a, nt).part(d_b, nt).part(d_alive, nt).part(d_rcache, 3 * nt).part(d_n, np).part(d_lab, nt)
+            .part(d_bad, 1).bytes();
     }));
+    const bool device_replay = replay && path == SPKD_AHC_MONO && n_max <= REPLAY_MAX_N;
+    if (replay) *replay->on_device = device_replay;
     if (path == SPKD_AHC_MONO) {
         auto kahc = P->kind == SPKD_GLR ? k_ahc<true> : k_ahc<false>;
         if (lds > 48 * 1024)
             (void)hipFuncSetAttribute((const void*)kahc, hipFuncAttributeMaxDynamicSharedMemorySize, (int)lds);
-        Timer t(c, SPKD_T_AHC);
-        hipLaunchKernelGGL(kahc, dim3((unsigned)n_prob), dim3(AHC_TPB), lds, c->stream,
-                           B.ex, B.pk, (const int64_t*)B.seg_off, P->variant, P->kind, P->max_spk, P->lambdac,
-                           P->threshold, B.ld, B.aux, B.mat, (const int64_t*)B.mat_off, d_alive, d_tmp,
-                           d_rmin, d_rcache, d_n, d_a, d_b, d_merge_d, B.smax, B.smin, d_fmax, d_fmin, c->d_err,
-                           c->pinv_cur);
+        {
+            Timer t(c, SPKD_T_AHC);
+            hipLaunchKernelGGL(kahc, dim3((unsigned)n_prob), dim3(AHC_TPB), lds, c->stream,
+                               B.ex, B.pk, (const int64_t*)B.seg_off, P->variant, P->kind, P->max_spk, P->lambdac,
+                               P->threshold, B.ld, B.aux, B.mat, (const int64_t*)B.mat_off, d_alive, d_tmp,
+                               d_rmin, d_rcache, d_n, d_a, d_b, d_merge_d, B.smax, B.smin, d_fmax, d_fmin, c->d_err,
+                               c->pinv_cur);
+        }
+        if (device_replay) {
+            HIPCHK(c, hipMemsetAsync(d_bad, 0, sizeof(int32_t), c->stream));
+            hipLaunchKernelGGL(k_replay_labels, dim3((unsigned)n_prob), dim3(RP_TPB), (size_t)n_max * 4 * sizeof(int32_t),
+                               c->stream, (const int64_t*)B.seg_off, (const int32_t*)d_n, (const int32_t*)d_a,
+                               (const int32_t*)d_b, d_lab, d_bad);
+        }
     } else {
         StepArrays Q;
         void *pe = nullptr, *pp = nullptr;
@@ -809,9 +890,16 @@
     }
     HIPCHK(c, hipGetLastError());
     HIPCHK(c, hipMemcpyAsync(h_n_merges, d_n, (size_t)n_prob * sizeof(int32_t), hipMemcpyDeviceToHost, c->stream));
-    HIPCHK(c, hipMemcpyAsync(h_merge_a, d_a, (size_t)n_total * sizeof(int32_t), hipMemcpyDeviceToHost, c->stream));
-    HIPCHK(c, hipMemcpyAsync(h_merge_b, d_b, (size_t)n_total * sizeof(int32_t), hipMemcpyDeviceToHost, c->stream));
-    HIPCHK(c, hipMemcpyAsync(h_merge_d, d_merge_d, (size_t)n_total * sizeof(double), hipMemcpyDeviceToHost, c->stream));
+    if (device_replay) {
+        HIPCHK(c, hipMemcpyAsync(replay->h_labels, d_lab, (size_t)n_total * sizeof(int32_t), hipMemcpyDeviceToHost, c->stream));
+        HIPCHK(c, hipMemcpyAsync(replay->h_bad, d_bad, sizeof(int32_t), hipMemcpyDeviceToHost, c->stream));
+    }
+    if (!device_replay || replay->want_log) {
+        HIPCHK(c, hipMemcpyAsync(h_merge_a, d_a, (size_t)n_total * sizeof(int32_t), hipMemcpyDeviceToHost, c->stream));
+        HIPCHK(c, hipMemcpyAsync(h_merge_b, d_b, (size_t)n_total * sizeof(int32_t), hipMemcpyDeviceToHost, c->stream));
+        HIPCHK(c, hipMemcpyAsync(h_merge_d, d_merge_d, (size_t)n_total * sizeof(double), hipMemcpyDeviceToHost, c->stream));
+    }
+    if (device_replay) return call.finish();
     HIPCHK(c, hipMemcpyAsync(kmax.data(), B.smax, (size_t)n_prob * sizeof(unsigned long long), hipMemcpyDeviceToHost, c->stream));
     HIPCHK(c, hipMemcpyAsync(kmin.data(), B.smin, (size_t)n_prob * sizeof(unsigned long long), hipMemcpyDeviceToHost, c->stream));
     HIPCHK(c, hipMemcpyAsync(fmax.data(), d_fmax, (size_t)n_prob * sizeof(double), hipMemcpyDeviceToHost, c->stream));
@@ -872,9 +960,11 @@
 namespace {
 spkd_status build_turns(spkd_ctx* c, int64_t n_frames, const int64_t* hb, const int64_t* he, int64_t n_turns,
                         const spkd_cd_params* P, const int64_t* h_off, bool gw, std::vector<TurnDesc>& turns,
-                        int64_t& n_cand) {
+                        std::vector<int32_t>& order, int64_t& n_cand) {
     n_cand = 0;
     turns.resize((size_t)n_turns);
+    order.resize((size_t)n_turns);
+    for (int64_t t = 0; t < n_turns; ++t) order[(size_t)t] = (int32_t)t;
     for (int64_t t = 0; t < n_turns; ++t) {
         if (hb[t] < 0 || he[t] < hb[t] || he[t] > n_frames) return fail(c, SPKD_EINVAL, "bad turn range");
         TurnDesc& T = turns[(size_t)t];
@@ -888,9 +978,29 @@
         T.id = t;
         if (T.ev_cap < 0) return fail(c, SPKD_EINVAL, "offsets must be non-decreasing");
     }
-    if (gw) std::stable_sort(turns.begin(), turns.end(), [](const TurnDesc& a, const TurnDesc& b) { return a.len > b.len; });
-    return SPKD_OK;
-}
+    if (gw && n_turns > 1) {
+        int64_t longest = 0;
+        for (const TurnDesc& T : turns) longest = std::max(longest, T.len);
+        std::vector<int32_t> next((size_t)n_turns);
+        for (int shift = 0; shift < 63 && (longest >> shift) != 0; shift += 11) {
+            size_t start[2049] = {};
+            auto digit = [&](int32_t t) { return (size_t)(((longest - turns[(size_t)t].len) >> shift) & 2047); };
+            for (int32_t t : order) ++start[digit(t) + 1];
+            for (int d = 0; d < 2048; ++d) start[d + 1] += start[d];
+            for (int32_t t : order) next[start[digit(t)]++] = t;
+            order.swap(next);
+        }
+    }
+    return SPKD_OK;
+}
+
+struct GwTable {
+    TurnDesc* turns;
+    double *ls, *le;
+    size_t parts(Layout& L, size_t n_turns, size_t n_times) {
+        return L.part(turns, n_turns).part(ls, n_times).part(le, n_times).bytes();
+    }
+};
 
 struct GwBatch {
     const double *turn_start_s, *turn_end_s;
@@ -909,10 +1019,8 @@
 spkd_status gw_batch_upload(spkd_ctx* c, GwBatch& G, int64_t n_turns) {
     const size_t nt = (size_t)n_turns;
     TRY(carve(c, scratch, S_CP_TURNS, [&](Layout L) {
-        return L.part(G.d_ls, nt).part(G.d_le, nt).part(G.d_line_off, nt + 1).part(G.d_n_det, nt).part(G.d_pos, nt).bytes();
+        return L.part(G.d_line_off, nt + 1).part(G.d_n_det, nt).part(G.d_pos, nt).bytes();
     }));
-    HIPCHK(c, hipMemcpyAsync(G.d_ls, G.turn_start_s, nt * sizeof(double), hipMemcpyHostToDevice, c->stream));
-    HIPCHK(c, hipMemcpyAsync(G.d_le, G.turn_end_s, nt * sizeof(double), hipMemcpyHostToDevice, c->stream));
     return carve(c, pinned, PIN_GW_TURNS, [&](Layout L) { return L.part(G.h_head, 2).part(G.h_n_win, nt).bytes(); });
 }
 
@@ -982,25 +1090,34 @@
 spkd_status gw_batch_finish(spkd_ctx* c, GwBatch& G, int64_t n_turns, double rate) {
     spkd_gw_lines_view& V = *G.view;
     double* times = const_cast<double*>(V.times);
-    spkd_py2_roundtrip(times, 2 * V.n_lines);
+    std::vector<int64_t> part[16];
+    std::atomic<int> bad{0};
+    split_over_threads(V.n_lines, 8192, [&](int th, int64_t lo, int64_t hi) {
+        std::vector<int64_t>& mine = part[th];
+        for (int64_t i = lo; i < hi; ++i) {
+            const int64_t t = V.turn[i];
+            if (t < 0 || t >= n_turns) { bad.store(1); return; }
+            const double t0 = times[2 * i] = roundtrip_one(times[2 * i]);
+            const double t1 = times[2 * i + 1] = roundtrip_one(times[2 * i + 1]);
+            const int64_t fn = G.file_len[t];
+            int64_t a0 = (int64_t)(t0 * rate), a1 = (int64_t)(t1 * rate);
+            a0 = a0 < 0 ? 0 : (a0 > fn ? fn : a0);
+            a1 = a1 < 0 ? 0 : (a1 > fn ? fn : a1);
+            if (a1 < a0) a1 = a0;
+            const int64_t b = G.file_off[t] + a0, e = G.file_off[t] + a1;
+            if (b != V.frame_b[i] || e != V.frame_e[i]) { mine.push_back(i); mine.push_back(b); mine.push_back(e); }
+        }
+    });
+    if (bad.load()) return fail(c, SPKD_EHIP, "internal error: line of no turn");
     c->redo_line.clear();
     c->redo_begin.clear();
     c->redo_end.clear();
-    for (int64_t i = 0; i < V.n_lines; ++i) {
-        const int64_t t = V.turn[i];
-        if (t < 0 || t >= n_turns) return fail(c, SPKD_EHIP, "internal error: line of no turn");
-        const int64_t fn = G.file_len[t];
-        int64_t a0 = (int64_t)(times[2 * i] * rate), a1 = (int64_t)(times[2 * i + 1] * rate);
-        a0 = a0 < 0 ? 0 : (a0 > fn ? fn : a0);
-        a1 = a1 < 0 ? 0 : (a1 > fn ? fn : a1);
-        if (a1 < a0) a1 = a0;
-        const int64_t b = G.file_off[t] + a0, e = G.file_off[t] + a1;
-        if (b != V.frame_b[i] || e != V.frame_e[i]) {
-            c->redo_line.push_back(i);
-            c->redo_begin.push_back(b);
-            c->redo_end.push_back(e);
-        }
-    }
+    for (const std::vector<int64_t>& mine : part)
+        for (size_t k = 0; k + 2 < mine.size(); k += 3) {
+            c->redo_line.push_back(mine[k]);
+            c->redo_begin.push_back(mine[k + 1]);
+            c->redo_end.push_back(mine[k + 2]);
+        }
     V.n_redo = (int64_t)c->redo_line.size();
     V.redo_line = c->redo_line.data();
     V.redo_begin = c->redo_begin.data();
@@ -1057,8 +1174,9 @@
     if (log_cap < 0 || (log_cap > 0 && !out.h_log)) return fail(c, SPKD_EINVAL, "gw: log capacity without a log buffer");
     if (!c->gw_lds_ok) return fail(c, SPKD_EHIP, "gw: the kernel's dynamic LDS size was not admitted on this device");
     std::vector<TurnDesc> turns;
+    std::vector<int32_t> order;
     int64_t n_cand;
-    TRY(build_turns(c, in.n_frames, in.hb, in.he, n_turns, P, in.h_ev_off, true, turns, n_cand));
+    TRY(build_turns(c, in.n_frames, in.hb, in.he, n_turns, P, in.h_ev_off, true, turns, order, n_cand));
     for (int64_t t = 0; in.check_capacity && t < n_turns; ++t)
         if (turns[(size_t)t].ev_cap < spkd_gw_event_capacity_p(turns[(size_t)t].len, P))
             return fail(c, SPKD_EINVAL, "gw: event capacity too small, see spkd_gw_event_capacity_p");
@@ -1071,7 +1189,22 @@
     TurnDesc* d_turns = nullptr;
     void *d_snap = nullptr, *d_cand = nullptr, *d_log = nullptr;
     GwEvents ev;
-    TRY(upload(c, S_TURNS, turns.data(), turns.size(), &d_turns));
+    {
+        const size_t nt = (size_t)n_turns, n_times = batch ? nt : 0;
+        GwTable H, D;
+        TRY(carve(c, pinned, PIN_GW_TABLE, [&](Layout L) { return H.parts(L, nt, n_times); }));
+        TRY(carve(c, scratch, S_TURNS, [&](Layout L) { return D.parts(L, nt, n_times); }));
+        for (size_t i = 0; i < nt; ++i) H.turns[i] = turns[(size_t)order[i]];
+        if (batch) {
+            std::memcpy(H.ls, batch->turn_start_s, nt * sizeof(double));
+            std::memcpy(H.le, batch->turn_end_s, nt * sizeof(double));
+            batch->d_ls = D.ls;
+            batch->d_le = D.le;
+        }
+        Layout measure;
+        HIPCHK(c, hipMemcpyAsync(D.turns, H.turns, GwTable().parts(measure, nt, n_times), hipMemcpyHostToDevice, c->stream));
+        d_turns = D.turns;
+    }
     TRY(scratch(c, S_SNAP, (size_t)n_cand * REC * sizeof(double), &d_snap));
     TRY(scratch(c, S_CAND, (size_t)n_cand * 4 * sizeof(double), &d_cand));
     auto ev_bytes = [&](const GwEventArray& a) { return (size_t)(a.per_turn ? n_turns : n_ev) * a.elem; };
@@ -1202,7 +1335,7 @@
 spkd_status spkd_ahc_fused(spkd_ctx* c, const float* d_frames, int64_t n_frames, const double* d_records,
                            int64_t n_records, int64_t* d_line_index, const int64_t* h_seg_off, int64_t n_prob,
                            const int64_t* h_redo_line, const int64_t* h_redo_begin, const int64_t* h_redo_end,
-                           int64_t n_redo, const spkd_ahc_params* P, const int32_t** h_n_merges,
+                           int64_t n_redo, const spkd_ahc_params* P, int want_merges, const int32_t** h_n_merges,
                            const int32_t** h_merge_a, const int32_t** h_merge_b, const double** h_merge_d,
                            const int32_t** h_labels) {
     if (!c || !P || n_prob < 0 || n_redo < 0) return SPKD_EINVAL;
@@ -1223,10 +1356,14 @@
             return fail(c, SPKD_EINVAL, "ahc_fused: redo lines must be ascending line indices");
     const size_t nt = (size_t)n_total, np = (size_t)n_prob;
     double *md, *smax, *smin;
-    int32_t *ma, *mb, *lab, *nm;
+    int32_t *ma, *mb, *lab, *nm, *bad;
     TRY(carve(c, pinned, PIN_AHC_OUT, [&](Layout L) {
-        return L.part(md, nt).part(smax, np).part(smin, np).part(ma, nt).part(mb, nt).part(lab, nt).part(nm, np).bytes();
+        return L.part(md, nt).part(smax, np).part(smin, np).part(ma, nt).part(mb, nt).part(lab, nt).part(nm, np)
+            .part(bad, 1).bytes();
     }));
+    *bad = 0;
+    bool on_device = false;
+    const LabelReplay replay = {lab, bad, want_merges != 0, &on_device};
     MatrixPlan plan;
     plan.d_map = d_line_index;
     plan.n_src = n_records;
@@ -1236,13 +1373,14 @@
     plan.redo_begin = h_redo_begin;
     plan.redo_end = h_redo_end;
     plan.n_redo = n_redo;
-    TRY(ahc_impl(c, d_records, h_seg_off, n_prob, P, plan, nm, ma, mb, md, smax, smin));
-    if (spkd_labels_from_merges_batch(n_prob, h_seg_off, nm, ma, mb, lab) != SPKD_OK)
+    TRY(ahc_impl(c, d_records, h_seg_off, n_prob, P, plan, nm, ma, mb, md, smax, smin, &replay));
+    if (on_device ? *bad != 0 : spkd_labels_from_merges_batch(n_prob, h_seg_off, nm, ma, mb, lab) != SPKD_OK)
         return fail(c, SPKD_EHIP, "internal error: merge log does not replay");
+    const bool have_log = !on_device || want_merges;
     *h_n_merges = nm;
-    *h_merge_a = ma;
-    *h_merge_b = mb;
-    *h_merge_d = md;
+    *h_merge_a = have_log ? ma : nullptr;
+    *h_merge_b = have_log ? mb : nullptr;
+    *h_merge_d = have_log ? md : nullptr;
     *h_labels = lab;
     return SPKD_OK;
 }
@@ -1414,74 +1552,16 @@
     return call.finish();
 }
 
-static const double kPow10[23] = {1e0, 1e1, 1e2, 1e3, 1e4, 1e5, 1e6, 1e7, 1e8, 1e9, 1e10, 1e11,
-                                  1e12, 1e13, 1e14, 1e15, 1e16, 1e17, 1e18, 1e19, 1e20, 1e21, 1e22};
-static const uint64_t kPow10u[20] = {1ull, 10ull, 100ull, 1000ull, 10000ull, 100000ull, 1000000ull,
-                                     10000000ull, 100000000ull, 1000000000ull, 10000000000ull,
-                                     100000000000ull, 1000000000000ull, 10000000000000ull,
-                                     100000000000000ull, 1000000000000000ull, 10000000000000000ull,
-                                     100000000000000000ull, 1000000000000000000ull,
-                                     10000000000000000000ull};
-
-static bool roundtrip_fast(double x, double* out) {
-    if (!(x >= 1e-3 && x < 1e11)) return false;
-    int e10 = (int)std::floor(std::log10(x));
-    if (e10 < -3) e10 = -3;
-    if (e10 >= 0) { if (x < kPow10[e10]) --e10; else if (e10 + 1 <= 22 && x >= kPow10[e10 + 1]) ++e10; }
-    else { if (x * kPow10[-e10] < 1.0) --e10; else if (x * kPow10[-e10 - 1] >= 1.0) ++e10; }
-    if (e10 < -3 || e10 > 10) return false;
-    int s = 11 - e10;
-    int k;
-    const double fr = std::frexp(x, &k);
-    const uint64_t m = (uint64_t)std::ldexp(fr, 53);
-    k -= 53;
-    unsigned __int128 prod = (unsigned __int128)m * kPow10u[s];
-    uint64_t q;
-    if (k >= 0) {
-        if (k > 20) return false;
-        q = (uint64_t)(prod << k);
-    } else {
-        const int sh = -k;
-        if (sh >= 120) return false;
-        const unsigned __int128 one = 1;
-        const unsigned __int128 fl = prod >> sh;
-        const unsigned __int128 remn = prod & ((one << sh) - 1);
-        const unsigned __int128 half = one << (sh - 1);
-        q = (uint64_t)fl;
-        if (remn > half || (remn == half && (q & 1))) ++q;
-    }
-    if (q >= 1000000000000ull) {
-        if (q != 1000000000000ull) return false;
-        q = 100000000000ull;
-        s -= 1;
-    } else if (q < 100000000000ull) {
-        return false;
-    }
-    *out = s >= 0 ? (double)q / kPow10[s] : (double)q * kPow10[-s];
-    return true;
-}
-
-static void roundtrip_range(double* v, int64_t lo, int64_t hi) {
+void spkd_py2_roundtrip(double* v, int64_t n) {
+    split_over_threads(n, 16384, [v](int, int64_t lo, int64_t hi) { roundtrip_range(v, lo, hi); });
+}
+
+void spkd_py2_roundtrip_printf(double* v, int64_t n) {
     char buf[64];
-    for (int64_t i = lo; i < hi; ++i) {
-        double r;
-        if (roundtrip_fast(v[i], &r)) { v[i] = r; continue; }
+    for (int64_t i = 0; i < n; ++i) {
         std::snprintf(buf, sizeof buf, "%.12g", v[i]);
         v[i] = std::strtod(buf, nullptr);
     }
-}
-
-void spkd_py2_roundtrip(double* v, int64_t n) {
-    const int64_t kMinPerThread = 8192;
-    int nthreads = (int)std::min<int64_t>(8, n / kMinPerThread);
-    if (nthreads <= 1) { roundtrip_range(v, 0, n); return; }
-    std::vector<std::thread> pool;
-    const int64_t step = (n + nthreads - 1) / nthreads;
-    for (int t = 0; t < nthreads; ++t) {
-        const int64_t lo = t * step, hi = std::min<int64_t>(n, lo + step);
-        if (lo < hi) pool.emplace_back(roundtrip_range, v, lo, hi);
-    }
-    for (auto& th : pool) th.join();
 }
 
 spkd_status spkd_labels_from_merges(int64_t n, int64_t n_merges, const int32_t* h_a, const int32_t* h_b,
diff --git a/speaker-diarization_amd/hipabi.py b/speaker-diarization_amd/hipabi.py
--- a/speaker-diarization_amd/hipabi.py
+++ b/speaker-diarization_amd/hipabi.py
@@ -18,7 +18,7 @@
            'spkd_malloc', 'spkd_free', 'spkd_memcpy_h2d', 'spkd_memcpy_d2h', 'spkd_memcpy_d2d',
            'spkd_last_kernel_ms', 'spkd_last_gw_items', 'spkd_set_stats', 'spkd_pair_terms',
            'spkd_distance_matrix', 'spkd_gw_event_capacity', 'spkd_gw_event_capacity_p', 'spkd_gw', 'spkd_gw_ex', 'spkd_gw_fused', 'spkd_gw_batch', 'spkd_ahc_fused', 'spkd_gather_stats', 'spkd_mfcc',
-           'spkd_sw_window_count', 'spkd_sw', 'spkd_ahc', 'spkd_ahc_matrix', 'spkd_distance_rows', 'spkd_cluster_in', 'spkd_py2_roundtrip',
+           'spkd_sw_window_count', 'spkd_sw', 'spkd_ahc', 'spkd_ahc_matrix', 'spkd_distance_rows', 'spkd_cluster_in', 'spkd_py2_roundtrip', 'spkd_py2_roundtrip_printf',
            'spkd_labels_from_merges', 'spkd_labels_from_merges_batch', 'spkd_count_flags', 'spkd_gw_lines',
            'spkd_gmm_loglik', 'spkd_vad_viterbi']
 
@@ -155,7 +155,7 @@
                                   vp, vp, vp, i64, P(i64)]
     lib.spkd_gw_batch.argtypes = [vp, vp, i64, vp, vp, i64, P(CdParams), vp, vp, vp, vp, vp, vp, C.c_int, P(GwLinesView)]
     lib.spkd_ahc_fused.argtypes = [vp, vp, i64, vp, i64, vp, vp, i64, vp, vp, vp, i64, P(AhcParams),
-                                   P(vp), P(vp), P(vp), P(vp), P(vp)]
+                                   C.c_int, P(vp), P(vp), P(vp), P(vp), P(vp)]
     lib.spkd_gather_stats.argtypes = [vp, vp, i64, vp, vp, i64, i64, vp]
     lib.spkd_mfcc.argtypes = [vp, vp, i64, P(MfccParams), vp, vp, vp, vp, vp, vp, P(i64)]
     lib.spkd_sw_window_count.argtypes = [i64, dbl, dbl]
@@ -167,6 +167,8 @@
     lib.spkd_cluster_in.argtypes = [vp, vp, i64, C.c_int, dbl, dbl, vp, vp, i64, vp, P(i64), P(i64)]
     lib.spkd_py2_roundtrip.argtypes = [vp, i64]
     lib.spkd_py2_roundtrip.restype = None
+    lib.spkd_py2_roundtrip_printf.argtypes = [vp, i64]
+    lib.spkd_py2_roundtrip_printf.restype = None
     lib.spkd_labels_from_merges.argtypes = [i64, i64, vp, vp, vp]
     lib.spkd_labels_from_merges_batch.argtypes = [i64, vp, vp, vp, vp, vp]
     lib.spkd_count_flags.argtypes = [vp, vp, vp, i64, vp]
@@ -191,10 +193,11 @@
     return np.ctypeslib.as_array(C.cast(C.c_void_p(addr), C.POINTER(ct)), shape=(int(n),))
 
 
-def py2_roundtrip(values):
+def py2_roundtrip(values, printf=False):
     v = np.ascontiguousarray(values, dtype=np.float64).copy()
     if v.size:
-        load_library().spkd_py2_roundtrip(_ptr(v), v.size)
+        lib = load_library()
+        (lib.spkd_py2_roundtrip_printf if printf else lib.spkd_py2_roundtrip)(_ptr(v), v.size)
     return v
 
 
@@ -482,7 +485,7 @@
                     redo_end=_view(view.redo_end, nr, np.int64))
 
     def ahc_fused(self, d_frames, n_frames, d_records, n_records, d_line_index, seg_off, redo_line, redo_begin,
-                  redo_end, params):
+                  redo_end, params, want_merges=False):
         c = np.ascontiguousarray
         seg_off = c(seg_off, dtype=np.int64)
         rl, rb, re_ = c(redo_line, dtype=np.int64), c(redo_begin, dtype=np.int64), c(redo_end, dtype=np.int64)
@@ -492,12 +495,12 @@
         out = [C.c_void_p() for _ in range(5)]
         st = self.lib.spkd_ahc_fused(self.h, C.c_void_p(d_frames), n_frames, C.c_void_p(d_records), n_records,
                                      C.c_void_p(d_line_index), _ptr(seg_off), npb, _ptr(rl), _ptr(rb), _ptr(re_), len(rl),
-                                     C.byref(params), *[C.byref(o) for o in out])
+                                     C.byref(params), 1 if want_merges else 0, *[C.byref(o) for o in out])
         self.check(st, allow=(SPKD_ENONFINITE,))
         if st != SPKD_OK:
             return dict(status=st)
-        return dict(status=st, n_merges=_view(out[0].value, npb, np.int32), a=_view(out[1].value, nt, np.int32),
-                    b=_view(out[2].value, nt, np.int32), d=_view(out[3].value, nt, np.float64),
+        log = [_view(o.value, nt, t) if o.value else None for o, t in zip(out[1:4], (np.int32, np.int32, np.float64))]
+        return dict(status=st, n_merges=_view(out[0].value, npb, np.int32), a=log[0], b=log[1], d=log[2],
                     labels=_view(out[4].value, nt, np.int32))
 
     def sw(self, d_frames, n_frames, begins, ends, params):
diff --git a/speaker-diarization_amd/pipeline.py b/speaker-diarization_amd/pipeline.py
--- a/speaker-diarization_amd/pipeline.py
+++ b/speaker-diarization_amd/pipeline.py
@@ -231,7 +231,7 @@
     ap = _ahc_params(cl)
     _t4 = time.perf_counter()
     a = ctx.ahc_fused(d_frames, total_frames, r['d_seg'], r['n_ev'], r['d_index'], seg_off, r['redo_line'],
-                      r['redo_begin'], r['redo_end'], ap)
+                      r['redo_begin'], r['redo_end'], ap, want_merges=detail is not None)
     _t5 = time.perf_counter()
     if timings is not None:
         _time_stats(ctx, timings, r['n_lines'], r['redo_begin'], r['redo_end'])
```
